# Alee08/multiagent-rl-rm

Measured on AMD Instinct MI355X. Metric: env×agent steps/sec at 65,536 envs (1/2/4/8 GPU) + CPU-ref parity rate, higher is better.
Workload: dtype int32; 1 GPU; FrozenLake map1, 65,536 envs/GPU x 2 agents, built-in A->B->C RM (3-state RM), random actions; n_envs_per_gpu=65536, n_envs_total=65536, n_agents=2, rm_states=4, parallelism=dp1 (env shards, no data-path collective), dispatch=queue, windows=5

## Files before the change

### include/rmx.h

```cpp
#ifndef RMX_H
#define RMX_H

#include <stdint.h>
#include <stddef.h>

#ifdef __cplusplus
extern "C" {
#endif

#define RMX_ABI_VERSION 12

#define RMX_MAX_AGENTS 8
#define RMX_MAX_CELLS 4096
#define RMX_MAX_RM_STATES 255
#define RMX_MAX_EVENTS 255

#define RMX_OK 0
#define RMX_E_INVALID (-1)
#define RMX_E_HIP (-2)
#define RMX_E_ACTION (-3)
#define RMX_E_STATE (-4)
#define RMX_E_TRACE (-5)

#define RMX_DEVICE_HOST (-1)

#define RMX_FROZEN_LAKE 0
#define RMX_OFFICE_WORLD 1

#define RMX_UP 0
#define RMX_DOWN 1
#define RMX_LEFT 2
#define RMX_RIGHT 3
#define RMX_WAIT 4

#define RMX_CELL_CAN_UP 0x01u
#define RMX_CELL_CAN_DOWN 0x02u
#define RMX_CELL_CAN_LEFT 0x04u
#define RMX_CELL_CAN_RIGHT 0x08u
#define RMX_CELL_HAZARD 0x10u

#define RMX_F_ACTIVE 0x01u
#define RMX_F_FAIL 0x02u
#define RMX_F_TERM 0x04u
#define RMX_F_TRUNC 0x08u
#define RMX_F_ENV_TERM 0x10u
#define RMX_F_RM_TERM 0x20u
#define RMX_F_ENV_DONE 0x40u
#define RMX_F_STEPS_SHIFT 16

#define RMX_STAT_SUM_RETURN 0
#define RMX_STAT_EPISODES 1
#define RMX_STAT_SUCCESSES 2
#define RMX_STAT_SUM_LENGTH 3
#define RMX_NSTATS 4

typedef struct rmx_config {
  int32_t kind;
  int32_t width;
  int32_t height;
  int32_t n_agents;
  int32_t n_rm_states;
  int32_t n_events;
  int32_t max_t;
  int32_t device;
  int64_t n_envs;
  int64_t env_offset;
  int64_t n_envs_global;
  float hazard_penalty;
  float wall_penalty;
  int32_t hazard_fail;
  int32_t wall_fail;
  float gamma;
  int32_t has_shaping;
  float reward_modifier;
  int32_t n_qrm_max;
  int32_t stochastic;
  int32_t slip_n[4];
  int32_t slip_out[4][4];
  double slip_cdf[4][4];
  uint64_t seed_scale, seed_env_stride, seed_episode_stride;
  int32_t random_starts;
  const uint16_t* cell;
  const uint8_t* cell_event;
  const uint8_t* next_q;
  const float* rm_reward;
  const float* shape;
  const int32_t* init_q;
  const int32_t* final_q;
  const int32_t* start_xy;
  const int32_t* n_qrm;
  const uint8_t* qrm_states;
  const int32_t* enc_nq;
} rmx_config;

typedef struct rmx_buffers {
  int32_t* pos_x;
  int32_t* pos_y;
  int32_t* rm_q;
  uint32_t* flags;
  float* ep_ret;
  int32_t* t;
  float* reward;
  float* shaping;
  uint8_t* env_done;
  float* renv;
  int32_t* qrm_s;
  int32_t* qrm_sn;
  float* qrm_rq;
  uint8_t* qrm_done;
  uint64_t* rng;
  int32_t* episode;
  int32_t* enc_state;
} rmx_buffers;

typedef struct rmx_handle rmx_handle;

int rmx_abi_version(void);
int rmx_device_count(int32_t* n);
const char* rmx_last_error(void);
const char* rmx_build_info(void);

int rmx_create(const rmx_config* cfg, rmx_handle** out);
void rmx_destroy(rmx_handle* h);

int rmx_bind(rmx_handle* h, const rmx_buffers* buf);

int rmx_reset(rmx_handle* h, const uint8_t* env_mask_dev, uint64_t seed, void* hip_stream);

int rmx_step(rmx_handle* h, const int32_t* actions_dev, int autoreset, void* hip_stream);

int rmx_step_hashed(rmx_handle* h, uint64_t seed, int64_t t_global, int autoreset, void* hip_stream);

int rmx_fill_actions(rmx_handle* h, uint64_t seed, int64_t t0, int32_t T, int32_t* actions_dev,
                     void* hip_stream);

int rmx_rollout(rmx_handle* h, uint64_t seed, int64_t t0, int32_t T, float* reward_trace_dev,
                void* hip_stream);

int rmx_mdp_states(rmx_handle* h, int32_t agent, int64_t* n_states);
int rmx_mdp(rmx_handle* h, int32_t agent, int32_t fix_frozen_lake, int32_t* next_dev, float* reward_dev,
            uint8_t* done_dev, void* hip_stream);

int rmx_stats_device(rmx_handle* h, double* out_dev, void* hip_stream);
int rmx_stats_host(rmx_handle* h, double* out_host);
int rmx_stats_clear(rmx_handle* h, void* hip_stream);

int rmx_step_report(rmx_handle* h, const int32_t* actions_dev, int autoreset, double* stats_out_dev,
                    void* hip_stream);
int rmx_step_report_fused(const rmx_handle* h);

int rmx_step_seq(rmx_handle* h, const int32_t* actions_dev, int64_t action_stride, int32_t n_steps, int autoreset,
                 double* stats_out_dev, void* hip_stream);
int rmx_seq_packed(const rmx_handle* h);
int rmx_queue_counters(const rmx_handle* h, int64_t* out3);
#define RMX_QUEUE_INFO_N 7
#define RMX_QUEUE_UNUSED 0
#define RMX_QUEUE_READY 1
#define RMX_QUEUE_UNAVAILABLE 2
#define RMX_QUEUE_RETIRED 3
#define RMX_SEQ_NONE 0
#define RMX_SEQ_QUEUE 1
#define RMX_SEQ_STREAM_KERNEL 2
#define RMX_SEQ_STREAM_DISABLED 3
#define RMX_SEQ_STREAM_QUEUE 4
#define RMX_SEQ_HOST 5
int rmx_queue_info(const rmx_handle* h, int64_t* out, int32_t n);
int rmx_queue_timing(rmx_handle* h, int every);
int rmx_queue_times(const rmx_handle* h, uint64_t* stamps, int64_t cap, int64_t* n);
int rmx_code_object_check(const void* co, size_t bytes, int64_t* n_step_kernels, int64_t* n_refused, char* report,
                          size_t report_cap);

#define RMX_VARIANT_GENERIC 0
#define RMX_VARIANT_LANE_PER_AGENT 1
#define RMX_VARIANT_FAST 2
#define RMX_VARIANT_FAST_LANE_PER_AGENT 3
#define RMX_VARIANT_HOST 4
int rmx_step_variant(const rmx_handle* h);

#define RMX_STEP_INFO_N 14
#define RMX_TABLES_NONE 0
#define RMX_TABLES_GLOBAL 1
#define RMX_TABLES_MERGED 2
#define RMX_TABLES_MERGED4 3
int rmx_step_info(const rmx_handle* h, int64_t* out, int32_t n);

typedef struct rmx_learn_config {
  double gamma, learning_rate ;
  int32_t use_qrm, use_rsh, trunc_is_terminal, dynamics ;
  const double* phi;
} rmx_learn_config;
#define RMX_LEARN_DYN_FIXED 0
#define RMX_LEARN_DYN_ENV 1
#define RMX_LEARN_UPDATE 1
#define RMX_LEARN_BEST 2
#define RMX_LEARN_NUMPY 4
int rmx_learn_states(const rmx_handle* h, int64_t* s_max);
int rmx_learn_bind(rmx_handle* h, const rmx_learn_config* cfg, double* q, double* visits);
int rmx_learn_step(rmx_handle* h, const int32_t* actions, int autoreset, void* hip_stream);
int rmx_learn_step_policy(rmx_handle* h, double epsilon, int flags, uint64_t seed, int64_t t_global, int autoreset,
                          int32_t* actions_out, void* hip_stream);
#define RMX_LEARN_RUN_MAX 4096
int rmx_learn_run(rmx_handle* h, int32_t T, double epsilon, int flags, uint64_t seed, int64_t t_global,
                  int32_t* actions_out , void* hip_stream);
int rmx_learn_rng_bind(rmx_handle* h, uint64_t* rng);
int rmx_learn_rng_seed(rmx_handle* h, const uint64_t* seeds_host , void* hip_stream);

int rmx_learn_lambda_slots(const rmx_handle* h, int32_t* l_full);
int rmx_learn_lambda_bind(rmx_handle* h, double lambd, int32_t cap, int32_t* trace_idx, double* trace_val,
                          int32_t* trace_cnt);
int rmx_learn_traces_clear(rmx_handle* h, const uint8_t* env_mask_dev, void* hip_stream);

int rmx_learn_eps_bind(rmx_handle* h, double* eps , double eps_end, double eps_decay);
int rmx_learn_eps_decay(rmx_handle* h, const uint8_t* env_mask , void* hip_stream);

int rmx_check_errors(rmx_handle* h);

int rmx_state_bytes(const rmx_handle* h, size_t* bytes);
int rmx_get_state(rmx_handle* h, void* host_blob, size_t bytes);
int rmx_set_state(rmx_handle* h, const void* host_blob, size_t bytes);

#define RMX_SYNC_MAX_ENVS 256
int rmx_reset_sync(rmx_handle* h, uint64_t seed, const rmx_buffers* out_host, void* hip_stream);
int rmx_step_sync(rmx_handle* h, const int32_t* actions_host, int autoreset, const rmx_buffers* out_host,
                  void* hip_stream);
int rmx_step_sync_begin(rmx_handle* h, const int32_t* actions_host, int autoreset, void* hip_stream);
int rmx_sync_wait(rmx_handle* h, const rmx_buffers* out_host);
int rmx_sync_end(rmx_handle* h);

#ifdef __cplusplus
}
#endif

#endif
```

### multiagent-rl-rm_amd/csrc/rmx_capi.cpp

```cpp
#include <algorithm>
#include <cstdlib>
#include <cstring>
#include <exception>
#include <string>
#include <vector>

#include "rmx_handle.h"

using namespace rmx::capi;

rmx::KParams rmx::capi::base_params(const rmx_handle* h) {
  rmx::KParams p;
  std::memset(&p, 0, sizeof(p));
  const rmx_config& c = h->cfg;
  p.tables = reinterpret_cast<const uint4*>(h->d_tables);
  p.tables_n16 = (int32_t)(h->tables_bytes / 16);
  p.skip_same = h->generic_skip;
  p.off_cell = h->off_cell;
  p.off_ev = h->off_ev;
  p.off_nq = h->off_nq;
  p.off_rr = h->off_rr;
  p.off_sh = h->off_sh;
  p.off_qrm = h->off_qrm;
  p.reward_modifier = c.reward_modifier;
  p.n_qrm_max = c.n_qrm_max;
  p.stochastic = c.stochastic ? 1 : 0;
  rmx::slip_fill(p, c);
  p.seed_scale = c.seed_scale;
  p.seed_env_stride = c.seed_env_stride;
  p.seed_episode_stride = c.seed_episode_stride;
  p.base_seed = h->base_seed;
  p.rng = h->buf.rng;
  p.episode = h->buf.episode;
  p.rng_on = (c.stochastic || c.random_starts) ? 1 : 0;
  p.random_starts = c.random_starts ? 1 : 0;
  p.n_free = h->n_free;
  p.free_cells = h->d_free;
  p.start_ws = h->d_start_ws;
  if (h->d_rsc) {
    p.rs_cells = reinterpret_cast<uint32_t*>(h->d_rsc);
    p.rs_rng = reinterpret_cast<uint64_t*>(h->d_rsc + rmx::start_cache_rng_off(c.n_agents, c.n_envs));
  }
  for (int a = 0; a < RMX_MAX_AGENTS; ++a) {
    p.n_qrm[a] = h->n_qrm[a];
    p.enc_nq[a] = h->enc_nq[a];
  }
  p.W = c.width;
  p.HW = c.width * c.height;
  p.A = c.n_agents;
  p.Q = c.n_rm_states;
  p.E = c.n_events;
  p.max_t = c.max_t;
  p.N = c.n_envs;
  p.hazard_penalty = c.hazard_penalty;
  p.wall_penalty = c.wall_penalty;
  p.hazard_fail = c.hazard_fail ? 1 : 0;
  p.wall_fail = c.wall_fail ? 1 : 0;
  p.has_shaping = c.has_shaping ? 1 : 0;
  p.gamma_is_one = (c.gamma == 1.0f) ? 1 : 0;
  for (int a = 0; a < RMX_MAX_AGENTS; ++a) {
    p.init_q[a] = h->init_q[a];
    p.final_q[a] = h->final_q[a];
    p.start_x[a] = h->start_x[a];
    p.start_y[a] = h->start_y[a];
  }
  p.disc = h->d_disc;
  p.pos_x = h->buf.pos_x;
  p.pos_y = h->buf.pos_y;
  p.rm_q = h->buf.rm_q;
  p.flags = h->buf.flags;
  p.ep_ret = h->buf.ep_ret;
  p.t = h->buf.t;
  p.reward = h->buf.reward;
  p.shaping = h->buf.shaping;
  p.env_done = h->buf.env_done;
  p.renv = h->buf.renv;
  p.enc_state = h->buf.enc_state;
  if (c.n_qrm_max > 0 && h->buf.qrm_s) {
    p.qrm_s = h->buf.qrm_s;
    p.qrm_sn = h->buf.qrm_sn;
    p.qrm_rq = h->buf.qrm_rq;
    p.qrm_done = h->buf.qrm_done;
  }
  p.env_offset = c.env_offset;
  p.n_global = c.n_envs_global;
  p.slab = h->d_slab;
  p.err = h->d_err;
  p.diag = h->diag;
  return p;
}

rmx::FastParams rmx::capi::fast_params(const rmx_handle* h) {
  rmx::FastParams p;
  std::memset(&p, 0, sizeof(p));
  const rmx_config& c = h->cfg;
  p.tables = reinterpret_cast<const uint4*>(h->d_fast);
  p.n16 = h->fast_n16;
  p.off_rm = h->fast_off_rm;
  p.off_info = h->fast_off_info;
  p.A = c.n_agents;
  p.W = c.width;
  p.E = c.n_events;
  p.max_t = c.max_t;
  p.N = (int32_t)c.n_envs;
  for (int a = 0; a < c.n_agents; ++a) {
    p.mv_base[a] = a * c.width * c.height * 5;
    p.rm_base[a] = a * c.n_rm_states * c.n_events;
    p.final_q[a] = h->final_q[a];
    p.init_q[a] = h->init_q[a];
    p.start_x[a] = h->start_x[a];
    p.start_y[a] = h->start_y[a];
  }
  p.hazard_penalty = c.hazard_penalty;
  p.wall_penalty = c.wall_penalty;
  p.has_shaping = c.has_shaping ? 1 : 0;
  p.gamma_is_one = (c.gamma == 1.0f) ? 1 : 0;
  p.tbl_mode = h->fast_tables;
  p.H = c.height;
  p.hazard_fail = c.hazard_fail ? 1 : 0;
  p.wall_fail = c.wall_fail ? 1 : 0;
  p.merged = reinterpret_cast<const uint4*>(h->d_merged);
  p.merged4 = h->merged4_bytes ? reinterpret_cast<const uint32_t*>(static_cast<unsigned char*>(h->d_merged) + h->merged4_off)
                               : nullptr;
  p.merged4_bytes = (int32_t)h->merged4_bytes;
  std::memcpy(p.mg_palb, h->mg_palb, sizeof(p.mg_palb));
  p.merged_bytes = (int32_t)h->merged_bytes;
  if (c.n_qrm_max > 0 && h->buf.qrm_s) {
    p.qrm_s = h->buf.qrm_s;
    p.qrm_sn = h->buf.qrm_sn;
    p.qrm_rq = h->buf.qrm_rq;
    p.qrm_done = h->buf.qrm_done;
    p.n_qrm_max = c.n_qrm_max;
    for (int a = 0; a < c.n_agents; ++a) {
      p.n_qrm[a] = h->n_qrm[a];
      p.enc_nq[a] = h->enc_nq[a];
      for (int j = 0; j < c.n_qrm_max && j < rmx::kFastMaxQrm; ++j) p.qrm_q[a][j] = h->fast_qrm_q[a][j];
    }
  }
  p.HW = c.width * c.height;
  for (int a = 0; a < c.n_agents; ++a) {
    p.mg_base[a] = h->mg_base[a];
    p.enc_nq[a] = h->enc_nq[a];
  }
  p.disc = h->d_disc;
  p.pos_x = h->buf.pos_x;
  p.pos_y = h->buf.pos_y;
  p.rm_q = h->buf.rm_q;
  p.flags = h->buf.flags;
  p.ep_ret = h->buf.ep_ret;
  p.t = h->buf.t;
  p.reward = h->buf.reward;
  p.shaping = h->buf.shaping;
  p.env_done = h->buf.env_done;
  p.renv = h->buf.renv;
  p.enc_state = h->buf.enc_state;
  p.env_offset = c.env_offset;
  p.n_global = c.n_envs_global;
  p.wave_stats = h->fast_wave_stats;
  p.skip_same = h->fast_skip;
  p.block = h->fast_block;
  p.slab = h->d_slab;
  p.es_ret = h->es_ret;
  p.es_cnt = h->es_cnt;
  p.es_succ = h->es_succ;
  p.err = h->d_err;
  p.diag = h->diag;
  p.stamps = h->d_stamps;
  p.pk = h->seq.d_pk;
  if (c.stochastic || c.random_starts) {
    p.slip = (c.stochastic ? rmx::kRngSlip : 0) | (c.random_starts ? rmx::kRngStarts : 0) |
             (h->seed_fixed ? rmx::kRngFixedSeed : 0);
    p.n_free = h->n_free;
    p.free_cells = h->d_free;
    p.start_ws = h->d_start_ws;
    if (h->d_rsc) {
      p.rs_cells = reinterpret_cast<const uint32_t*>(h->d_rsc);
      p.rs_rng = reinterpret_cast<const uint64_t*>(h->d_rsc + rmx::start_cache_rng_off(c.n_agents, c.n_envs));
      p.rs_dirty = h->rs_dirty ? 1 : 0;
    }
    if (h->d_nx) {
      const size_t N = (size_t)c.n_envs;
      p.nx_rng = reinterpret_cast<uint64_t*>(h->d_nx);
      p.nx_idx = reinterpret_cast<int32_t*>(h->d_nx + 32 * N);
      p.nx_ep = reinterpret_cast<int32_t*>(h->d_nx + 36 * N);
      p.rs_jump = reinterpret_cast<const uint4*>(h->d_nx + nx_jump_offset(c.n_envs));
    }
    rmx::slip_fill(p, c);
    p.seed_scale = c.seed_scale;
    p.seed_env_stride = c.seed_env_stride;
    p.seed_episode_stride = c.seed_episode_stride;
    p.base_seed = h->base_seed;
    p.rng = h->buf.rng;
    p.episode = h->buf.episode;
  }
  return p;
}

bool rmx::capi::fast_applies(const rmx_handle* h) {
  if (h->fast && (h->cfg.stochastic || h->cfg.random_starts)) {
    const int tm = h->fast_tables;
    return !h->buf.qrm_s && h->fast_skip == rmx::kSkipRare && (tm == rmx::kTblMerged4 || tm == rmx::kTblMerged) &&
           h->cfg.n_envs < ((int64_t)1 << 27) &&
           (!h->cfg.random_starts || h->seed_fixed || h->n_free + 8 <= rmx::kRsRowMax);
  }
  const int qmax = h->cfg.n_agents <= 2 ? rmx::kFastMaxQrm : 8;
  return h->fast && (!h->buf.qrm_s || (h->cfg.n_qrm_max <= qmax &&
                                       (int64_t)h->cfg.n_qrm_max * h->cfg.n_agents * h->cfg.n_envs < ((int64_t)1 << 30)));
}

hipError_t rmx::capi::reduce_stats(const rmx_handle* h, double* out, hipStream_t st) {
  double* partial = h->d_slab + (size_t)RMX_NSTATS * h->n_waves;
  unsigned int* ticket = reinterpret_cast<unsigned int*>(partial + (size_t)RMX_NSTATS * 2 * rmx::kStatsPartials);
  return rmx::launch_stats_reduce(h->d_slab, h->n_waves, h->es_ret, h->es_cnt, h->es_succ, h->cfg.n_envs, partial,
                                  ticket, out, st);
}

static hipError_t invalidate_next_shuffles(const rmx_handle* h, hipStream_t st) {
  if (!h->d_nx) return hipSuccess;
  const size_t N = (size_t)h->cfg.n_envs;
  return hipMemsetAsync(h->d_nx + 36 * N, 0xFF, 4 * N, st);
}

hipError_t rmx::capi::refresh_starts(rmx_handle* h, hipStream_t st) {
  hipError_t e = hipSuccess;
  if (h->d_rsc) e = rmx::launch_reset(base_params(h), nullptr, 0, st);
  if (e == hipSuccess) e = invalidate_next_shuffles(h, st);
  if (e == hipSuccess) h->rs_stale = false;
  return e;
}

int rmx::capi::starts_current(rmx_handle* h, void* stream) {
  if (h->rs_stale) HIP_TRY(refresh_starts(h, as_stream(stream)), "start cache refresh");
  return RMX_OK;
}

rmx::FastParams rmx::capi::step_fp(const rmx_handle* h, const int32_t* actions, uint64_t seed, int64_t t_global,
                                   int autoreset) {
  rmx::FastParams fp = fast_params(h);
  if (!h->cfg.random_starts) fp.slip &= ~rmx::kRngFixedSeed;
  fp.actions = actions;
  fp.seed = seed;
  fp.t_global = t_global;
  fp.autoreset = autoreset ? 1 : 0;
  if (fp.qrm_s) fp.tbl_mode = rmx::kTblGlobal;
  return fp;
}

int rmx::capi::do_step(rmx_handle* h, const int32_t* actions, int hashed, uint64_t seed, int64_t t_global, int autoreset,
                       void* stream) {
  int rc = check_bound(h);
  if (rc) return rc;
  if (!hashed && !actions) return fail(RMX_E_INVALID, "actions is NULL");
  if (h->host) {
    h->host->step(actions, autoreset, hashed != 0, seed, t_global);
    return RMX_OK;
  }
  SYNC_END_OR_RETURN(h);
  HIP_TRY(hipSetDevice(h->device), "hipSetDevice");
  if ((rc = starts_current(h, stream))) return rc;
  if (fast_applies(h)) {
    const rmx::FastParams fp = step_fp(h, actions, seed, t_global, autoreset);
    HIP_TRY(rmx::launch_step_fast(fp, hashed, h->cfg.kind, as_stream(stream)), "step launch");
    return RMX_OK;
  }
  rmx::KParams p = base_params(h);
  p.actions = actions;
  p.seed = seed;
  p.t_global = t_global;
  p.autoreset = autoreset ? 1 : 0;
  HIP_TRY(rmx::launch_step(p, hashed, h->cfg.kind, h->step_layout, grid_for(h, h->step_layout), dim3(h->block), h->tables_bytes, as_stream(stream)),
          "step launch");
  return RMX_OK;
}

bool rmx::capi::report_fuses(const rmx_handle* h) {
  const int64_t grid = (h->cfg.n_envs + 63) / 64;
  const int tm = h->fast_tables;
  return fast_applies(h) && !h->buf.qrm_s && !h->fast_wave_stats && h->fast_block == 64 &&
         h->fast_skip == rmx::kSkipRare && h->rpt_partial &&
         (tm == rmx::kTblMerged4 || tm == rmx::kTblMerged || tm == rmx::kTblGlobal) && h->n_waves <= 64 * grid;
}

rmx::FastParams rmx::capi::report_fp(const rmx_handle* h, const int32_t* actions, int autoreset, double* stats_out) {
  rmx::FastParams fp = fast_params(h);
  fp.actions = actions;
  fp.autoreset = autoreset ? 1 : 0;
  const int64_t grid = (h->cfg.n_envs + 63) / 64;
  fp.rpt_out = stats_out;
  fp.rpt_partial = h->rpt_partial;
  fp.rpt_ticket = h->rpt_ticket;
  fp.rpt_cs = (int32_t)((h->n_waves + grid - 1) / grid);
  fp.rpt_n_slab = (int32_t)h->n_waves;
  return fp;
}

extern "C" {

int rmx_abi_version(void) { return RMX_ABI_VERSION; }

int rmx_device_count(int32_t* n) {
  if (!n) return fail(RMX_E_INVALID, "n is NULL");
  int c = 0;
  const hipError_t e = hipGetDeviceCount(&c);
  *n = e == hipSuccess ? c : 0;
  return RMX_OK;
}

const char* rmx_last_error(void) { return g_err.c_str(); }

void rmx_destroy(rmx_handle* h) {
  if (!h) return;
  if (h->host) {
    delete h->host;
    delete h;
    return;
  }
  (void)hipSetDevice(h->device);
  (void)sync_end(h);
  if (h->sync.mb) (void)hipHostFree(h->sync.mb);
  if (h->sync.done) (void)hipEventDestroy(h->sync.done);
  if (h->sync.dep) (void)hipEventDestroy(h->sync.dep);
  if (h->sync.stream) (void)hipStreamDestroy(h->sync.stream);
  (void)hipFree(h->d_tables);
  (void)hipFree(h->d_disc);
  (void)hipFree(h->d_slab);
  (void)hipFree(h->d_stats);
  (void)hipFree(h->d_err);
  (void)hipFree(h->d_fast);
  (void)hipFree(h->d_merged);
  (void)hipFree(h->d_es);
  (void)hipFree(h->d_stamps);
  (void)hipFree(h->d_free);
  (void)hipFree(h->d_start_ws);
  (void)hipFree(h->d_nx);
  (void)hipFree(h->d_rsc);
  (void)hipFree(h->seq.d_pk);
  (void)hipFree(h->learn.d_phi);
  delete h;
}

int rmx_bind(rmx_handle* h, const rmx_buffers* b) {
  if (!h || !b) return fail(RMX_E_INVALID, "handle or buffers NULL");
  if (!b->pos_x || !b->pos_y || !b->rm_q || !b->flags || !b->ep_ret || !b->t || !b->reward)
    return fail(RMX_E_STATE, "a required state/output buffer is NULL");
  const bool any_qrm = b->qrm_s || b->qrm_sn || b->qrm_rq || b->qrm_done;
  const bool all_qrm = b->qrm_s && b->qrm_sn && b->qrm_rq && b->qrm_done;
  if (any_qrm && !all_qrm) return fail(RMX_E_STATE, "QRM outputs must be all bound or all NULL");
  if (all_qrm && h->cfg.n_qrm_max == 0) return fail(RMX_E_STATE, "QRM outputs bound but n_qrm_max == 0");
  if ((h->cfg.stochastic || h->cfg.random_starts) && (!b->rng || !b->episode))
    return fail(RMX_E_STATE, "stochastic mode / random starts need the rng and episode buffers");
  if (b->enc_state)
    for (int a = 0; a < h->cfg.n_agents; ++a)
      if (h->enc_nq[a] < 1) return fail(RMX_E_STATE, "enc_state bound but enc_nq not provided at rmx_create");
  if (h->host) {
    h->host->bind(*b);
    h->buf = *b;
    h->bound = true;
    return RMX_OK;
  }
  SYNC_END_OR_RETURN(h);
  if (h->sync.mb) {
    (void)hipHostFree(h->sync.mb);
    h->sync.mb = nullptr;
  }
  h->buf = *b;
  h->bound = true;
  h->rs_dirty = true;
  return RMX_OK;
}

int rmx_reset(rmx_handle* h, const uint8_t* env_mask_dev, uint64_t seed, void* stream) {
  int rc = check_bound(h);
  if (rc) return rc;
  if (h->host) {
    h->host->reset(env_mask_dev, seed);
    h->base_seed = seed;
    return RMX_OK;
  }
  SYNC_END_OR_RETURN(h);
  h->rs_dirty = env_mask_dev ? (h->rs_dirty || seed != h->base_seed) : false;
  h->base_seed = seed;
  HIP_TRY(hipSetDevice(h->device), "hipSetDevice");
  rmx::KParams p = base_params(h);
  HIP_TRY(rmx::launch_reset(p, env_mask_dev, 1, as_stream(stream)), "reset launch");
  HIP_TRY(invalidate_next_shuffles(h, as_stream(stream)), "reset precompute");
  h->rs_stale = false;
  return lambda_clear(h, env_mask_dev, stream);
}

int rmx_step(rmx_handle* h, const int32_t* actions_dev, int autoreset, void* stream) {
  return do_step(h, actions_dev, 0, 0, 0, autoreset, stream);
}

int rmx_step_report(rmx_handle* h, const int32_t* actions_dev, int autoreset, double* stats_out_dev, void* stream) {
  int rc = check_bound(h);
  if (rc) return rc;
  if (!actions_dev || !stats_out_dev) return fail(RMX_E_INVALID, "bad rmx_step_report arguments");
  if (h->host) {
    h->host->step(actions_dev, autoreset);
    std::memcpy(stats_out_dev, h->host->stats, sizeof(h->host->stats));
    return RMX_OK;
  }
  SYNC_END_OR_RETURN(h);
  if (!report_fuses(h)) {
    if ((rc = do_step(h, actions_dev, 0, 0, 0, autoreset, stream))) return rc;
    HIP_TRY(reduce_stats(h, stats_out_dev, as_stream(stream)), "stats launch");
    return RMX_OK;
  }
  HIP_TRY(hipSetDevice(h->device), "hipSetDevice");
  const rmx::FastParams fp = report_fp(h, actions_dev, autoreset, stats_out_dev);
  HIP_TRY(rmx::launch_step_fast(fp, 0, h->cfg.kind, as_stream(stream)), "step launch");
  return RMX_OK;
}

int rmx_step_report_fused(const rmx_handle* h) { return h && h->bound && report_fuses(h) ? 1 : 0; }

int rmx_step_hashed(rmx_handle* h, uint64_t seed, int64_t t_global, int autoreset, void* stream) {
  if (t_global < 0) return fail(RMX_E_INVALID, "t_global < 0");
  return do_step(h, nullptr, 1, seed, t_global, autoreset, stream);
}

int rmx_fill_actions(rmx_handle* h, uint64_t seed, int64_t t0, int32_t T, int32_t* actions_dev, void* stream) {
  if (!h || !actions_dev || T < 0 || t0 < 0) return fail(RMX_E_INVALID, "bad rmx_fill_actions arguments");
  if (T == 0) return RMX_OK;
  if (h->host) {
    h->host->fill_actions(seed, t0, T, actions_dev);
    return RMX_OK;
  }
  HIP_TRY(hipSetDevice(h->device), "hipSetDevice");
  HIP_TRY(rmx::launch_fill_actions(seed, t0, T, h->cfg.n_envs_global, h->cfg.env_offset, h->cfg.n_envs,
                                   h->cfg.n_agents, actions_dev, as_stream(stream)),
          "fill_actions launch");
  return RMX_OK;
}

int rmx_rollout(rmx_handle* h, uint64_t seed, int64_t t0, int32_t T, float* trace, void* stream) {
  int rc = check_bound(h);
  if (rc) return rc;
  if (T < 0 || t0 < 0) return fail(RMX_E_INVALID, "bad rollout length");
  if (T == 0) return RMX_OK;
  if (h->host) {
    const size_t AN = (size_t)h->cfg.n_agents * (size_t)h->cfg.n_envs;
    for (int32_t it = 0; it < T; ++it) h->host->step(nullptr, 1, true, seed, t0 + it, trace ? trace + (size_t)it * AN : nullptr);
    return RMX_OK;
  }
  SYNC_END_OR_RETURN(h);
  HIP_TRY(hipSetDevice(h->device), "hipSetDevice");
  if ((rc = starts_current(h, stream))) return rc;
  if (h->fast && ((!h->cfg.stochastic && !h->cfg.random_starts) || fast_applies(h))) {
    rmx::FastParams fp = fast_params(h);
    fp.seed = seed;
    fp.t_global = t0;
    fp.autoreset = 1;
    const bool merged = fp.tbl_mode == rmx::kTblMerged || fp.tbl_mode == rmx::kTblMerged4;
    const size_t rs_lds = h->cfg.random_starts ? 4 * (size_t)rmx::kRsWaveLds : 0;
    if (h->rollout_lds && (!merged || ((h->merged_bytes + 15) & ~(size_t)15) + rs_lds <= rmx::kRolloutLdsMax)) {
      fp.tbl_mode = merged ? rmx::kTblMergedLds : rmx::kTblLds;
      fp.block = 256;
    } else {
      fp.tbl_mode = merged ? rmx::kTblMerged : rmx::kTblGlobal;
    }
    HIP_TRY(rmx::launch_rollout_fast(fp, h->cfg.kind, T, trace, as_stream(stream)), "rollout launch");
    return RMX_OK;
  }
  rmx::KParams p = base_params(h);
  p.seed = seed;
  p.t_global = t0;
  p.autoreset = 1;
  HIP_TRY(rmx::launch_rollout(p, h->cfg.kind, h->rollout_layout, T, trace, grid_for(h, h->rollout_layout), dim3(h->block), h->tables_bytes,
                              as_stream(stream)),
          "rollout launch");
  return RMX_OK;
}

int rmx_mdp_states(rmx_handle* h, int32_t agent, int64_t* n_states) {
  if (!h || !n_states || agent < 0 || agent >= h->cfg.n_agents) return fail(RMX_E_INVALID, "bad rmx_mdp_states arguments");
  if (h->enc_nq[agent] < 1) return fail(RMX_E_INVALID, "enc_nq not provided at rmx_create");
  *n_states = (int64_t)h->cfg.width * h->cfg.height * h->enc_nq[agent];
  return RMX_OK;
}

int rmx_mdp(rmx_handle* h, int32_t agent, int32_t fix_frozen_lake, int32_t* next_dev, float* reward_dev,
            uint8_t* done_dev, void* stream) {
  int64_t S = 0;
  int rc = rmx_mdp_states(h, agent, &S);
  if (rc) return rc;
  if (!next_dev || !reward_dev || !done_dev) return fail(RMX_E_INVALID, "rmx_mdp output is NULL");
  if (h->host) {
    h->host->mdp(agent, fix_frozen_lake ? 1 : 0, next_dev, reward_dev, done_dev);
// ... 118 lines not shown
```

### multiagent-rl-rm_amd/csrc/rmx_capi_create.cpp

```cpp
#include <algorithm>
#include <cstdlib>
#include <cstring>
#include <exception>
#include <string>
#include <vector>

#include "rmx_handle.h"

using namespace rmx::capi;

namespace {

int validate(const rmx_config* c) {
  if (!c) return fail(RMX_E_INVALID, "config is NULL");
  const std::string msg = rmx::validate_config(*c);
  return msg.empty() ? RMX_OK : fail(RMX_E_INVALID, msg);
}

int create_host(const rmx_config* cfg, rmx_handle** out) {
  rmx_handle* h = new rmx_handle();
  h->host = new rmx::HostEngine();
  const std::string msg = h->host->init(*cfg);
  if (!msg.empty()) {
    delete h->host;
    delete h;
    return fail(RMX_E_INVALID, msg);
  }
  h->cfg = h->host->cfg;
  h->device = RMX_DEVICE_HOST;
  h->digest = rmx::config_digest(*cfg);
  for (int a = 0; a < cfg->n_agents; ++a) h->enc_nq[a] = h->host->p.enc_nq[a];
  *out = h;
  return RMX_OK;
}

struct RsJumpTable {
  uint32_t w[64][2][4];
  RsJumpTable() {
    typedef unsigned __int128 u128;
    const u128 M = ((u128)0x2360ED051FC65DA4ull << 64) | 0x4385DF649FCCF645ull;
    u128 mj = 1, sj = 0;
    for (int j = 0; j < 64; ++j) {
      sj += mj;
      mj *= M;
      const u128 v[2] = {mj, sj};
      for (int k = 0; k < 2; ++k)
        for (int q = 0; q < 4; ++q) w[j][k][q] = (uint32_t)(v[k] >> (32 * q));
    }
  }
};
const RsJumpTable rs_jump_table;

}

extern "C" {

struct CreateTables {
  std::vector<unsigned char> blob, fast_blob;
  std::vector<uint32_t> merged_tab;
  std::vector<float> disc;
  std::vector<uint16_t> free_cells;
};

static void create_env(rmx_handle* h, const rmx_config* cfg) {
  if (const char* qv = std::getenv("RMX_QUEUE")) h->seq.queue_off = std::strcmp(qv, "0") == 0;
  if (const char* pv = std::getenv("RMX_SEQ_PACKED")) h->seq.packed_off = std::strcmp(pv, "0") == 0;
  if (const char* b = std::getenv("RMX_BLOCK")) {
    int v = std::atoi(b);
    if (v == 64 || v == 128 || v == 256) h->block = v;
  }
#ifdef RMX_DIAG
  if (const char* d = std::getenv("RMX_DIAG_BITS")) h->diag = std::atoi(d);
#endif
  const bool rng_on = cfg->stochastic || cfg->random_starts;
  if (rng_on) h->rollout_layout = rmx::kLayoutThreadPerEnv;
  if (const char* l = std::getenv("RMX_LAYOUT")) {
    if (!std::strcmp(l, "tpe")) h->step_layout = h->rollout_layout = rmx::kLayoutThreadPerEnv;
    if (!std::strcmp(l, "lpe") && !rng_on) h->step_layout = h->rollout_layout = rmx::kLayoutLanePerAgent;
  }
}

static bool create_plan(rmx_handle* h, const rmx_config* cfg, CreateTables& tb) {
  const int A = cfg->n_agents;
  for (int a = 0; a < A; ++a) {
    h->init_q[a] = cfg->init_q[a];
    h->final_q[a] = cfg->final_q[a];
    h->start_x[a] = cfg->start_xy[2 * a];
    h->start_y[a] = cfg->start_xy[2 * a + 1];
  }
  rmx::BlobOffsets bo;
  if (!rmx::build_table_blob(*cfg, tb.blob, bo)) return false;
  h->tables_bytes = tb.blob.size();
  h->digest = rmx::config_digest(*cfg);
  h->off_cell = bo.cell;
  h->off_ev = bo.ev;
  h->off_nq = bo.nq;
  h->off_rr = bo.rr;
  h->off_sh = bo.sh;
  h->off_qrm = bo.qrm;
  if (cfg->n_qrm_max > 0) {
    for (int a = 0; a < A; ++a) {
      h->n_qrm[a] = cfg->n_qrm[a];
      for (int j = 0; j < cfg->n_qrm_max && j < rmx::kFastMaxQrm; ++j)
        h->fast_qrm_q[a][j] = cfg->qrm_states[a * cfg->n_qrm_max + j];
    }
  }
  for (int a = 0; a < A; ++a) h->enc_nq[a] = cfg->enc_nq ? cfg->enc_nq[a] : 0;
  tb.disc = rmx::discount_table(*cfg);
  if (cfg->random_starts) tb.free_cells = rmx::free_cells(*cfg);
  h->n_free = (int32_t)tb.free_cells.size();
  const int64_t gmax = std::max(grid_for(h, h->step_layout).x, grid_for(h, h->rollout_layout).x);
  std::vector<unsigned char>& fast_blob = tb.fast_blob;
  std::vector<uint32_t>& merged_tab = tb.merged_tab;
  {
    const char* fe = std::getenv("RMX_FAST");
    const bool want = fe ? std::strcmp(fe, "0") != 0 : true;
    rmx::FastLayout fl;
    h->fast = want && h->step_layout == rmx::kLayoutThreadPerEnv && rmx::build_fast_blob(*cfg, fast_blob, fl);
    h->fast_off_rm = fl.off_rm;
    h->fast_off_info = fl.off_info;
    h->fast_n16 = (int32_t)(fast_blob.size() / 16);
    if (h->fast) {
      std::vector<uint32_t> probe;
      const bool ok = rmx::build_merged(*cfg, fast_blob, h->fast_off_rm, h->mg_base, probe);
      h->fast_tables = ok && probe.size() * 4 <= kFastMergedDefaultBytes ? rmx::kTblMerged : rmx::kTblGlobal;
      if (h->fast_tables == rmx::kTblMerged && !cfg->stochastic) h->fast_tables = rmx::kTblMerged4;
    }
    if (const char* ft = std::getenv("RMX_FAST_TABLES")) {
      if (!std::strcmp(ft, "global")) h->fast_tables = rmx::kTblGlobal;
      if (!std::strcmp(ft, "merged")) h->fast_tables = rmx::kTblMerged;
      if (!std::strcmp(ft, "merged4")) h->fast_tables = rmx::kTblMerged4;
    }
    const bool want_m4 = h->fast_tables == rmx::kTblMerged4;
    if (h->fast && (h->fast_tables == rmx::kTblMerged || want_m4) &&
        !rmx::build_merged(*cfg, fast_blob, h->fast_off_rm, h->mg_base, merged_tab))
      h->fast_tables = rmx::kTblGlobal;
    if (want_m4 && h->fast_tables != rmx::kTblGlobal) {
      std::vector<uint32_t> compact;
      if (rmx::build_compact(*cfg, h->mg_base, merged_tab, h->mg_palb, compact)) {
        h->merged4_off = merged_tab.size() * 4;
        h->merged4_bytes = compact.size() * 4;
        merged_tab.insert(merged_tab.end(), compact.begin(), compact.end());
        while (merged_tab.size() % 4) merged_tab.push_back(0u);
      } else {
        h->fast_tables = rmx::kTblMerged;
      }
    }
    if (h->fast && h->fast_tables != rmx::kTblGlobal) {
      const size_t sec_words = (size_t)cfg->n_rm_states * cfg->width * cfg->height * 5 * 4;
      const size_t words16 = h->merged4_bytes ? h->merged4_off / 4 : merged_tab.size();
      h->merged_sections = (int)(words16 / sec_words);
    }
    if (!merged_tab.empty()) h->merged_bytes = h->merged4_bytes ? h->merged4_off : merged_tab.size() * 4;
  }
  h->seed_fixed = h->fast && (cfg->stochastic || cfg->random_starts) && cfg->seed_episode_stride == 0;
  h->n_waves = std::max<int64_t>(gmax * (h->block / 64), (cfg->n_envs + 255) / 256 * 4);
  h->fast_wave_stats = cfg->n_envs >= kFastWaveStatsMinEnvs ? 1 : 0;
  if (const char* fs = std::getenv("RMX_FAST_STATS")) h->fast_wave_stats = !std::strcmp(fs, "wave") ? 1 : 0;
  h->fast_skip = cfg->n_envs * (int64_t)cfg->n_agents >= kFastNtMinInstances ? rmx::kSkipRareNT : rmx::kSkipRare;
  h->generic_skip = cfg->n_envs >= kFastSkipMinEnvs ? 1 : 0;
  if (const char* fk = std::getenv("RMX_FAST_SKIP")) {
    const int v = std::atoi(fk);
    if (v == rmx::kSkipRare || v == rmx::kSkipRareNT) h->fast_skip = v;
  }
  if (const char* gk = std::getenv("RMX_GENERIC_SKIP")) h->generic_skip = std::atoi(gk) ? 1 : 0;
  h->fast_block = cfg->n_envs >= kFastSkipMinEnvs ? 256 : 64;
  if (const char* rl = std::getenv("RMX_ROLLOUT_LDS")) h->rollout_lds = std::atoi(rl) ? 1 : 0;
  return true;
}

static hipError_t create_upload(rmx_handle* h, const rmx_config* cfg, const CreateTables& tb) {
  hipError_t e = hipSuccess;
  auto put = [&e](auto** p, size_t bytes, int fill, const void* src = nullptr, size_t src_bytes = 0) {
    if (e == hipSuccess) e = hipMalloc(p, bytes);
    if (e == hipSuccess && fill >= 0) e = hipMemset(*p, fill, bytes);
    if (e == hipSuccess && src) e = hipMemcpy(*p, src, src_bytes, hipMemcpyHostToDevice);
  };
  const size_t N = (size_t)cfg->n_envs;
#ifdef RMX_DIAG
  if (std::getenv("RMX_DIAG_STAMPS")) put(&h->d_stamps, (N + 255) / 256 * 4 * 2 * rmx::kStamps * 8, 0);
#endif
  if (h->fast && !h->fast_wave_stats) {
    const size_t o_cnt = 8 * N, o_succ = o_cnt + 8 * N, o_part = (o_succ + 4 * N + 15) & ~size_t(15);
    const size_t o_ticket = (o_part + sizeof(double) * RMX_NSTATS * ((N + 63) / 64) + 127) & ~size_t(127);
    h->es_bytes = o_ticket + 128 * (1 + 32);
    put(&h->d_es, h->es_bytes, 0);
    if (e == hipSuccess) {
      h->es_ret = reinterpret_cast<double*>(h->d_es);
      h->es_cnt = reinterpret_cast<unsigned long long*>(h->d_es + o_cnt);
      h->es_succ = reinterpret_cast<uint32_t*>(h->d_es + o_succ);
      h->rpt_partial = reinterpret_cast<double*>(h->d_es + o_part);
      h->rpt_ticket = reinterpret_cast<unsigned int*>(h->d_es + o_ticket);
    }
  }
  put(&h->d_tables, h->tables_bytes, -1, tb.blob.data(), h->tables_bytes);
  put(&h->d_disc, sizeof(float) * tb.disc.size(), -1, tb.disc.data(), sizeof(float) * tb.disc.size());
  put(&h->d_slab, sizeof(double) * (RMX_NSTATS * (h->n_waves + 2 * rmx::kStatsPartials) + 2), 0);
  put(&h->d_stats, sizeof(double) * RMX_NSTATS, -1);
  put(&h->d_err, sizeof(uint32_t), 0);
  if (h->n_free > 0) {
    put(&h->d_free, sizeof(uint16_t) * (tb.free_cells.size() + 1), 0, tb.free_cells.data(),
        sizeof(uint16_t) * tb.free_cells.size());
    put(&h->d_start_ws, sizeof(uint16_t) * (size_t)rmx::shuffle_stride((int32_t)tb.free_cells.size()) * N, -1);
    if (!h->seed_fixed) {
      put(&h->d_nx, nx_jump_offset(cfg->n_envs) + sizeof(rs_jump_table.w), -1);
      if (e == hipSuccess) e = hipMemset(h->d_nx + 36 * N, 0xFF, 4 * N);
      if (e == hipSuccess)
        e = hipMemcpy(h->d_nx + nx_jump_offset(cfg->n_envs), rs_jump_table.w, sizeof(rs_jump_table.w), hipMemcpyHostToDevice);
    }
  }
  if (h->seed_fixed) put(&h->d_rsc, rmx::start_cache_bytes(cfg->n_agents, cfg->n_envs), 0);
  if (h->fast) put(&h->d_fast, tb.fast_blob.size(), -1, tb.fast_blob.data(), tb.fast_blob.size());
  if (!tb.merged_tab.empty())
    put(&h->d_merged, tb.merged_tab.size() * 4, -1, tb.merged_tab.data(), tb.merged_tab.size() * 4);
  return e;
}

int rmx_create(const rmx_config* cfg, rmx_handle** out) {
  if (!out) return fail(RMX_E_INVALID, "out is NULL");
  *out = nullptr;
  int rc = validate(cfg);
  if (rc) return rc;
  if (cfg->device == RMX_DEVICE_HOST) {
    try {
      return create_host(cfg, out);
    } catch (const std::exception& e) {
      return fail(RMX_E_INVALID, std::string("rmx_create (host): ") + e.what());
    }
  }
  if (cfg->device < 0) return fail(RMX_E_INVALID, "device must be a HIP device ordinal or RMX_DEVICE_HOST");
  HIP_TRY(hipSetDevice(cfg->device), "hipSetDevice");
  rmx_handle* h = new rmx_handle();
  h->cfg = *cfg;
  h->device = cfg->device;
  create_env(h, cfg);
  CreateTables tb;
  if (!create_plan(h, cfg, tb)) {
    delete h;
    return fail(RMX_E_INVALID, "tables exceed 64 KiB of LDS");
  }
  const hipError_t e = create_upload(h, cfg, tb);
  if (e != hipSuccess) {
    rmx_destroy(h);
    return hip_fail(e, "rmx_create allocation/upload");
  }
  h->cfg.cell = nullptr;
  h->cfg.cell_event = nullptr;
  h->cfg.next_q = nullptr;
  h->cfg.rm_reward = nullptr;
  h->cfg.shape = nullptr;
  h->cfg.init_q = h->cfg.final_q = h->cfg.start_xy = nullptr;
  h->cfg.n_qrm = h->cfg.enc_nq = nullptr;
  h->cfg.qrm_states = nullptr;
  *out = h;
  return RMX_OK;
}

}
```

### multiagent-rl-rm_amd/csrc/rmx_capi_seq.cpp

```cpp
#include <algorithm>
#include <atomic>
#include <cstring>
#include <exception>

#include "rmx_handle.h"

using namespace rmx::capi;

static bool seq_packs(const rmx_handle* h) {
  const int tm = h->fast_tables;
  return !h->seq.packed_off && !h->seq.pk_failed && !h->seq.pk_refused && h->cfg.n_envs < kFastWaveStatsMinEnvs &&
         rmx::pk_bytes(h->cfg.n_agents, (size_t)h->cfg.n_envs) < ((size_t)1 << 31) && fast_applies(h) && !h->cfg.stochastic && !h->cfg.random_starts &&
         !h->buf.qrm_s && !h->fast_wave_stats && h->fast_skip == rmx::kSkipRare &&
         (tm == rmx::kTblMerged4 || tm == rmx::kTblMerged) && h->cfg.n_agents <= rmx::kFastMaxAgents;
}

static bool seq_pack_buffer(rmx_handle* h) {
  if (h->seq.d_pk) return true;
  if (hipMalloc(&h->seq.d_pk, rmx::pk_bytes(h->cfg.n_agents, (size_t)h->cfg.n_envs)) != hipSuccess) {
    (void)hipGetLastError();
    h->seq.d_pk = nullptr;
    h->seq.pk_failed = true;
    return false;
  }
  return true;
}

static bool record_seq(rmx_handle* h, const int32_t* actions, int64_t stride, int32_t K, int autoreset,
                       double* stats_out, bool fused, bool packed) {
  h->seq.window.resize((size_t)K);
  for (int32_t k = 0; k < K; ++k) {
    const int32_t* a = actions + (size_t)k * (size_t)stride;
    const bool rpt = fused && k == K - 1;
    rmx::FastParams fp = rpt ? report_fp(h, a, autoreset, stats_out) : step_fp(h, a, 0, 0, autoreset);
    if (packed) fp.pk_io = k == 0 ? rmx::kIoColsToPk : (k == K - 1 ? rmx::kIoPkToCols : rmx::kIoPkToPk);
    rmx::StepCapture cap{&h->seq.window[(size_t)k], false};
    rmx::tl_capture = &cap;
    (void)rmx::launch_step_fast(fp, 0, h->cfg.kind, nullptr);
    rmx::tl_capture = nullptr;
    if (!cap.ok) return false;
    if (packed && !std::strstr(h->seq.window[(size_t)k].symbol, "step_fast_kernel_win")) return false;
  }
  return true;
}

static std::atomic<uint64_t> g_seq_keys{0};
constexpr int32_t kSeqMaxSteps = 1 << 20;

static int step_seq(rmx_handle* h, const int32_t* actions_dev, int64_t action_stride, int32_t n_steps, int autoreset,
                    double* stats_out_dev, void* stream) {
  int rc = check_bound(h);
  if (rc) return rc;
  if (!actions_dev || n_steps <= 0 || action_stride < 0) return fail(RMX_E_INVALID, "bad rmx_step_seq arguments");
  if (h->host) {
    h->seq.dispatch = RMX_SEQ_HOST;
    for (int32_t k = 0; k < n_steps; ++k) h->host->step(actions_dev + (size_t)k * (size_t)action_stride, autoreset);
    if (stats_out_dev) std::memcpy(stats_out_dev, h->host->stats, sizeof(h->host->stats));
    return RMX_OK;
  }
  SYNC_END_OR_RETURN(h);
  HIP_TRY(hipSetDevice(h->device), "hipSetDevice");
  if ((rc = starts_current(h, stream))) return rc;
  hipStream_t st = as_stream(stream);
  const bool fused = stats_out_dev && report_fuses(h);
  auto on_stream = [&](int why) {
    h->seq.dispatch = why;
    for (int32_t k = 0; k < n_steps; ++k) {
      const int32_t* a = actions_dev + (size_t)k * (size_t)action_stride;
      const int r = stats_out_dev && k == n_steps - 1 ? rmx_step_report(h, a, autoreset, stats_out_dev, stream)
                                                      : do_step(h, a, 0, 0, 0, autoreset, stream);
      if (r) return r;
    }
    HIP_TRY(hipStreamSynchronize(st), "step sequence");
    return (int)RMX_OK;
  };
  if (!fast_applies(h) || h->seq.queue_off) {
    rmx::queue_note_stream(h->device);
    return on_stream(h->seq.queue_off && fast_applies(h) ? RMX_SEQ_STREAM_DISABLED : RMX_SEQ_STREAM_KERNEL);
  }
  const bool packed = n_steps >= 2 && seq_packs(h) && seq_pack_buffer(h);
  rmx::FastParams base = fast_params(h);
  const bool same = h->seq.key && h->seq.actions == actions_dev && h->seq.stride == action_stride &&
                    h->seq.k == n_steps && h->seq.autoreset == (autoreset ? 1 : 0) && h->seq.out == stats_out_dev &&
                    std::memcmp(&base, &h->seq.base, sizeof(base)) == 0;
  if (!same) {
    h->seq.key = 0;
    h->seq.is_packed = packed && record_seq(h, actions_dev, action_stride, n_steps, autoreset, stats_out_dev, fused, true);
    if (packed && !h->seq.is_packed) {
      h->seq.pk_refused = true;
      (void)hipFree(h->seq.d_pk);
      h->seq.d_pk = nullptr;
      base = fast_params(h);
    }
    if (!h->seq.is_packed &&
        !record_seq(h, actions_dev, action_stride, n_steps, autoreset, stats_out_dev, fused, false)) {
      rmx::queue_note_stream(h->device);
      return on_stream(RMX_SEQ_STREAM_KERNEL);
    }
    ++h->seq.recordings;
    std::memcpy(&h->seq.base, &base, sizeof(base));
    h->seq.actions = actions_dev;
    h->seq.out = stats_out_dev;
    h->seq.stride = action_stride;
    h->seq.k = n_steps;
    h->seq.autoreset = autoreset ? 1 : 0;
    h->seq.key = ++g_seq_keys;
  }
  const hipError_t q = hipStreamQuery(st);
  if (q == hipErrorNotReady) HIP_TRY(hipStreamSynchronize(st), "step sequence");
  else if (q != hipSuccess) return hip_fail(q, "step sequence");
  std::string err;
  const int qr = rmx::queue_run(h->device, h->seq.window.data(), n_steps, h->seq.key, &err);
  if (qr == rmx::kQueueStream) return on_stream(RMX_SEQ_STREAM_QUEUE);
  if (qr) {
    h->seq.key = 0;
    h->seq.dispatch = RMX_SEQ_QUEUE;
    return fail(RMX_E_HIP, err);
  }
  h->seq.dispatch = RMX_SEQ_QUEUE;
  if (stats_out_dev && !fused) {
    HIP_TRY(reduce_stats(h, stats_out_dev, st), "stats launch");
    HIP_TRY(hipStreamSynchronize(st), "step sequence");
  }
  return RMX_OK;
}

extern "C" {

int rmx_step_seq(rmx_handle* h, const int32_t* actions_dev, int64_t action_stride, int32_t n_steps, int autoreset,
                 double* stats_out_dev, void* stream) {
  if (n_steps > kSeqMaxSteps) return fail(RMX_E_INVALID, "rmx_step_seq: more steps than one window takes");
  try {
    return step_seq(h, actions_dev, action_stride, n_steps, autoreset, stats_out_dev, stream);
  } catch (const std::exception& e) {
    if (h) h->seq.key = 0;
    return fail(RMX_E_HIP, std::string("rmx_step_seq: ") + e.what());
  }
}

int rmx_seq_packed(const rmx_handle* h) {
  return h && !h->host && h->seq.dispatch == RMX_SEQ_QUEUE && h->seq.key && h->seq.is_packed ? 1 : 0;
}

int rmx_queue_counters(const rmx_handle* h, int64_t* out3) {
  if (!h || !out3) return fail(RMX_E_INVALID, "bad rmx_queue_counters arguments");
  rmx::QueueInfo qi{0, 0, 0, 0, RMX_QUEUE_UNUSED};
  if (!h->host) rmx::queue_info(h->device, &qi);
  out3[0] = qi.windows;
  out3[1] = qi.uploads;
  out3[2] = qi.packets;
  return RMX_OK;
}

int rmx_queue_info(const rmx_handle* h, int64_t* out, int32_t n) {
  if (!h || !out || n < 0) return fail(RMX_E_INVALID, "bad rmx_queue_info arguments");
  rmx::QueueInfo qi{0, 0, 0, 0, RMX_QUEUE_UNUSED};
  if (!h->host) rmx::queue_info(h->device, &qi);
  const int64_t v[RMX_QUEUE_INFO_N] = {qi.windows,         qi.uploads,      qi.packets, qi.stream_windows, qi.state,
                                       h->seq.dispatch, h->seq.recordings};
  for (int32_t i = 0; i < n && i < RMX_QUEUE_INFO_N; ++i) out[i] = v[i];
  return RMX_OK;
}

int rmx_queue_timing(rmx_handle* h, int every) {
  if (!h || every < 0) return fail(RMX_E_INVALID, "bad rmx_queue_timing arguments");
  if (h->host) return RMX_OK;
  rmx::queue_set_timing(h->device, every);
  return RMX_OK;
}

int rmx_queue_times(const rmx_handle* h, uint64_t* stamps, int64_t cap, int64_t* n) {
  if (!h || !n || cap < 0 || (cap > 0 && !stamps)) return fail(RMX_E_INVALID, "bad rmx_queue_times arguments");
  *n = h->host || h->seq.dispatch != RMX_SEQ_QUEUE ? 0 : rmx::queue_times(h->device, stamps, cap);
  return RMX_OK;
}

int rmx_code_object_check(const void* co, size_t bytes, int64_t* n_step_kernels, int64_t* n_refused, char* report,
                          size_t report_cap) {
  if (!n_step_kernels || !n_refused || (co && bytes == 0)) return fail(RMX_E_INVALID, "bad rmx_code_object_check arguments");
  try {
    std::string first;
    const int rc = rmx::code_object_check(co, bytes, n_step_kernels, n_refused, &first);
    if (report && report_cap) {
      const size_t n = std::min(first.size(), report_cap - 1);
      std::memcpy(report, first.data(), n);
      report[n] = 0;
    }
    return rc ? fail(RMX_E_INVALID, "rmx_code_object_check: " + first) : RMX_OK;
  } catch (const std::exception& e) {
    return fail(RMX_E_INVALID, std::string("rmx_code_object_check: ") + e.what());
  }
}

}
```

### multiagent-rl-rm_amd/csrc/rmx_fast.hip

```cpp
#include <hip/hip_runtime.h>

#include <cstddef>
#include <cstdio>
#include <cstring>
#include <type_traits>
#include <stdint.h>

#include "rmx_device.h"
#include "rmx_internal.h"

namespace rmx {

namespace {

__device__ __forceinline__ __amdgpu_buffer_rsrc_t col_rsrc(const void* base, uint32_t bytes) {
  return __builtin_amdgcn_make_buffer_rsrc(const_cast<void*>(base), 0, (int)bytes, 0x00020000);
}
constexpr int kStoreAux = 16;
constexpr int kStoreAuxNT = 18;
__device__ __forceinline__ int32_t col_ld(__amdgpu_buffer_rsrc_t r, uint32_t lane_bytes, uint32_t sgpr_bytes) {
  return __builtin_amdgcn_raw_buffer_load_b32(r, lane_bytes, sgpr_bytes, 0);
}
#ifdef RMX_DIAG
__device__ __forceinline__ void col_st_d(__amdgpu_buffer_rsrc_t r, uint32_t lane_bytes, uint32_t sgpr_bytes, int32_t v,
// ... 443 lines not shown
  for (int a = 0; a < A; ++a) {
    int32_t pos = a;
#pragma unroll
    for (int k = 1; k < A; ++k) {
      const int32_t jk = lrow[n + k];
      pos = pos == k ? jk : (pos == jk ? k : pos);
    }
    for (int32_t h = 0; h < n; ++h) {
      const int32_t f = lrow[pos];
      if (f == 0) break;
      pos = f;
    }
    slot[a] = pos;
  }
}

constexpr int kRsCoopLanes = 8;
typedef unsigned __int128 u128;
__device__ __forceinline__ uint64_t rl64(uint64_t v, int l) {
  return ((uint64_t)(uint32_t)__builtin_amdgcn_readlane((int)(uint32_t)(v >> 32), l) << 32) |
         (uint32_t)__builtin_amdgcn_readlane((int)(uint32_t)v, l);
}

template <bool CHAIN>
__device__ __forceinline__ void rs_coop_finish(const FastParams& p, RsNext& nx, bool need, unsigned char* row,
                                               uint32_t lane, uint4* blk, int32_t n, int A) {
  uint2* outs = reinterpret_cast<uint2*>(blk + kRsCoopLanes * 64);
  if (!__any(need)) return;
  const uint4 m4 = p.rs_jump[2 * lane], s4 = p.rs_jump[2 * lane + 1];
  const u128 MJ = ((u128)(((uint64_t)m4.w << 32) | m4.z) << 64) | (((uint64_t)m4.y << 32) | m4.x);
  const u128 SJ = ((u128)(((uint64_t)s4.w << 32) | s4.z) << 64) | (((uint64_t)s4.y << 32) | s4.x);
  bool mine = need;
  while (true) {
    uint64_t todo = __ballot(mine && nx.i > 0);
    if (todo == 0) break;
    int slot_of_me = -1;
    for (int g = 0; g < kRsCoopLanes && todo != 0; ++g) {
      const int L = __builtin_ctzll(todo);
      todo &= todo - 1;
      const u128 s = ((u128)rl64(nx.g.hi, L) << 64) | rl64(nx.g.lo, L);
      const u128 c = ((u128)rl64(nx.g.ihi, L) << 64) | rl64(nx.g.ilo, L);
      const u128 sl = MJ * s + SJ * c;
      const uint64_t hi = (uint64_t)(sl >> 64), lo = (uint64_t)sl;
      blk[g * 64 + lane] = make_uint4((uint32_t)lo, (uint32_t)(lo >> 32), (uint32_t)hi, (uint32_t)(hi >> 32));
      const uint64_t x = hi ^ lo;
      const unsigned rot = (unsigned)(hi >> 58);
      const uint64_t o = (x >> rot) | (x << ((64u - rot) & 63u));
      outs[g * 64 + lane] = make_uint2((uint32_t)o, (uint32_t)(o >> 32));
      slot_of_me = (int)lane == L ? g : slot_of_me;
    }
    asm volatile("" ::: "memory");
    if (slot_of_me >= 0) {
      uint32_t mask = rs_mask(nx.i);
      const uint2* mo = outs + slot_of_me * 64;
      int q = 0;
      for (; q < 64 && nx.i > 0; ++q) {
        const uint2 o = mo[q];
        rs_take<CHAIN>(nx, mask, o.x, row, n, A);
        if (nx.i > 0) rs_take<CHAIN>(nx, mask, o.y, row, n, A);
      }
      const uint4 last = blk[slot_of_me * 64 + q - 1];
      nx.g.hi = ((uint64_t)last.w << 32) | last.z;
      nx.g.lo = ((uint64_t)last.y << 32) | last.x;
    }
    asm volatile("" ::: "memory");
  }
}

template <int A>
__device__ __forceinline__ void rs_step(const FastParams& p, Pcg& rng, int32_t& episode, RsNext& nx, bool rs, bool live,
                                        int64_t e_global, unsigned char* row, unsigned char* lds, uint32_t tid,
                                        int32_t (&sx)[A], int32_t (&sy)[A]) {
  const int32_t n = p.n_free;
  constexpr bool CHAIN = A >= 3;
  const bool any_rs = __any(rs && live);
  uint32_t fc0 = 0, fc1 = 0;
  const uint32_t lane = tid & 63u;
  if (any_rs) {
    const auto rf = col_rsrc(p.free_cells, ((uint32_t)n * 2u + 3u) & ~3u);
    fc0 = __builtin_amdgcn_raw_buffer_load_b32(rf, lane * 4u, 0, 0);
    fc1 = __builtin_amdgcn_raw_buffer_load_b32(rf, lane * 4u + 256u, 0, 0);
  }
  if (rs) episode += 1;
  const int32_t want = rs ? episode : episode + 1;
  if (live && nx.k != want) {
    nx.g = seed_pcg64(seed_of(p, e_global, want));
    nx.i = n - 1;
    nx.k = want;
    nx.fresh = true;
    if constexpr (CHAIN) rs_clear_row(row, n);
  }
  int32_t slot[A];
  if (any_rs)
    rs_coop_finish<CHAIN>(p, nx, rs && live && nx.i > 0, row, lane,
                   reinterpret_cast<uint4*>(lds + (tid >> 6) * (uint32_t)kRsWaveLds + 512u), n, A);
  if (rs) {
    if (live) {
      asm volatile("" ::: "memory");
      if constexpr (CHAIN)
        rs_undo_chain<A>(row, n, lds + (tid >> 6) * (uint32_t)kRsWaveLds + 512u + lane * (uint32_t)kRsRowMax, slot);
      else
        rs_undo_full<A>(row, n, slot);
      rng = nx.g;
      nx.g = seed_pcg64(seed_of(p, e_global, episode + 1));
      nx.i = n - 1;
      nx.k = episode + 1;
      nx.fresh = true;
      if constexpr (CHAIN) rs_clear_row(row, n);
    } else {
      rng = seed_pcg64(seed_of(p, e_global, episode));
    }
  }
  if (__any(live && nx.i > 0)) {
    if (live) rs_draws<CHAIN>(nx, row, kRsDrawsPerStep / 2, n, A);
  }
  if (any_rs) {
    uint32_t* cw = reinterpret_cast<uint32_t*>(lds + (tid >> 6) * (uint32_t)kRsWaveLds);
    cw[lane] = fc0;
    cw[lane + 64] = fc1;
    asm volatile("" ::: "memory");
    if (rs && live) {
      const uint16_t* cells = reinterpret_cast<const uint16_t*>(cw);
#pragma unroll
      for (int a = 0; a < A; ++a) {
        const int32_t c = (int32_t)cells[slot[a]];
        sx[a] = c % p.W;
        sy[a] = c / p.W;
      }
    }
  }
}


template <int KIND, int A, bool HASHED, int TBL, int QXB = 0, int SKIP = kSkipNone, bool RPT = false,
          int SLIP = 0>
__global__ void __launch_bounds__(256) step_fast_kernel(int32_t N_arg, int32_t blk_arg, const int32_t* x_arg,
                                                        const int32_t* y_arg, const int32_t* q_arg,
                                                        const uint32_t* f_arg, const int32_t* t_arg,
                                                        const int32_t* act_arg, FastParams p) {
  constexpr int IO = kIoCols;
#include "rmx_fast_step.inc"
}

template <int KIND, int A, int TBL, bool RPT, int IO>
__global__ void __launch_bounds__(256) step_fast_kernel_win(int32_t N_arg, int32_t blk_arg, const int32_t* x_arg,
                                                            const int32_t* y_arg, const int32_t* q_arg,
                                                            const uint32_t* f_arg, const int32_t* t_arg,
                                                            const int32_t* act_arg, FastParams p) {
  constexpr bool HASHED = false;
  constexpr int QXB = 0, SKIP = kSkipRare, SLIP = 0;
#include "rmx_fast_step.inc"
}

template <int KIND, int A, int TBL, int SLIP = 0>
__global__ void __launch_bounds__(256) rollout_fast_kernel(FastParams p, int32_t T, float* __restrict__ trace) {
  static_assert(TBL == kTblGlobal || TBL == kTblMerged || TBL == kTblLds || TBL == kTblMergedLds,
                "rollout: global / merged tables, in L2 or LDS");
  static_assert(!SLIP || TBL == kTblMerged || TBL == kTblMergedLds, "rollout slip: merged tables");
  constexpr bool RNG = SLIP != 0, DRAW = (SLIP & kRngSlip) != 0;
  constexpr bool RSTART = (SLIP & kRngStarts) != 0 && KIND == RMX_FROZEN_LAKE;
  constexpr bool OW_SLIP = DRAW && KIND == RMX_OFFICE_WORLD;
  constexpr bool MERGED = TBL == kTblMerged || TBL == kTblMergedLds;
  constexpr bool IN_LDS = TBL == kTblLds || TBL == kTblMergedLds;
  extern __shared__ __attribute__((aligned(16))) unsigned char lds[];
  const int tid = threadIdx.x;
  if constexpr (IN_LDS) {
    const uint4* src = MERGED ? p.merged : p.tables;
    const int n16 = MERGED ? p.merged_bytes / 16 : p.n16;
    for (int i = tid; i < n16; i += (int)blockDim.x) reinterpret_cast<uint4*>(lds)[i] = src[i];
    __syncthreads();
  }
  const uint32_t mg_n16 = (uint32_t)p.merged_bytes / 16u;
  const uint32_t rs_lds_off = IN_LDS ? ((uint32_t)(MERGED ? p.merged_bytes : p.n16 * 16) + 15u) & ~15u : 0u;
  const int32_t N = p.N;
  const int32_t e_raw = (int32_t)(blockIdx.x * blockDim.x) + tid;
  const bool live = e_raw < N;
  const int32_t e = live ? e_raw : N - 1;
  const uint32_t off = (uint32_t)e * 4u;
  const uint32_t col = (uint32_t)N * 4u;
  const uint32_t cols = col * (uint32_t)A;
  const auto r_x = col_rsrc(p.pos_x, cols), r_y = col_rsrc(p.pos_y, cols), r_q = col_rsrc(p.rm_q, cols);
  const auto r_f = col_rsrc(p.flags, cols), r_ret = col_rsrc(p.ep_ret, cols), r_t = col_rsrc(p.t, col);
  const auto r_rew = col_rsrc(p.reward, cols);
  AgentIO s[A];
  int32_t t = col_ld(r_t, off, 0);
#pragma unroll
  for (int a = 0; a < A; ++a) {
    s[a].x = col_ld(r_x, off, a * col);
    s[a].y = col_ld(r_y, off, a * col);
    s[a].q = col_ld(r_q, off, a * col);
    s[a].f = (uint32_t)col_ld(r_f, off, a * col);
    s[a].ret = __int_as_float(col_ld(r_ret, off, a * col));
  }
  Pcg rng = {0ull, 0ull, 0ull, 0ull};
  int32_t episode = 0;
  if constexpr (RNG) {
    rng = {p.rng[e], p.rng[(int64_t)N + e], p.rng[2 * (int64_t)N + e], p.rng[3 * (int64_t)N + e]};
    episode = p.episode[e];
  }
  constexpr bool FIXED = RNG && (SLIP & kRngFixedSeed) != 0;
  constexpr bool FCELLS = FIXED && RSTART;
  uint32_t fcw[FCELLS ? (A + 1) / 2 : 1] = {};
  Pcg frng = {0ull, 0ull, 0ull, 0ull};
  if constexpr (FIXED) {
    if constexpr (FCELLS)
#pragma unroll
      for (int w = 0; w < (A + 1) / 2; ++w) fcw[w] = p.rs_cells[(int64_t)w * N + e];
    frng = {p.rs_rng[e], p.rs_rng[(int64_t)N + e], p.rs_rng[2 * (int64_t)N + e], p.rs_rng[3 * (int64_t)N + e]};
  }
  RsNext nx = {{0ull, 0ull, 0ull, 0ull}, 0, -1, 0, false};
  unsigned char* rs_row = nullptr;
  if constexpr (RSTART && !FIXED) {
    nx.g = {p.nx_rng[e], p.nx_rng[(int64_t)N + e], p.nx_rng[2 * (int64_t)N + e], p.nx_rng[3 * (int64_t)N + e]};
    nx.i = p.nx_idx[e];
    nx.k = p.nx_ep[e];
    nx.i0 = nx.i;
    rs_row = reinterpret_cast<unsigned char*>(p.start_ws) + (size_t)e * (size_t)(2 * shuffle_stride(p.n_free));
  }
  const auto mg = col_rsrc(p.merged, MERGED ? (uint32_t)p.merged_bytes : 0u);
  const auto tb = make_tables<!IN_LDS>(lds, p);
  const int64_t eg = p.env_offset + e;
  uint64_t ctr[A];
#pragma unroll
  for (int a = 0; a < A; ++a)
    ctr[a] = (((uint64_t)p.t_global * (uint64_t)p.n_global + (uint64_t)eg) * (uint64_t)A + (uint64_t)a) * kGolden;
  const uint64_t dctr = (uint64_t)p.n_global * (uint64_t)A * kGolden;
  LaneStats ls = {0.0, 0, 0, 0};
  uint32_t bad = 0, done = 0;
  AgentRes o[A];
  for (int32_t it = 0; it < T; ++it) {
    const bool rs = (s[0].f & RMX_F_ENV_DONE) != 0;
    t = rs ? 0 : t;
    const int32_t t1 = t + 1;
    const float disc = p.gamma_is_one ? 1.0f : p.disc[min((uint32_t)t, (uint32_t)p.max_t + 1u)];
    int32_t sx[A], sy[A];
#pragma unroll
    for (int a = 0; a < A; ++a) sx[a] = p.start_x[a], sy[a] = p.start_y[a];
    if constexpr (RNG) {
      if constexpr (FIXED) {
        if (rs) {
          if constexpr (FCELLS) fixed_start_cells<A>(fcw, sx, sy);
          rng = frng;
          episode += 1;
        }
      } else if constexpr (RSTART)
        rs_step<A>(p, rng, episode, nx, rs, live, eg, rs_row, lds + rs_lds_off, (uint32_t)tid, sx, sy);
      else
        random_start_reset<A, false>(p, rng, episode, rs, live, eg, lds, (uint32_t)tid, rs_lds_off, sx, sy);
    }
    AgentTmp k[A];
    uint32_t m[A];
    uint4 r[A];
    auto record = [&](int a, uint32_t mi) {
      const uint32_t idx = (uint32_t)p.mg_base[a] + __umul24(__umul24((uint32_t)s[a].q, (uint32_t)p.HW), 5u) + mi;
      if constexpr (IN_LDS) {
        return reinterpret_cast<const uint4*>(lds)[min(idx, mg_n16 - 1u)];
      } else {
        const auto v = __builtin_amdgcn_raw_buffer_load_b128(mg, idx * 16u, 0, 0);
        return make_uint4(v[0], v[1], v[2], v[3]);
      }
    };
    uint32_t blocked[OW_SLIP ? A : 1] = {};
#pragma unroll
    for (int a = 0; a < A; ++a) {
      s[a].act = (int32_t)(splitmix64(p.seed ^ ctr[a]) >> 62);
      ctr[a] += dctr;
      s[a].x = rs ? sx[a] : s[a].x;
      s[a].y = rs ? sy[a] : s[a].y;
      s[a].q = rs ? p.init_q[a] : s[a].q;
      s[a].f = rs ? RMX_F_ACTIVE : s[a].f;
      s[a].ret = rs ? 0.0f : s[a].ret;
    }
    if constexpr (OW_SLIP) {
      uint32_t wi[A];
#pragma unroll
      for (int a = 0; a < A; ++a) wi[a] = record(a, move_index<KIND>(s[a], (uint32_t)p.final_q[a], 0u, p, bad, k[a])).x;
#pragma unroll
      for (int a = 0; a < A; ++a) {
        const uint32_t ac = agent_action<KIND>(s[a], (uint32_t)p.final_q[a], bad, k[a]);
        blocked[a] = (ac < (uint32_t)RMX_WAIT && (wi[a] & kMvWall)) ? 1u : 0u;
        s[a].act = (int32_t)(blocked[a] ? (uint32_t)RMX_WAIT
                                        : (ac < (uint32_t)RMX_WAIT ? (uint32_t)slip_choice(p, (int32_t)ac, rng) : ac));
      }
    }
#pragma unroll
    for (int a = 0; a < A; ++a) {
      if constexpr (DRAW && KIND == RMX_FROZEN_LAKE) {
        if ((s[a].f & RMX_F_ACTIVE) && (uint32_t)s[a].q != (uint32_t)p.final_q[a])
          s[a].act = slip_choice(p, s[a].act, rng);
      }
      if constexpr (MERGED) {
        r[a] = record(a, move_index<KIND>(s[a], (uint32_t)p.final_q[a], 0u, p, bad, k[a]));
      } else {
        m[a] = tb.mv(move_index<KIND>(s[a], (uint32_t)p.final_q[a], (uint32_t)p.mv_base[a], p, bad, k[a]));
      }
    }
#pragma unroll
    for (int a = 0; a < A; ++a) {
      if constexpr (OW_SLIP) {
        const uint32_t hz = __builtin_amdgcn_ubfe(r[a].x, 25, 1);
        const uint32_t fl = (blocked[a] & (uint32_t)p.wall_fail) | (hz & (uint32_t)p.hazard_fail);
        r[a].x = (r[a].x & ~(kMvWall | kMvFail)) | (blocked[a] << 24) | (fl << 26);
      }
      if constexpr (MERGED) {
        const uint32_t w0 = r[a].x;
        k[a].mm = k[a].moving ? w0 : 0u;
// ... 16 lines not shown
    double rsum = 0.0;
    int succ = 0;
#pragma unroll
    for (int a = 0; a < A; ++a) {
      s[a].f |= done ? RMX_F_ENV_DONE : 0u;
      rsum += (double)s[a].ret;
      succ += (int)o[a].succ;
      if (trace && live) trace[((int64_t)it * A + a) * N + e] = o[a].reward;
    }
    if (done && live) {
      ls.ret += rsum;
      ls.episodes += 1;
      ls.successes += succ;
      ls.length += t1;
    }
  }
  if (live) {
    col_st(r_t, off, 0, t);
    if (p.env_done) byte_st(p, (uint32_t)e, done);
    if constexpr (RNG) {
      p.rng[e] = rng.hi;
      p.rng[(int64_t)N + e] = rng.lo;
      p.rng[2 * (int64_t)N + e] = rng.ihi;
      p.rng[3 * (int64_t)N + e] = rng.ilo;
      p.episode[e] = episode;
    }
    if constexpr (RSTART && !FIXED) {
      p.nx_rng[e] = nx.g.hi;
      p.nx_rng[(int64_t)N + e] = nx.g.lo;
      p.nx_rng[2 * (int64_t)N + e] = nx.g.ihi;
      p.nx_rng[3 * (int64_t)N + e] = nx.g.ilo;
      p.nx_idx[e] = nx.i;
      p.nx_ep[e] = nx.k;
    }
#pragma unroll
    for (int a = 0; a < A; ++a) {
      col_st(r_x, off, a * col, s[a].x);
      col_st(r_y, off, a * col, s[a].y);
      col_st(r_q, off, a * col, s[a].q);
      col_st(r_f, off, a * col, (int32_t)s[a].f);
      col_st(r_ret, off, a * col, __float_as_int(s[a].ret));
      col_st(r_rew, off, a * col, __float_as_int(o[a].reward));
      if (p.shaping) col_st(col_rsrc(p.shaping, cols), off, a * col, __float_as_int(o[a].shaping));
      if (p.renv) col_st(col_rsrc(p.renv, cols), off, a * col, __float_as_int(o[a].renv));
      if (p.enc_state)
        col_st(col_rsrc(p.enc_state, cols), off, a * col, (s[a].y * p.W + s[a].x) * p.enc_nq[a] + s[a].q);
    }
  } else {
    bad = 0;
  }
  if (__any(bad)) {
    if ((tid & 63) == 0) atomicOr(p.err, 1u);
  }
  wave_flush(p.slab, ls, __any(ls.episodes != 0));
}

template <int KIND, int A>
static void launch_rollout_a(const FastParams& p, int32_t T, float* trace, dim3 g, dim3 b, hipStream_t st) {
  if (p.slip) {
    auto go = [&](auto rng_flags) {
      constexpr int R = decltype(rng_flags)::value;
      const size_t rs = (R & kRngStarts) && !(R & kRngFixedSeed) ? (size_t)(b.x / 64) * (size_t)kRsWaveLds : 0;
      if (p.tbl_mode == kTblMergedLds)
        hipLaunchKernelGGL((rollout_fast_kernel<KIND, A, kTblMergedLds, R>), g, b,
                           (((size_t)p.merged_bytes + 15) & ~(size_t)15) + rs, st, p, T, trace);
      else
        hipLaunchKernelGGL((rollout_fast_kernel<KIND, A, kTblMerged, R>), g, b, rs, st, p, T, trace);
    };
    if constexpr (KIND == RMX_FROZEN_LAKE) {
      constexpr int S = kRngStarts, F = kRngStarts | kRngFixedSeed;
      if (p.slip == S) return go(std::integral_constant<int, S>{});
      if (p.slip == (kRngSlip | S)) return go(std::integral_constant<int, kRngSlip | S>{});
      if (p.slip == F) return go(std::integral_constant<int, F>{});
      if (p.slip == (kRngSlip | F)) return go(std::integral_constant<int, kRngSlip | F>{});
    }
    if (p.slip == (kRngSlip | kRngFixedSeed)) return go(std::integral_constant<int, kRngSlip | kRngFixedSeed>{});
    return go(std::integral_constant<int, kRngSlip>{});
  }
  switch (p.tbl_mode) {
    case kTblMergedLds:
      hipLaunchKernelGGL((rollout_fast_kernel<KIND, A, kTblMergedLds>), g, b, (size_t)p.merged_bytes, st, p, T, trace);
      break;
    case kTblLds:
      hipLaunchKernelGGL((rollout_fast_kernel<KIND, A, kTblLds>), g, b, (size_t)p.n16 * 16, st, p, T, trace);
      break;
    case kTblMerged: hipLaunchKernelGGL((rollout_fast_kernel<KIND, A, kTblMerged>), g, b, 0, st, p, T, trace); break;
    default: hipLaunchKernelGGL((rollout_fast_kernel<KIND, A, kTblGlobal>), g, b, 0, st, p, T, trace); break;
  }
}

template <int KIND>
static void launch_rollout_k(const FastParams& p, int32_t T, float* trace, hipStream_t st) {
  const dim3 b((unsigned)p.block), g((unsigned)(((int64_t)p.N + p.block - 1) / p.block));
  switch (p.A) {
    case 1: launch_rollout_a<KIND, 1>(p, T, trace, g, b, st); break;
    case 2: launch_rollout_a<KIND, 2>(p, T, trace, g, b, st); break;
    case 3: launch_rollout_a<KIND, 3>(p, T, trace, g, b, st); break;
    default: launch_rollout_a<KIND, 4>(p, T, trace, g, b, st); break;
  }
}

hipError_t launch_rollout_fast(const FastParams& p, int kind, int32_t T, float* trace, hipStream_t st) {
  if (kind == RMX_FROZEN_LAKE)
    launch_rollout_k<RMX_FROZEN_LAKE>(p, T, trace, st);
  else
    launch_rollout_k<RMX_OFFICE_WORLD>(p, T, trace, st);
  return hipGetLastError();
}

thread_local StepCapture* tl_capture = nullptr;

static StepArgs step_args(const FastParams& p, uint32_t blk) {
  return StepArgs{p.N, (int32_t)blk, p.pos_x, p.pos_y, p.rm_q, p.flags, p.t, p.actions, p};
}

static void capture_launch(StepCapture* c, dim3 g, dim3 b, size_t lds, const StepArgs& a, const FastParams& p) {
  StepLaunch& L = *c->out;
  L.grid = g.x;
  L.block = b.x;
  L.lds = (uint32_t)lds;
  std::memset(&L.args, 0, sizeof(L.args));
  std::memcpy(&L.args, &a, offsetof(StepArgs, p));
  std::memcpy(&L.args.p, &p, sizeof(FastParams));
  c->ok = true;
}

template <int KIND, int A, bool HASHED, int TBL, int QXB = 0, int SKIP = kSkipNone, bool RPT = false, int SLIP = 0>
static void go_step(dim3 g, dim3 b, size_t lds, hipStream_t st, const FastParams& p) {
  const StepArgs a = step_args(p, b.x);
  if (StepCapture* c = tl_capture) {
    snprintf(c->out->symbol, sizeof(c->out->symbol),
             "_ZN3rmx16step_fast_kernelILi%dELi%dELb%dELi%dELi%dELi%dELb%dELi%dEEEviiPKiS2_S2_PKjS2_S2_NS_"
             "10FastParamsE.kd",
             KIND, A, (int)HASHED, TBL, QXB, SKIP, (int)RPT, SLIP);
    return capture_launch(c, g, b, lds, a, p);
  }
  hipLaunchKernelGGL((step_fast_kernel<KIND, A, HASHED, TBL, QXB, SKIP, RPT, SLIP>), g, b, lds, st, a.N, a.blk, a.pos_x,
                     a.pos_y, a.rm_q, a.flags, a.t, a.actions, a.p);
}

template <int KIND, int A, int TBL, bool RPT, int IO>
static void go_step_win(dim3 g, dim3 b, hipStream_t st, const FastParams& p) {
  const StepArgs a = step_args(p, b.x);
  if (StepCapture* c = tl_capture) {
    snprintf(c->out->symbol, sizeof(c->out->symbol),
             "_ZN3rmx20step_fast_kernel_winILi%dELi%dELi%dELb%dELi%dEEEviiPKiS2_S2_PKjS2_S2_NS_10FastParamsE.kd", KIND, A,
             TBL, (int)RPT, IO);
    return capture_launch(c, g, b, 0, a, p);
  }
  hipLaunchKernelGGL((step_fast_kernel_win<KIND, A, TBL, RPT, IO>), g, b, 0, st, a.N, a.blk, a.pos_x, a.pos_y, a.rm_q,
                     a.flags, a.t, a.actions, a.p);
}

template <int KIND, int A, int TBL>
static void launch_win(const FastParams& p, dim3 g, dim3 b, hipStream_t st) {
  switch (p.pk_io) {
    case kIoColsToPk: go_step_win<KIND, A, TBL, false, kIoColsToPk>(g, b, st, p); break;
    case kIoPkToPk: go_step_win<KIND, A, TBL, false, kIoPkToPk>(g, b, st, p); break;
    default:
      if (p.rpt_out)
        go_step_win<KIND, A, TBL, true, kIoPkToCols>(g, b, st, p);
      else
        go_step_win<KIND, A, TBL, false, kIoPkToCols>(g, b, st, p);
      break;
  }
}

template <int KIND, int A, int QXB>
static void launch_qrm(const FastParams& p, int hashed, dim3 g, hipStream_t st) {
  if (hashed)
    go_step<KIND, A, true, kTblGlobal, QXB>(g, dim3(256), 0, st, p);
  else
    go_step<KIND, A, false, kTblGlobal, QXB>(g, dim3(256), 0, st, p);
}

template <int KIND, int A, int TBL>
static void launch_tpe_t(const FastParams& p, int hashed, hipStream_t st) {
  if constexpr (TBL == kTblGlobal) {
    if (p.qrm_s) {
      const dim3 g((unsigned)(((int64_t)p.N + 255) / 256));
      if (p.n_qrm_max <= 4)
        launch_qrm<KIND, A, 4>(p, hashed, g, st);
      else if (p.n_qrm_max <= 8 || A > 2)
        launch_qrm<KIND, A, 8>(p, hashed, g, st);
      else if constexpr (A <= 2)
        launch_qrm<KIND, A, 16>(p, hashed, g, st);
      return;
    }
  }
  const dim3 b((unsigned)p.block), g((unsigned)(((int64_t)p.N + p.block - 1) / p.block));
  if (p.skip_same == kSkipRareNT) {
    if (hashed)
      go_step<KIND, A, true, TBL, 0, kSkipRareNT>(g, b, 0, st, p);
    else
      go_step<KIND, A, false, TBL, 0, kSkipRareNT>(g, b, 0, st, p);
    return;
  }
  if constexpr (TBL == kTblMerged4 || TBL == kTblMerged) {
    if (p.slip) {
      auto go = [&](auto rng_flags) {
        constexpr int R = decltype(rng_flags)::value;
        const size_t lr = (R & kRngStarts) && !(R & kRngFixedSeed) ? (size_t)(b.x / 64) * (size_t)kRsWaveLds
                                                                      : 0;
        if (hashed)
          go_step<KIND, A, true, TBL, 0, kSkipRare, false, R>(g, b, lr, st, p);
        else if (p.rpt_out)
          go_step<KIND, A, false, TBL, 0, kSkipRare, true, R>(g, b, lr, st, p);
        else
          go_step<KIND, A, false, TBL, 0, kSkipRare, false, R>(g, b, lr, st, p);
      };
      if constexpr (KIND == RMX_FROZEN_LAKE) {
        constexpr int S = kRngStarts, F = kRngStarts | kRngFixedSeed;
        if (p.slip == S) return go(std::integral_constant<int, S>{});
        if (p.slip == (kRngSlip | S)) return go(std::integral_constant<int, kRngSlip | S>{});
        if (p.slip == F) return go(std::integral_constant<int, F>{});
        if (p.slip == (kRngSlip | F)) return go(std::integral_constant<int, kRngSlip | F>{});
      }
      return go(std::integral_constant<int, kRngSlip>{});
    }
    if (p.pk_io != kIoCols && p.pk && !hashed && !p.qrm_s && !p.wave_stats) return launch_win<KIND, A, TBL>(p, g, b, st);
  }
  if (p.rpt_out && !hashed) {
    go_step<KIND, A, false, TBL, 0, kSkipRare, true>(g, b, 0, st, p);
    return;
  }
  if (hashed)
    go_step<KIND, A, true, TBL, 0, kSkipRare>(g, b, 0, st, p);
  else
    go_step<KIND, A, false, TBL, 0, kSkipRare>(g, b, 0, st, p);
}

template <int KIND, int A>
static void launch_tpe(const FastParams& p, int hashed, hipStream_t st) {
  switch (p.tbl_mode) {
    case kTblMerged: launch_tpe_t<KIND, A, kTblMerged>(p, hashed, st); break;
    case kTblMerged4: launch_tpe_t<KIND, A, kTblMerged4>(p, hashed, st); break;
    default: launch_tpe_t<KIND, A, kTblGlobal>(p, hashed, st); break;
  }
}

template <int KIND>
static void launch_k(const FastParams& p, int hashed, hipStream_t st) {
  switch (p.A) {
    case 1: launch_tpe<KIND, 1>(p, hashed, st); break;
    case 2: launch_tpe<KIND, 2>(p, hashed, st); break;
    case 3: launch_tpe<KIND, 3>(p, hashed, st); break;
    default: launch_tpe<KIND, 4>(p, hashed, st); break;
  }
}

hipError_t launch_step_fast(const FastParams& p, int hashed, int kind, hipStream_t st) {
  if (kind == RMX_FROZEN_LAKE)
    launch_k<RMX_FROZEN_LAKE>(p, hashed, st);
  else
    launch_k<RMX_OFFICE_WORLD>(p, hashed, st);
  return hipGetLastError();
}

}
```

### multiagent-rl-rm_amd/csrc/rmx_fast_step.inc

```
  constexpr bool QRM = QXB > 0;
  constexpr bool IN_PK = IO == kIoPkToPk || IO == kIoPkToCols, OUT_PK = IO == kIoColsToPk || IO == kIoPkToPk;
  static_assert(IO == kIoCols || ((TBL == kTblMerged || TBL == kTblMerged4) && !HASHED && QXB == 0 && SLIP == 0 &&
                                  SKIP == kSkipRare),
                "packed windows: the deterministic merged-table step (x, y, rm_q come out of table bytes)");
  static_assert(!(RPT && OUT_PK), "the report rides in a window's last packet");
  static_assert(TBL == kTblGlobal || TBL == kTblMerged || TBL == kTblMerged4, "step: global or merged tables");
  static_assert(!QRM || TBL == kTblGlobal, "QRM outputs need the move word's event (global tables)");
  constexpr bool M4 = TBL == kTblMerged4;
  constexpr bool MERGED = TBL == kTblMerged || M4;
  constexpr bool STATS_FIRST = KIND == RMX_FROZEN_LAKE && A <= 2;
  constexpr bool RNG = SLIP != 0, DRAW = (SLIP & kRngSlip) != 0;
  constexpr bool RSTART = (SLIP & kRngStarts) != 0 && KIND == RMX_FROZEN_LAKE;
  constexpr int SAUX = SKIP == kSkipRareNT ? kStoreAuxNT : kStoreAux;
  const auto st = [&](__amdgpu_buffer_rsrc_t r, uint32_t lane_bytes, uint32_t sgpr_bytes, int32_t v) {
#ifdef RMX_DIAG
    if (p.diag & 32) {
      __builtin_amdgcn_raw_buffer_store_b32(v, r, lane_bytes, sgpr_bytes, 0);
      return;
    }
#endif
    __builtin_amdgcn_raw_buffer_store_b32(v, r, lane_bytes, sgpr_bytes, SAUX);
  };
  extern __shared__ __attribute__((aligned(16))) unsigned char lds[];
  const int tid = threadIdx.x;
#ifdef RMX_DIAG
  uint64_t st_clk[kStamps] = {}, st_rt[kStamps] = {};
#endif
  STAMP(0);
  constexpr bool PRE = A >= 3;
  const int32_t N = PRE ? N_arg : p.N;
#ifdef RMX_DIAG
  uint32_t wg = blockIdx.x;
  if ((p.diag & 65536) && (gridDim.x & 7u) == 0) wg = (wg & 7u) * (gridDim.x >> 3) + (wg >> 3);
  const int32_t e_raw = (int32_t)(wg * blockDim.x) + tid;
#else
  const int32_t e_raw = (int32_t)blockIdx.x * (PRE ? blk_arg : (int32_t)blockDim.x) + tid;
#endif
  const bool live = e_raw < N;
  const int32_t e = live ? e_raw : N - 1;
  const uint32_t off = (uint32_t)e * 4u;
  const uint32_t col = (uint32_t)N * 4u;
  const uint32_t cols = col * (uint32_t)A;
  const auto r_x = col_rsrc(PRE ? x_arg : p.pos_x, cols), r_y = col_rsrc(PRE ? y_arg : p.pos_y, cols);
  const auto r_q = col_rsrc(PRE ? q_arg : p.rm_q, cols), r_f = col_rsrc(PRE ? f_arg : p.flags, cols);
  const auto r_t = col_rsrc(PRE ? t_arg : p.t, col);
  const auto r_act = col_rsrc(PRE ? act_arg : p.actions, cols), r_rew = col_rsrc(p.reward, cols);
  AgentIO s[A];
  AgentIO s0[A];
  int32_t t;
  if constexpr (!IN_PK) t = col_ld(r_t, off, 0);
  __amdgpu_buffer_rsrc_t r_ret;
  [[maybe_unused]] const auto r_pk = col_rsrc(p.pk, IO != kIoCols ? col * (uint32_t)(3 * A + 1) : 0u);
  if constexpr (IN_PK) {
    t = col_ld(r_pk, off, (uint32_t)pk_col_t(A) * col);
    r_ret = col_rsrc(p.ep_ret, cols);
#pragma unroll
    for (int a = 0; a < A; ++a) {
      const uint32_t cw = (uint32_t)col_ld(r_pk, off, (uint32_t)pk_col_cell(A, a) * col);
      s[a].x = (int32_t)pk_x(cw);
      s[a].y = (int32_t)pk_y(cw);
      s[a].q = (int32_t)pk_q(cw);
      s[a].f = (uint32_t)col_ld(r_pk, off, (uint32_t)pk_col_flags(A, a) * col);
      s[a].ret = __int_as_float(col_ld(r_pk, off, (uint32_t)pk_col_ret(A, a) * col));
      s[a].act = col_ld(r_act, off, a * col);
      s0[a] = s[a];
    }
  } else if constexpr (!PRE) {
    r_ret = col_rsrc(p.ep_ret, cols);
#pragma unroll
    for (int a = 0; a < A; ++a) {
      s[a].x = col_ld(r_x, off, a * col);
      s[a].y = col_ld(r_y, off, a * col);
      s[a].q = col_ld(r_q, off, a * col);
      s[a].f = (uint32_t)col_ld(r_f, off, a * col);
      s[a].ret = __int_as_float(col_ld(r_ret, off, a * col));
      s[a].act = HASHED ? hash_action(p.seed, p.t_global, p.n_global, p.env_offset + e, A, a) : col_ld(r_act, off, a * col);
      s0[a] = s[a];
    }
  } else {
#pragma unroll
    for (int a = 0; a < A; ++a) {
      s[a].x = col_ld(r_x, off, a * col);
      s[a].y = col_ld(r_y, off, a * col);
      s[a].q = col_ld(r_q, off, a * col);
      s[a].f = (uint32_t)col_ld(r_f, off, a * col);
      s[a].act = HASHED ? hash_action(p.seed, p.t_global, p.n_global, p.env_offset + e, A, a) : col_ld(r_act, off, a * col);
      if constexpr (KIND == RMX_FROZEN_LAKE) __builtin_amdgcn_sched_barrier(0);
    }
    __builtin_amdgcn_sched_barrier(0);
    r_ret = col_rsrc(p.ep_ret, cols);
#pragma unroll
    for (int a = 0; a < A; ++a) {
      s[a].ret = __int_as_float(col_ld(r_ret, off, a * col));
      s0[a] = s[a];
    }
  }
  Pcg rng = {0ull, 0ull, 0ull, 0ull};
  int32_t episode = 0;
  constexpr bool FIXED = RNG && (SLIP & kRngFixedSeed) != 0;
  constexpr bool FCELLS = FIXED && RSTART;
  constexpr bool RNG_LATE = FIXED && !DRAW;
  if constexpr (RNG && !RNG_LATE) {
    rng = ld_pcg(p.rng, N, e);
    episode = col_ld(col_rsrc(p.episode, (uint32_t)N * 4u), off, 0);
  }
  uint32_t fcw[FCELLS ? (A + 1) / 2 : 1] = {};
  Pcg frng = {0ull, 0ull, 0ull, 0ull};
  if constexpr (FIXED) {
    if constexpr (FCELLS) {
      const auto r_fc = col_rsrc(p.rs_cells, col * (uint32_t)((A + 1) / 2));
#pragma unroll
      for (int w = 0; w < (A + 1) / 2; ++w) fcw[w] = (uint32_t)col_ld(r_fc, off, (uint32_t)w * col);
    }
    if constexpr (RNG_LATE) episode = col_ld(col_rsrc(p.episode, (uint32_t)N * 4u), off, 0);
    if constexpr (DRAW) {
      if (p.rs_dirty) {
        frng = ld_pcg(p.rs_rng, N, e);
      } else {
        const auto r = col_rsrc(p.rs_rng, (uint32_t)N * 16u);
        const auto w0 = __builtin_amdgcn_raw_buffer_load_b64(r, (uint32_t)e * 8u, 0, 0);
        const auto w1 = __builtin_amdgcn_raw_buffer_load_b64(r, (uint32_t)e * 8u, (uint32_t)N * 8u, 0);
        frng.hi = ((uint64_t)w0[1] << 32) | w0[0];
        frng.lo = ((uint64_t)w1[1] << 32) | w1[0];
      }
    }
  }
  RsNext nx = {{0ull, 0ull, 0ull, 0ull}, 0, -1, 0, false};
  if constexpr (RSTART && !FIXED) {
    const auto r_nx = col_rsrc(p.nx_rng, (uint32_t)N * 32u);
    const uint32_t o8 = (uint32_t)e * 8u, c8 = (uint32_t)N * 8u;
    const auto w0 = __builtin_amdgcn_raw_buffer_load_b64(r_nx, o8, 0, 0);
    const auto w1 = __builtin_amdgcn_raw_buffer_load_b64(r_nx, o8, c8, 0);
    const auto w2 = __builtin_amdgcn_raw_buffer_load_b64(r_nx, o8, 2u * c8, 0);
    const auto w3 = __builtin_amdgcn_raw_buffer_load_b64(r_nx, o8, 3u * c8, 0);
    nx.g = {((uint64_t)w0[1] << 32) | w0[0], ((uint64_t)w1[1] << 32) | w1[0], ((uint64_t)w2[1] << 32) | w2[0],
            ((uint64_t)w3[1] << 32) | w3[0]};
    nx.i = col_ld(col_rsrc(p.nx_idx, (uint32_t)N * 4u), off, 0);
    nx.k = col_ld(col_rsrc(p.nx_ep, (uint32_t)N * 4u), off, 0);
    nx.i0 = nx.i;
  }
  SlabSlot slot = {{0.0, 0.0, 0.0, 0.0}};
  if (p.wave_stats) slot = slab_prefetch(p.slab);
  ReportIn rin;
  if constexpr (RPT) rin = report_prefetch(p, e, live);
  const auto mg = col_rsrc(p.merged, MERGED ? (uint32_t)p.merged_bytes : 0u);
  const auto mg4 = col_rsrc(p.merged4, M4 ? (uint32_t)p.merged4_bytes : 0u);
#ifdef RMX_DIAG
  const int diag = p.diag;
  STAMP(1);
  STAMP(2);
#endif
  const auto tb = make_tables<true>(lds, p);

#ifdef RMX_DIAG
  if (diag & 8192) {
    if (live) {
      st(r_t, off, 0, t + 1);
      if (p.env_done) byte_st<SAUX>(p, (uint32_t)e, (uint32_t)t & 1u);
#pragma unroll
      for (int a = 0; a < A; ++a) {
        st(r_x, off, a * col, s[a].x + s[a].act);
        st(r_y, off, a * col, s[a].y);
        st(r_q, off, a * col, s[a].q);
        st(r_f, off, a * col, (int32_t)s[a].f);
        st(r_ret, off, a * col, __float_as_int(s[a].ret));
        st(r_rew, off, a * col, s[a].act);
      }
    }
    return;
  }
#endif
  const bool rs = p.autoreset && (s[0].f & RMX_F_ENV_DONE);
  t = rs ? 0 : t;
  const int32_t t1 = t + 1;
  constexpr bool LATE_DISC = KIND == RMX_OFFICE_WORLD && A == 1;
  float disc = LATE_DISC ? 1.0f : (p.gamma_is_one ? 1.0f : p.disc[min((uint32_t)t, (uint32_t)p.max_t + 1u)]);
  uint32_t bad = 0, all_term = 1u, all_trunc = 1u;
  int32_t sx[A], sy[A];
#pragma unroll
  for (int a = 0; a < A; ++a) sx[a] = p.start_x[a], sy[a] = p.start_y[a];
  if constexpr (RNG) {
    if constexpr (FIXED) {
      if (rs) {
        if constexpr (FCELLS) fixed_start_cells<A>(fcw, sx, sy);
        episode += 1;
        if constexpr (DRAW) {
          rng.hi = frng.hi;
          rng.lo = frng.lo;
          if (p.rs_dirty) {
            rng.ihi = frng.ihi;
            rng.ilo = frng.ilo;
          }
        }
      }
    } else if constexpr (RSTART)
      rs_step<A>(p, rng, episode, nx, rs, live, p.env_offset + e,
                 reinterpret_cast<unsigned char*>(p.start_ws) + (size_t)e * (size_t)(2 * shuffle_stride(p.n_free)), lds,
                 (uint32_t)tid, sx, sy);
    else
      random_start_reset<A, false>(p, rng, episode, rs, live, p.env_offset + e, lds, (uint32_t)tid, 0u, sx, sy);
  }
  AgentTmp k[A];
  uint32_t m[A];
  uint32_t prev_cell[A];
  uint2 qe[A][QXB > 0 ? QXB : 1];
  constexpr bool OW_SLIP = DRAW && KIND == RMX_OFFICE_WORLD;
  uint32_t blocked[OW_SLIP ? A : 1] = {};
  if constexpr (OW_SLIP) {
    static_assert(MERGED, "OfficeWorld slip: 16-B or 4-B merged records");
    uint32_t wi[A];
#pragma unroll
    for (int a = 0; a < A; ++a) {
      s[a].x = rs ? sx[a] : s[a].x;
      s[a].y = rs ? sy[a] : s[a].y;
      s[a].q = rs ? p.init_q[a] : s[a].q;
      s[a].f = rs ? RMX_F_ACTIVE : s[a].f;
      s[a].ret = rs ? 0.0f : s[a].ret;
      const uint32_t mi = move_index<KIND>(s[a], (uint32_t)p.final_q[a], 0u, p, bad, k[a]);
      const uint32_t idx = (uint32_t)p.mg_base[a] + __umul24(__umul24((uint32_t)s[a].q, (uint32_t)p.HW), 5u) + mi;
      wi[a] = M4 ? __builtin_amdgcn_raw_buffer_load_b32(mg4, idx * 4u, 0, 0)
                 : __builtin_amdgcn_raw_buffer_load_b32(mg, idx * 16u, 0, 0);
    }
#pragma unroll
    for (int a = 0; a < A; ++a) {
      const uint32_t ac = agent_action<KIND>(s[a], (uint32_t)p.final_q[a], bad, k[a]);
      blocked[a] = (ac < (uint32_t)RMX_WAIT && (wi[a] & kMvWall)) ? 1u : 0u;
      s[a].act = (int32_t)(blocked[a] ? (uint32_t)RMX_WAIT
                                      : (ac < (uint32_t)RMX_WAIT ? (uint32_t)slip_choice(p, (int32_t)ac, rng) : ac));
    }
  }
  uint4 r[A];
  AgentRes o[A];
#pragma unroll
  for (int a = 0; a < A; ++a) {
    s[a].x = rs ? sx[a] : s[a].x;
    s[a].y = rs ? sy[a] : s[a].y;
    s[a].q = rs ? p.init_q[a] : s[a].q;
    s[a].f = rs ? RMX_F_ACTIVE : s[a].f;
    s[a].ret = rs ? 0.0f : s[a].ret;
    if constexpr (DRAW && KIND == RMX_FROZEN_LAKE) {
      if ((s[a].f & RMX_F_ACTIVE) && (uint32_t)s[a].q != (uint32_t)p.final_q[a]) {
        if (s[a].act == RMX_WAIT)
          bad |= 1u;
        else if ((uint32_t)s[a].act < (uint32_t)RMX_WAIT)
          s[a].act = slip_choice(p, s[a].act, rng);
      }
    }
#ifdef RMX_DIAG
    if (a == 0) STAMP(3);
    if (diag & 4096) {
      const uint32_t mi = move_index<KIND>(s[a], (uint32_t)p.final_q[a], (uint32_t)p.mv_base[a], p, bad, k[a]);
      m[a] = (mi & 0x00030303u);
      continue;
    }
#endif
    if constexpr (MERGED) {
      const uint32_t ac = agent_action<KIND>(s[a], (uint32_t)p.final_q[a], bad, k[a]);
      constexpr uint32_t RB = M4 ? 4u : 16u;
      const uint32_t hw5 = ((uint32_t)p.HW * (5u * RB)) & 0xFFFFFFu, w5 = ((uint32_t)p.W * (5u * RB)) & 0xFFFFFFu;
      const uint32_t ro = ((uint32_t)s[a].q & 0xFFu) * hw5 + ((uint32_t)s[a].y & 0xFFu) * w5 +
                          ((uint32_t)s[a].x & 0xFFu) * (5u * RB) + (ac + (uint32_t)p.mg_base[a]) * RB;
      if constexpr (M4) {
        r[a] = make_uint4(__builtin_amdgcn_raw_buffer_load_b32(mg4, ro, 0, 0), 0u, 0u, 0u);
      } else {
        const auto v = __builtin_amdgcn_raw_buffer_load_b128(mg, ro, 0, 0);
        r[a] = make_uint4(v[0], v[1], v[2], v[3]);
      }
    } else {
      if constexpr (QRM) prev_cell[a] = (uint32_t)(s[a].y * p.W + s[a].x);
      m[a] = tb.mv(move_index<KIND>(s[a], (uint32_t)p.final_q[a], (uint32_t)p.mv_base[a], p, bad, k[a]));
    }
  }
  if constexpr (RNG_LATE) {
    if (rs && live && p.rs_dirty) rng = ld_pcg(p.rs_rng, N, e);
  }
  if (LATE_DISC && !p.gamma_is_one) {
    __builtin_amdgcn_sched_barrier(0);
    disc = p.disc[min((uint32_t)t, (uint32_t)p.max_t + 1u)];
  }
#pragma unroll
  for (int a = 0; a < A; ++a) {
#ifdef RMX_DIAG
    if (a == 0) STAMP(4);
    if (diag & 4096) {
      const uint32_t ti = rm_index(s[a], m[a], (uint32_t)p.rm_base[a], p, k[a]);
      r[a] = make_uint4(ti & 3u, 0u, 0u, 0u);
      continue;
    }
#endif
    if constexpr (M4) {
      const int32_t pb = __builtin_amdgcn_readfirstlane((int)p.mg_palb[a]);
      r[a].y = __float_as_uint((float)(int32_t)__builtin_amdgcn_sbfe(pb, (r[a].x >> 25) & 0x18u, 8u));
    }
    if constexpr (OW_SLIP) {
      const uint32_t hz = __builtin_amdgcn_ubfe(r[a].x, 25, 1);
      const uint32_t fl = (blocked[a] & (uint32_t)p.wall_fail) | (hz & (uint32_t)p.hazard_fail);
      r[a].x = (r[a].x & ~(kMvWall | kMvFail)) | (blocked[a] << 24) | (fl << 26);
    }
    if constexpr (MERGED) {
      const uint32_t w0 = r[a].x;
      k[a].mm = k[a].moving ? w0 : 0u;
      s[a].x = (int32_t)(w0 & 0xFFu);
      s[a].y = (int32_t)__builtin_amdgcn_ubfe(w0, 8, 8);
      r[a].x = __builtin_amdgcn_ubfe(w0, 16, 8) | (__builtin_amdgcn_ubfe(w0, 27, 1) << 8);
      continue;
    }
    const uint32_t ti = rm_index(s[a], m[a], (uint32_t)p.rm_base[a], p, k[a]);
    if constexpr (QRM) {
      const uint32_t ev = __builtin_amdgcn_ubfe(m[a], 16, 8);
#pragma unroll
      for (int j = 0; j < QXB; ++j) {
        qe[a][j] = make_uint2(0u, 0u);
        if (j < p.n_qrm[a]) {
          const uint4 v = tb.rm((uint32_t)p.rm_base[a] + (uint32_t)p.qrm_q[a][j] * (uint32_t)p.E + ev);
          qe[a][j] = make_uint2(v.x, v.w);
        }
      }
    }
    r[a] = tb.rm(ti);
  }
  STAMP(5);
#pragma unroll
  for (int a = 0; a < A; ++a) {
    o[a] = finish<KIND>(s[a], k[a], r[a], t1, disc, p);
    all_term &= o[a].term;
    all_trunc &= o[a].trunc;
  }
  const uint32_t done = (all_term | all_trunc) & (live ? 1u : 0u);
#ifdef RMX_DIAG
  if (p.stamps) {
    asm volatile("" ::"v"(done), "v"(s[0].f), "v"(s[A - 1].f), "v"(o[0].reward), "v"(o[A - 1].reward));
  }
#endif
  auto flush_stats = [&]() {
    if (p.wave_stats) {
      LaneStats ls = {0.0, (int)done, 0, done ? t1 : 0};
      double rsum = 0.0;
#pragma unroll
      for (int a = 0; a < A; ++a) {
        rsum += (double)s[a].ret;
        ls.successes += done ? (int)o[a].succ : 0;
      }
      ls.ret = done ? rsum : 0.0;
      wave_flush_slot(p.slab, slot, ls, __any(done));
    } else if (done) {
      double rs = 0.0;
      uint32_t sc = 0;
#pragma unroll
      for (int a = 0; a < A; ++a) {
        rs += (double)s[a].ret;
        sc += o[a].succ;
      }
      env_stats_env(p, e, t1);
      env_stats_ret(p, e, rs, sc);
    }
  };
  if constexpr (STATS_FIRST) flush_stats();
  STAMP(6);
  if constexpr (OUT_PK) {
    if (live) {
      st(r_pk, off, (uint32_t)pk_col_t(A) * col, t1);
#pragma unroll
      for (int a = 0; a < A; ++a) {
        const uint32_t f1 = s[a].f | (done ? RMX_F_ENV_DONE : 0u);
        st(r_pk, off, (uint32_t)pk_col_cell(A, a) * col, (int32_t)pk_cell((uint32_t)s[a].x, (uint32_t)s[a].y, (uint32_t)s[a].q));
        st(r_pk, off, (uint32_t)pk_col_flags(A, a) * col, (int32_t)f1);
        if (IO == kIoColsToPk || __float_as_int(s[a].ret) != __float_as_int(s0[a].ret))
          st(r_pk, off, (uint32_t)pk_col_ret(A, a) * col, __float_as_int(s[a].ret));
      }
    } else {
      bad = 0;
    }
  } else if (live) {
    constexpr bool ALL = SKIP == kSkipNone || IO == kIoPkToCols;
    st(r_t, off, 0, t1);
    if (p.env_done) byte_st<SAUX>(p, (uint32_t)e, done);
#pragma unroll
    for (int a = 0; a < A; ++a) {
      const uint32_t f1 = s[a].f | (done ? RMX_F_ENV_DONE : 0u);
      st(r_x, off, a * col, s[a].x);
      st(r_y, off, a * col, s[a].y);
      if (ALL || s[a].q != s0[a].q) st(r_q, off, a * col, s[a].q);
      st(r_f, off, a * col, (int32_t)f1);
      if (ALL || __float_as_int(s[a].ret) != __float_as_int(s0[a].ret))
        st(r_ret, off, a * col, __float_as_int(s[a].ret));
      st(r_rew, off, a * col, __float_as_int(o[a].reward));
    }
    if (p.shaping) {
      const auto r = col_rsrc(p.shaping, cols);
#pragma unroll
      for (int a = 0; a < A; ++a) st(r, off, a * col, __float_as_int(o[a].shaping));
    }
    if (p.renv) {
      const auto r = col_rsrc(p.renv, cols);
#pragma unroll
      for (int a = 0; a < A; ++a) st(r, off, a * col, __float_as_int(o[a].renv));
    }
    if (p.enc_state) {
      const auto r = col_rsrc(p.enc_state, cols);
#pragma unroll
      for (int a = 0; a < A; ++a) st(r, off, a * col, (s[a].y * p.W + s[a].x) * p.enc_nq[a] + s[a].q);
    }
    if constexpr (RNG) {
      const auto r_rng = col_rsrc(p.rng, (uint32_t)N * 32u);
      const uint32_t o8 = (uint32_t)e * 8u, c8 = (uint32_t)N * 8u;
      typedef uint32_t u32x2 __attribute__((ext_vector_type(2)));
      if (DRAW || (rs && (!FIXED || p.rs_dirty))) {
        __builtin_amdgcn_raw_buffer_store_b64(u32x2{(uint32_t)rng.hi, (uint32_t)(rng.hi >> 32)}, r_rng, o8, 0, SAUX);
        __builtin_amdgcn_raw_buffer_store_b64(u32x2{(uint32_t)rng.lo, (uint32_t)(rng.lo >> 32)}, r_rng, o8, c8, SAUX);
      }
      if (rs && FIXED && !p.rs_dirty) {
        st(col_rsrc(p.episode, (uint32_t)N * 4u), off, 0, episode);
      } else if (rs) {
        __builtin_amdgcn_raw_buffer_store_b64(u32x2{(uint32_t)rng.ihi, (uint32_t)(rng.ihi >> 32)}, r_rng, o8, 2u * c8,
                                              SAUX);
        __builtin_amdgcn_raw_buffer_store_b64(u32x2{(uint32_t)rng.ilo, (uint32_t)(rng.ilo >> 32)}, r_rng, o8, 3u * c8,
                                              SAUX);
        st(col_rsrc(p.episode, (uint32_t)N * 4u), off, 0, episode);
      }
      if constexpr (RSTART && !FIXED) {
        const auto r_nx = col_rsrc(p.nx_rng, (uint32_t)N * 32u);
        if (nx.fresh || nx.i != nx.i0) {
          __builtin_amdgcn_raw_buffer_store_b64(u32x2{(uint32_t)nx.g.hi, (uint32_t)(nx.g.hi >> 32)}, r_nx, o8, 0, SAUX);
          __builtin_amdgcn_raw_buffer_store_b64(u32x2{(uint32_t)nx.g.lo, (uint32_t)(nx.g.lo >> 32)}, r_nx, o8, c8, SAUX);
          st(col_rsrc(p.nx_idx, (uint32_t)N * 4u), off, 0, nx.i);
        }
        if (nx.fresh) {
          __builtin_amdgcn_raw_buffer_store_b64(u32x2{(uint32_t)nx.g.ihi, (uint32_t)(nx.g.ihi >> 32)}, r_nx, o8, 2u * c8,
                                                SAUX);
          __builtin_amdgcn_raw_buffer_store_b64(u32x2{(uint32_t)nx.g.ilo, (uint32_t)(nx.g.ilo >> 32)}, r_nx, o8, 3u * c8,
                                                SAUX);
          st(col_rsrc(p.nx_ep, (uint32_t)N * 4u), off, 0, nx.k);
        }
      }
    }
  } else {
    bad = 0;
  }
#ifdef RMX_DIAG
  if (QRM && (p.diag & 131072)) {
    uint32_t keep = 0;
#pragma unroll
    for (int a = 0; a < A; ++a)
#pragma unroll
      for (int j = 0; j < (QXB > 0 ? QXB : 1); ++j) keep ^= qe[a][j].x ^ qe[a][j].y;
    if (keep == 0x7fffffffu) atomicOr(p.err, 2u);
  } else
#endif
  if constexpr (QRM) {
    const int32_t Qx = p.n_qrm_max;
    const uint32_t nq_col = (uint32_t)Qx * (uint32_t)A * (uint32_t)N;
    const auto r_s = col_rsrc(p.qrm_s, nq_col * 4u), r_sn = col_rsrc(p.qrm_sn, nq_col * 4u);
    const auto r_rq = col_rsrc(p.qrm_rq, nq_col * 4u), r_dn = col_rsrc(p.qrm_done, nq_col);
#pragma unroll
    for (int a = 0; a < A; ++a) {
      const uint32_t nQ = (uint32_t)p.enc_nq[a];
      const uint32_t new_cell = (uint32_t)(s[a].y * p.W + s[a].x);
      const uint32_t env_term = (s[a].f >> 4) & 1u;
#pragma unroll
      for (int j = 0; j < QXB; ++j) {
        if (j >= Qx) continue;
        const bool valid = j < p.n_qrm[a];
        const uint32_t so = (uint32_t)(a * Qx + j) * (uint32_t)N;
        const int32_t s_enc = valid ? (int32_t)(prev_cell[a] * nQ + p.qrm_q[a][j]) : -1;
        const int32_t sn_enc = valid ? (int32_t)(new_cell * nQ + (qe[a][j].x & 0xFFu)) : -1;
        const uint32_t dn = valid ? (env_term | ((qe[a][j].x >> 8) & 1u)) : 0u;
        if (live) {
          st(r_s, off, so * 4u, s_enc);
          st(r_sn, off, so * 4u, sn_enc);
          st(r_rq, off, so * 4u, valid ? (int32_t)qe[a][j].y : 0);
          __builtin_amdgcn_raw_buffer_store_b8((uint8_t)dn, r_dn, (uint32_t)e, so, kStoreAux);
        }
      }
    }
  }
  if (__any(bad)) {
    if ((tid & 63) == 0) atomicOr(p.err, 1u);
  }
#ifdef RMX_DIAG
  STAMP(7);
  if (!(diag & 1)) {
#endif
  if constexpr (!STATS_FIRST) flush_stats();
#ifdef RMX_DIAG
  }
  STAMP(8);
  if (p.stamps && (tid & 63) == 0) {
    unsigned long long* w = p.stamps + (((size_t)blockIdx.x * blockDim.x + tid) >> 6) * (2 * kStamps);
#pragma unroll
    for (int i = 0; i < kStamps; ++i) {
      w[i] = st_clk[i];
      w[kStamps + i] = st_rt[i];
    }
  }
#endif
  if constexpr (RPT) {
    double rs = 0.0;
    uint32_t sc = 0;
#pragma unroll
    for (int a = 0; a < A; ++a) {
      rs += (double)s[a].ret;
      sc += o[a].succ;
    }
    report_tail(p, rin, done, rs, sc, t1);
  }
```

### multiagent-rl-rm_amd/csrc/rmx_handle.h

```cpp
#pragma once
#include <hip/hip_runtime.h>

#include <chrono>
#include <string>
#include <vector>

#include "rmx_host.h"
#include "rmx_hoststep.h"
#include "rmx_internal.h"

struct rmx_handle {
  rmx_config cfg;
  rmx::HostEngine* host = nullptr;
  struct Seq {
    std::vector<rmx::StepLaunch> window;
    rmx::FastParams base;
    const int32_t* actions = nullptr;
    const double* out = nullptr;
    int64_t stride = 0;
    int32_t k = 0;
    int autoreset = -1;
    uint64_t key = 0;
    bool queue_off = false;
    bool packed_off = false;
    bool pk_failed = false;
    bool pk_refused = false;
    uint32_t* d_pk = nullptr;
    bool is_packed = false;
    int dispatch = RMX_SEQ_NONE;
    int64_t recordings = 0;
  } seq;
  int device = 0;
  int block = 256;
  int step_layout = rmx::kLayoutThreadPerEnv;
  int rollout_layout = rmx::kLayoutLanePerAgent;
  void* d_tables = nullptr;
  size_t tables_bytes = 0;
  int32_t off_cell = 0, off_ev = 0, off_nq = 0, off_rr = 0, off_sh = 0, off_qrm = 0;
  int32_t n_qrm[RMX_MAX_AGENTS]{}, enc_nq[RMX_MAX_AGENTS]{};
  float* d_disc = nullptr;
  double* d_slab = nullptr;
  int64_t n_waves = 0;
  double* d_stats = nullptr;
  uint32_t* d_err = nullptr;
  rmx_buffers buf{};
  bool bound = false;
  uint64_t base_seed = 123;
  uint64_t digest = 0;
  int32_t diag = 0;
  unsigned long long* d_stamps = nullptr;
  int32_t init_q[RMX_MAX_AGENTS]{}, final_q[RMX_MAX_AGENTS]{}, start_x[RMX_MAX_AGENTS]{}, start_y[RMX_MAX_AGENTS]{};
  bool fast = false;
  int fast_wave_stats = 0;
  int fast_skip = 0;
  int generic_skip = 0;
  int fast_block = 256;
  int rollout_lds = 1;
  int fast_tables = rmx::kTblGlobal;
  void* d_fast = nullptr;
  void* d_merged = nullptr;
  size_t merged_bytes = 0;
  int merged_sections = 0;
  unsigned char* d_es = nullptr;
  size_t es_bytes = 0;
  double* es_ret = nullptr;
  unsigned long long* es_cnt = nullptr;
  uint32_t* es_succ = nullptr;
  double* rpt_partial = nullptr;
  unsigned int* rpt_ticket = nullptr;
  int32_t fast_n16 = 0, fast_off_rm = 0, fast_off_info = 0;
  uint8_t fast_qrm_q[RMX_MAX_AGENTS][rmx::kFastMaxQrm]{};
  int32_t mg_base[RMX_MAX_AGENTS]{};
  size_t merged4_off = 0, merged4_bytes = 0;
  uint32_t mg_palb[RMX_MAX_AGENTS]{};
  int32_t n_free = 0;
  uint16_t* d_free = nullptr;
  uint16_t* d_start_ws = nullptr;
  unsigned char* d_nx = nullptr;
  bool seed_fixed = false;
  unsigned char* d_rsc = nullptr;
  bool rs_stale = false;
  bool rs_dirty = true;
  struct Sync {
    unsigned char* mb = nullptr;
    size_t bytes = 0;
    rmx::SyncIO io{};
    hipStream_t stream = nullptr;
    hipEvent_t done = nullptr, dep = nullptr;
    bool running = false;
    bool pending = false;
    void* caller = nullptr;
    uint32_t seq = 0;
    uint32_t served = 0;
    int oneshot = 0;
    uint64_t idle_ticks = 0, life_ticks = 0;
    bool enc = false;
#ifdef RMX_DIAG
    std::chrono::steady_clock::time_point t_post;
    double wait_ns = 0;
#endif
  } sync;
  struct Learn {
    rmx::LearnParams params{};
    bool on = false;
    double* d_phi = nullptr;
    uint64_t* rng = nullptr;
    rmx::LambdaParams lam{};
    bool lam_on = false;
    rmx::EpsParams eps{};
  } learn;
};

namespace rmx {
namespace capi {

constexpr size_t kFastMergedDefaultBytes = 128 * 1024;
constexpr int64_t kFastWaveStatsMinEnvs = 1 << 20;
constexpr int64_t kFastSkipMinEnvs = 1 << 20;
constexpr int64_t kFastNtMinInstances = int64_t(1) << 23;

inline thread_local std::string g_err;

inline int fail(int code, const std::string& msg) {
  g_err = msg;
  return code;
}

inline int hip_fail(hipError_t e, const char* what) {
  return fail(RMX_E_HIP, std::string(what) + ": " + hipGetErrorString(e));
}

#define HIP_TRY(expr, what)            \
  do {                                 \
    hipError_t _e = (expr);            \
    if (_e != hipSuccess) return rmx::capi::hip_fail(_e, what); \
  } while (0)

inline hipStream_t as_stream(void* s) { return reinterpret_cast<hipStream_t>(s); }

inline int check_bound(const rmx_handle* h) {
  if (!h) return fail(RMX_E_INVALID, "handle is NULL");
  if (!h->bound) return fail(RMX_E_STATE, "buffers not bound (rmx_bind)");
  return RMX_OK;
}

inline int64_t threads_for(const rmx_handle* h, int layout) {
  return layout == rmx::kLayoutLanePerAgent ? h->cfg.n_envs * rmx::lanes_per_env(h->cfg.n_agents) : h->cfg.n_envs;
}

inline dim3 grid_for(const rmx_handle* h, int layout) {
  return dim3((unsigned)((threads_for(h, layout) + h->block - 1) / h->block));
}

inline size_t nx_jump_offset(int64_t n_envs) { return (40 * (size_t)n_envs + 255) & ~(size_t)255; }

rmx::KParams base_params(const rmx_handle* h);
rmx::FastParams fast_params(const rmx_handle* h);
bool fast_applies(const rmx_handle* h);
hipError_t reduce_stats(const rmx_handle* h, double* out, hipStream_t st);
hipError_t refresh_starts(rmx_handle* h, hipStream_t st);
int starts_current(rmx_handle* h, void* stream);
rmx::FastParams step_fp(const rmx_handle* h, const int32_t* actions, uint64_t seed, int64_t t_global, int autoreset);
int do_step(rmx_handle* h, const int32_t* actions, int hashed, uint64_t seed, int64_t t_global, int autoreset,
            void* stream);
bool report_fuses(const rmx_handle* h);
rmx::FastParams report_fp(const rmx_handle* h, const int32_t* actions, int autoreset, double* stats_out);

int lambda_clear(rmx_handle* h, const uint8_t* env_mask_dev, void* stream);

int sync_end(rmx_handle* h);

#define SYNC_END_OR_RETURN(h)   \
  do {                          \
    const int _rc = rmx::capi::sync_end(h); \
    if (_rc) return _rc;        \
  } while (0)

}
}
```

### multiagent-rl-rm_amd/csrc/rmx_internal.h

```cpp
#pragma once
#include <hip/hip_runtime.h>
#include <stdint.h>

#include <cmath>
#include <string>

#include "../../include/rmx.h"
#include "rmx_layout.h"
#include "rmx_learn.h"
#include "rmx_rules.h"

namespace rmx {

__host__ __device__ constexpr int32_t shuffle_stride(int32_t n) { return (n + 7) & ~7; }
__host__ __device__ constexpr int32_t rs_wave_lds(int32_t n) { return 256 * ((n + 3) >> 2) + 512; }
constexpr int kRsWaveLds = 512 + 8 * 64 * (16 + 8);
constexpr int kRsRowMax = 192;
constexpr int kRngSlip = 1, kRngStarts = 2, kRngFixedSeed = 4;
inline size_t start_cache_rng_off(int A, int64_t N) { return (4 * (size_t)((A + 1) / 2) * (size_t)N + 255) & ~(size_t)255; }
inline size_t start_cache_bytes(int A, int64_t N) { return start_cache_rng_off(A, N) + 32 * (size_t)N; }

template <typename P>
inline void slip_fill(P& p, const rmx_config& c) {
  bool uniform = true;
  p.slip_pack = 0;
  for (int i = 0; i < 4; ++i) {
    p.slip_n[i] = c.slip_n[i];
    uniform = uniform && c.slip_n[i] == c.slip_n[0];
    for (int j = 0; j < 4; ++j) {
      p.slip_out[i][j] = c.slip_out[i][j];
      p.slip_thr[i][j] = slip_threshold(c.slip_cdf[i][j]);
      uniform = uniform && (j >= 3 || p.slip_thr[i][j] == slip_threshold(c.slip_cdf[0][j])) &&
                (uint32_t)c.slip_out[i][j] <= 7u;
      p.slip_pack |= (uint64_t)((uint32_t)c.slip_out[i][j] & 7u) << (3 * (4 * i + j));
    }
  }
  p.slip_uniform = uniform ? 1 : 0;
}

struct KParams {
  const uint4* tables;
  int32_t tables_n16;
  int32_t off_cell, off_ev, off_nq, off_rr, off_sh, off_qrm;
  int32_t W, HW, A, Q, E, max_t;
  int64_t N;
  float hazard_penalty, wall_penalty;
  int32_t hazard_fail, wall_fail, has_shaping, gamma_is_one;
  float reward_modifier;
  int32_t n_qrm_max;
  int32_t stochastic;
  int32_t slip_n[4], slip_out[4][4];
  uint64_t slip_thr[4][4];
  int32_t slip_uniform;
  uint64_t slip_pack;
  uint64_t seed_scale, seed_env_stride, seed_episode_stride, base_seed;
  uint64_t* rng;
  int32_t* episode;
  int32_t rng_on, random_starts, n_free;
  const uint16_t* free_cells;
  uint16_t* start_ws;
  int32_t* enc_state;
  int32_t n_qrm[RMX_MAX_AGENTS], enc_nq[RMX_MAX_AGENTS];
  int32_t init_q[RMX_MAX_AGENTS], final_q[RMX_MAX_AGENTS], start_x[RMX_MAX_AGENTS], start_y[RMX_MAX_AGENTS];
  const float* disc;
  int32_t* pos_x;
  int32_t* pos_y;
  int32_t* rm_q;
  uint32_t* flags;
  float* ep_ret;
  int32_t* t;
  float* reward;
  float* shaping;
  uint8_t* env_done;
  float* renv;
  int32_t* qrm_s;
  int32_t* qrm_sn;
  float* qrm_rq;
  uint8_t* qrm_done;
  const int32_t* actions;
  uint64_t seed;
  int64_t t_global, env_offset, n_global;
  int32_t autoreset;
  double* slab;
  int32_t diag;
  uint32_t* err;
  int32_t skip_same;
  uint32_t* rs_cells;
  uint64_t* rs_rng;
};


struct FastParams {
  const uint4* tables;
  int32_t n16, off_rm, off_info;
  int32_t pad6;
  const uint4* merged;
  int32_t merged_bytes;
  int32_t mg_base[kFastMaxAgents];
  int32_t pad0;
  const uint32_t* merged4;
  int32_t merged4_bytes;
  uint32_t mg_palb[kFastMaxAgents];
  int32_t HW;
  int32_t* qrm_s;
  int32_t* qrm_sn;
  float* qrm_rq;
  uint8_t* qrm_done;
  int32_t n_qrm_max;
  int32_t n_qrm[kFastMaxAgents], enc_nq[kFastMaxAgents];
  uint8_t qrm_q[kFastMaxAgents][kFastMaxQrm];
  int32_t W, H, E, max_t, N, A;
  int32_t hazard_fail, wall_fail;
  int32_t mv_base[kFastMaxAgents];
  int32_t rm_base[kFastMaxAgents];
  int32_t final_q[kFastMaxAgents], init_q[kFastMaxAgents], start_x[kFastMaxAgents], start_y[kFastMaxAgents];
  float hazard_penalty, wall_penalty;
  int32_t has_shaping, gamma_is_one, autoreset;
  int32_t tbl_mode;
  int32_t skip_same;
  int32_t block;
  int32_t pad1;
  const float* disc;
  int32_t* pos_x;
  int32_t* pos_y;
  int32_t* rm_q;
  uint32_t* flags;
  float* ep_ret;
  int32_t* t;
  float* reward;
  float* shaping;
  uint8_t* env_done;
  float* renv;
  int32_t* enc_state;
  const int32_t* actions;
  uint64_t seed;
  int64_t t_global, env_offset, n_global;
  int32_t wave_stats;
  int32_t pad2;
  double* slab;
  double* es_ret;
  unsigned long long* es_cnt;
  uint32_t* es_succ;
  uint32_t* err;
  int32_t diag;
  int32_t pad3;
  unsigned long long* stamps;
  double* rpt_out;
  double* rpt_partial;
  unsigned int* rpt_ticket;
  int32_t rpt_cs, rpt_n_slab;
  int32_t slip_n[4], slip_out[4][4];
  uint64_t slip_thr[4][4];
  int32_t slip_uniform;
  int32_t pad4;
  uint64_t slip_pack;
  uint64_t seed_scale, seed_env_stride, seed_episode_stride, base_seed;
  uint64_t* rng;
  int32_t* episode;
  int32_t slip;
  int32_t n_free;
  const uint16_t* free_cells;
  uint16_t* start_ws;
  uint64_t* nx_rng;
  int32_t* nx_idx;
  int32_t* nx_ep;
  const uint4* rs_jump;
  const uint32_t* rs_cells;
  const uint64_t* rs_rng;
  int32_t rs_dirty;
  int32_t pad5;
  uint32_t* pk;
  int32_t pk_io;
  int32_t pad7;
};
#define RMX_FAST_PARAMS_FIELDS(X) X(tables) X(n16) X(off_rm) X(off_info) X(pad6) X(merged) \
   X(merged_bytes) X(mg_base) X(pad0) X(merged4) X(merged4_bytes) X(mg_palb) X(HW) X(qrm_s) X(qrm_sn) X(qrm_rq) \
   X(qrm_done) X(n_qrm_max) X(n_qrm) X(enc_nq) X(qrm_q) X(W) X(H) X(E) X(max_t) X(N) X(A) X(hazard_fail) \
   X(wall_fail) X(mv_base) X(rm_base) X(final_q) X(init_q) X(start_x) X(start_y) X(hazard_penalty) X(wall_penalty) \
   X(has_shaping) X(gamma_is_one) X(autoreset) X(tbl_mode) X(skip_same) X(block) X(pad1) X(disc) X(pos_x) X(pos_y) \
   X(rm_q) X(flags) X(ep_ret) X(t) X(reward) X(shaping) X(env_done) X(renv) X(enc_state) X(actions) X(seed) \
   X(t_global) X(env_offset) X(n_global) X(wave_stats) X(pad2) X(slab) X(es_ret) X(es_cnt) X(es_succ) X(err) X(diag) \
   X(pad3) X(stamps) X(rpt_out) X(rpt_partial) X(rpt_ticket) X(rpt_cs) X(rpt_n_slab) X(slip_n) X(slip_out) \
   X(slip_thr) X(slip_uniform) X(pad4) X(slip_pack) X(seed_scale) X(seed_env_stride) X(seed_episode_stride) \
   X(base_seed) X(rng) X(episode) X(slip) X(n_free) X(free_cells) X(start_ws) X(nx_rng) X(nx_idx) X(nx_ep) \
   X(rs_jump) X(rs_cells) X(rs_rng) X(rs_dirty) X(pad5) X(pk) X(pk_io) X(pad7)
#define RMX_FP_FIELD_BYTES(f) +sizeof(FastParams::f)
constexpr size_t kFastParamsFieldBytes = 0 RMX_FAST_PARAMS_FIELDS(RMX_FP_FIELD_BYTES);
#undef RMX_FP_FIELD_BYTES
static_assert(kFastParamsFieldBytes == sizeof(FastParams), "FastParams has implicit padding or an unlisted field");
constexpr int kStamps = 9;

hipError_t launch_step_fast(const FastParams& p, int hashed, int kind, hipStream_t st);

struct StepArgs {
  int32_t N, blk;
  const int32_t *pos_x, *pos_y, *rm_q;
  const uint32_t* flags;
  const int32_t* t;
  const int32_t* actions;
  FastParams p;
};
static_assert(sizeof(StepArgs) == 56 + sizeof(FastParams), "step_fast_kernel's parameter list: no padding");
struct StepLaunch {
  char symbol[160];
  uint32_t grid, block, lds;
  StepArgs args;
};
struct StepCapture {
  StepLaunch* out;
  bool ok;
};
extern thread_local StepCapture* tl_capture;
constexpr int kQueueStream = 1;
constexpr int kQueueUnused = RMX_QUEUE_UNUSED, kQueueReady = RMX_QUEUE_READY, kQueueUnavailable = RMX_QUEUE_UNAVAILABLE,
              kQueueRetired = RMX_QUEUE_RETIRED;
int queue_run(int device, const StepLaunch* L, int K, uint64_t key, std::string* err);
void queue_note_stream(int device);
struct QueueInfo {
  int64_t windows, uploads, packets, stream_windows;
  int state;
};
void queue_info(int device, QueueInfo* out);
void queue_set_timing(int device, int every);
int64_t queue_times(int device, uint64_t* out, int64_t cap);
int code_object_check(const void* co, size_t bytes, int64_t* n_step, int64_t* n_refused, std::string* first);
hipError_t launch_rollout_fast(const FastParams& p, int kind, int32_t T, float* trace, hipStream_t st);

constexpr uint32_t kSyncStep = 1, kSyncReset = 2, kSyncExit = 3;
constexpr int kSyncInlineActs = 15;
constexpr uint32_t kSyncInline = 1u << 3, kSyncAutoreset = 1u << 2, kSyncBadAct = 15u;
struct alignas(128) SyncReq {
  uint32_t seq;
  uint32_t ctl;
  uint32_t acts;
  uint32_t seq_echo;
  uint64_t seed;
};
struct alignas(128) SyncAck {
  uint32_t seq;
  uint32_t bad;
  uint64_t t_seen, t_done;
};
struct SyncCols {
  uint4* rec;
  uint4* envrec;
  int32_t* qrm_s;
  int32_t* qrm_sn;
  float* qrm_rq;
  uint8_t* qrm_done;
};
struct SyncIO {
  SyncReq* req;
  SyncAck* ack;
  const int32_t* act;
  SyncCols out;
  uint32_t seq0;
  uint32_t pad;
  uint64_t idle_ticks;
  uint64_t life_ticks;
};
hipError_t launch_resident(const KParams& p, const SyncIO& io, int kind, int threads, size_t lds, hipStream_t st);

inline int amax_bucket(int A) { return A <= 4 ? A : 8; }
inline int lanes_per_env(int A) { return A <= 1 ? 1 : A <= 2 ? 2 : A <= 4 ? 4 : 8; }
constexpr int kLayoutThreadPerEnv = 0;
constexpr int kLayoutLanePerAgent = 1;

hipError_t launch_step(const KParams& p, int hashed, int kind, int layout, dim3 g, dim3 b, size_t lds,
                       hipStream_t st);
hipError_t launch_rollout(const KParams& p, int kind, int layout, int32_t T, float* trace, dim3 g, dim3 b,
                          size_t lds, hipStream_t st);
hipError_t launch_reset(const KParams& p, const uint8_t* mask, int write_state, hipStream_t st);
hipError_t launch_fill_actions(uint64_t seed, int64_t t0, int32_t T, int64_t n_global, int64_t env_offset, int64_t N,
                               int A, int32_t* out, hipStream_t st);
hipError_t launch_mdp(const KParams& p, int kind, int ag, int fix_fl, int64_t S, int32_t* next, float* reward,
                      uint8_t* done, size_t lds, hipStream_t st);
hipError_t launch_learn_step(const KParams& p, const LearnParams& lp, const LearnCall& lc, const LambdaParams* lam,
                             const EpsParams* eps, int kind, size_t lds, hipStream_t st);
hipError_t launch_learn_run(const KParams& p, const LearnParams& lp, const LearnCall& lc, const LambdaParams* lam,
                            const EpsParams* eps, int32_t T, int kind, size_t lds, hipStream_t st);
hipError_t launch_learn_step_eps(const KParams& p, const LearnParams& lp, const LearnCall& lc, const LambdaParams* lam,
                                 const EpsParams* eps, int kind, size_t lds, hipStream_t st);
hipError_t launch_learn_run_eps(const KParams& p, const LearnParams& lp, const LearnCall& lc, const LambdaParams* lam,
                                const EpsParams* eps, int32_t T, int kind, size_t lds, hipStream_t st);
hipError_t launch_traces_clear(int32_t* cnt, const uint8_t* mask, int A, int64_t N, hipStream_t st);
hipError_t launch_eps_decay(const EpsParams& ep, const uint8_t* mask, int A, int64_t N, hipStream_t st);
constexpr int kStatsPartials = 512;
constexpr int kStatsEnvsPerThread = 4;
hipError_t launch_stats_reduce(const double* slab, int64_t n_waves, const double* es_ret, const unsigned long long* es_cnt,
                               const uint32_t* es_succ, int64_t N, double* partial, unsigned int* ticket,
                               double* out, hipStream_t st);

}
```

### multiagent-rl-rm_amd/csrc/rmx_tables.cpp

```cpp
#include "rmx_host.h"

#include <string.h>

#include <algorithm>

namespace rmx {

namespace {

size_t align16(size_t x) { return (x + 15) & ~size_t(15); }

}

std::string validate_config(const rmx_config& cr) {
  const rmx_config* c = &cr;
  if (c->kind != RMX_FROZEN_LAKE && c->kind != RMX_OFFICE_WORLD) return "unknown env kind";
  if (c->width <= 0 || c->height <= 0 || (int64_t)c->width * c->height > RMX_MAX_CELLS) return "grid size out of range";
  if (c->n_agents < 1 || c->n_agents > RMX_MAX_AGENTS) return "n_agents must be 1..8";
  if (c->n_rm_states < 1 || c->n_rm_states > RMX_MAX_RM_STATES) return "n_rm_states out of range";
  if (c->n_events < 1 || c->n_events > RMX_MAX_EVENTS) return "n_events out of range";
  if (c->n_envs < 1 || c->n_envs > (int64_t)1 << 31) return "n_envs out of range";
  if (c->env_offset < 0 || c->n_envs_global < c->env_offset + c->n_envs) return "env_offset / n_envs_global inconsistent";
  if (c->max_t < 0 || c->max_t > 60000) return "max_t out of range";
  if (!c->cell || !c->cell_event || !c->next_q || !c->rm_reward || !c->init_q || !c->final_q || !c->start_xy)
    return "a required table pointer is NULL";
  if (c->has_shaping && !c->shape) return "has_shaping set but shape is NULL";
  if (c->n_qrm_max < 0 || c->n_qrm_max > c->n_rm_states) return "n_qrm_max out of range";
  if (c->stochastic) {
    for (int i = 0; i < 4; ++i) {
      if (c->slip_n[i] < 1 || c->slip_n[i] > 4) return "slip_n must be 1..4";
      for (int j = 0; j < c->slip_n[i]; ++j) {
        if (c->slip_out[i][j] < 0 || c->slip_out[i][j] > RMX_WAIT) return "slip_out id out of range";
        if (j > 0 && !(c->slip_cdf[i][j] >= c->slip_cdf[i][j - 1])) return "slip_cdf not monotone";
      }
    }
  }
  if (c->n_qrm_max > 0 && (!c->n_qrm || !c->qrm_states || !c->enc_nq)) return "n_qrm_max > 0 but a QRM table is NULL";
  const int A = c->n_agents, Q = c->n_rm_states, E = c->n_events, HW = c->width * c->height;
  for (int a = 0; a < A; ++a) {
    const int sx = c->start_xy[2 * a], sy = c->start_xy[2 * a + 1];
    if (sx < 0 || sx >= c->width || sy < 0 || sy >= c->height) return "start cell outside grid";
    if (c->init_q[a] < 0 || c->init_q[a] >= Q) return "init_q out of range";
    if (c->final_q[a] < -1 || c->final_q[a] >= Q) return "final_q out of range";
    for (int i = 0; i < HW; ++i)
      if (c->cell_event[(size_t)a * HW + i] >= E) return "cell_event id >= n_events";
    for (int i = 0; i < Q * E; ++i)
      if (c->next_q[(size_t)a * Q * E + i] >= Q) return "next_q entry >= n_rm_states";
    if (c->enc_nq && (c->enc_nq[a] < 1 || c->enc_nq[a] > Q)) return "enc_nq must be in 1..n_rm_states";
    if (c->n_qrm_max > 0) {
      if (c->n_qrm[a] < 0 || c->n_qrm[a] > c->n_qrm_max) return "n_qrm out of range";
      for (int j = 0; j < c->n_qrm[a]; ++j)
        if (c->qrm_states[(size_t)a * c->n_qrm_max + j] >= Q) return "qrm_states entry >= n_rm_states";
    }
  }
  const int up = c->kind == RMX_FROZEN_LAKE ? -1 : 1;
  const int dx[4] = {0, 0, -1, 1}, dy[4] = {up, -up, 0, 0};
  for (int y = 0; y < c->height; ++y)
    for (int x = 0; x < c->width; ++x)
      for (int k = 0; k < 4; ++k)
        if ((c->cell[y * c->width + x] >> k) & 1u) {
          const int nx = x + dx[k], ny = y + dy[k];
          if (nx < 0 || nx >= c->width || ny < 0 || ny >= c->height) return "cell tile allows a move off the grid";
        }
  if (c->random_starts) {
    if (c->kind != RMX_FROZEN_LAKE) return "random_starts is a FrozenLake option (ma_frozen_lake.py:37-39)";
    if ((int64_t)free_cells(cr).size() < A) return "Not enough free cells to place all agents.";
  }
  return std::string();
}

uint64_t config_digest(const rmx_config& c) {
  uint64_t h = 0xcbf29ce484222325ull;
  auto mix = [&](const void* p, size_t n) {
    const unsigned char* b = static_cast<const unsigned char*>(p);
    for (size_t i = 0; i < n; ++i) h = (h ^ b[i]) * 0x100000001b3ull;
  };
  auto mixv = [&](auto v) { mix(&v, sizeof(v)); };
  const size_t A = (size_t)c.n_agents, Q = (size_t)c.n_rm_states, E = (size_t)c.n_events;
  const size_t HW = (size_t)c.width * (size_t)c.height;
  mixv(c.kind), mixv(c.width), mixv(c.height), mixv(c.n_agents), mixv(c.n_rm_states), mixv(c.n_events);
  mixv(c.max_t), mixv(c.hazard_penalty), mixv(c.wall_penalty), mixv(c.hazard_fail), mixv(c.wall_fail);
  mixv(c.gamma), mixv(c.has_shaping), mixv(c.reward_modifier), mixv(c.stochastic), mixv(c.random_starts);
  if (c.stochastic) mix(c.slip_n, sizeof(c.slip_n)), mix(c.slip_out, sizeof(c.slip_out)), mix(c.slip_cdf, sizeof(c.slip_cdf));
  mixv(c.seed_scale), mixv(c.seed_env_stride), mixv(c.seed_episode_stride);
  mix(c.cell, 2 * HW), mix(c.cell_event, A * HW), mix(c.next_q, A * Q * E), mix(c.rm_reward, 4 * A * Q * E);
  if (c.has_shaping) mix(c.shape, 4 * A * Q * E);
  mix(c.init_q, 4 * A), mix(c.final_q, 4 * A);
  if (!c.random_starts) mix(c.start_xy, 8 * A);
  return h;
}

bool build_table_blob(const rmx_config& c, std::vector<unsigned char>& blob, BlobOffsets& o) {
  const int A = c.n_agents, Q = c.n_rm_states, E = c.n_events, HW = c.width * c.height;
  size_t off = 0;
  o.cell = (int32_t)off;
  off = align16(off + sizeof(uint16_t) * HW);
  o.ev = (int32_t)off;
  off = align16(off + (size_t)A * HW);
  o.nq = (int32_t)off;
  off = align16(off + (size_t)A * Q * E);
  o.rr = (int32_t)off;
  off = align16(off + sizeof(float) * A * Q * E);
  o.sh = (int32_t)off;
  if (c.has_shaping) off = align16(off + sizeof(float) * A * Q * E);
  o.qrm = (int32_t)off;
  if (c.n_qrm_max > 0) off = align16(off + (size_t)A * c.n_qrm_max);
  if (off > 64 * 1024) return false;
  blob.assign(off, 0);
  memcpy(blob.data() + o.cell, c.cell, sizeof(uint16_t) * HW);
  memcpy(blob.data() + o.ev, c.cell_event, (size_t)A * HW);
  memcpy(blob.data() + o.nq, c.next_q, (size_t)A * Q * E);
  memcpy(blob.data() + o.rr, c.rm_reward, sizeof(float) * A * Q * E);
  if (c.has_shaping) memcpy(blob.data() + o.sh, c.shape, sizeof(float) * A * Q * E);
  if (c.n_qrm_max > 0) memcpy(blob.data() + o.qrm, c.qrm_states, (size_t)A * c.n_qrm_max);
  return true;
}

std::vector<float> discount_table(const rmx_config& c) {
  std::vector<float> disc((size_t)c.max_t + 2);
  double g = 1.0;
  for (size_t i = 0; i < disc.size(); ++i) {
    disc[i] = (float)g;
    g *= (double)c.gamma;
  }
  return disc;
}

bool build_fast_blob(const rmx_config& c, std::vector<unsigned char>& blob, FastLayout& L) {
  const int A = c.n_agents, Q = c.n_rm_states, E = c.n_events, W = c.width, H = c.height, HW = W * H;
  if (A > kFastMaxAgents || W > 255 || H > 255 || E > 255 || Q > 255)
    return false;
  if ((int64_t)A * c.n_envs >= ((int64_t)1 << 30)) return false;
  const size_t mv_bytes = align16(sizeof(uint32_t) * (size_t)A * HW * 5);
  const size_t rm_bytes = 16 * (size_t)A * Q * E;
  const size_t info_bytes = 16 * (size_t)A;
  const size_t total = mv_bytes + rm_bytes + info_bytes;
  if (total + 4 * 128 + 4 * 3 * 64 > kFastBlobMaxBytes) return false;
  blob.assign(total, 0);
  L.off_rm = (int32_t)mv_bytes;
  L.off_info = (int32_t)(mv_bytes + rm_bytes);
  uint32_t* info = reinterpret_cast<uint32_t*>(blob.data() + L.off_info);
  for (int a = 0; a < A; ++a) {
    const uint32_t fqb = c.final_q[a] < 0 ? 255u : (uint32_t)c.final_q[a];
    info[4 * a + 0] = (uint32_t)(a * HW * 5);
    info[4 * a + 1] = (uint32_t)(a * Q * E);
    info[4 * a + 2] = (uint32_t)c.start_xy[2 * a] | ((uint32_t)c.start_xy[2 * a + 1] << 8) |
                      ((uint32_t)c.init_q[a] << 16) | (fqb << 24);
    info[4 * a + 3] = c.enc_nq ? (uint32_t)c.enc_nq[a] : 0u;
  }
  const int up = c.kind == RMX_FROZEN_LAKE ? -1 : 1;
  const int dx[4] = {0, 0, -1, 1}, dy[4] = {up, -up, 0, 0};
  uint32_t* mv = reinterpret_cast<uint32_t*>(blob.data());
  for (int a = 0; a < A; ++a)
    for (int y = 0; y < H; ++y)
      for (int x = 0; x < W; ++x)
        for (int ac = 0; ac <= RMX_WAIT; ++ac) {
          const int cix = y * W + x;
          const bool can = ac < RMX_WAIT && ((c.cell[cix] >> ac) & 1u);
          const bool wall = c.kind == RMX_OFFICE_WORLD && ac < RMX_WAIT && !can;
          const int nx = can ? x + dx[ac] : x, ny = can ? y + dy[ac] : y;
          const int nc = ny * W + nx;
          const bool haz = (c.cell[nc] & RMX_CELL_HAZARD) != 0;
          const bool failing = c.kind == RMX_FROZEN_LAKE ? haz : ((wall && c.wall_fail) || (haz && c.hazard_fail));
          const uint32_t ev = c.cell_event[(size_t)a * HW + nc];
          mv[((size_t)a * HW + cix) * 5 + ac] = (uint32_t)nx | ((uint32_t)ny << 8) | (ev << 16) | (wall ? kMvWall : 0u) |
                                                (haz ? kMvHazard : 0u) | (failing ? kMvFail : 0u);
        }
  uint32_t* rm = reinterpret_cast<uint32_t*>(blob.data() + L.off_rm);
  for (int a = 0; a < A; ++a)
    for (int i = 0; i < Q * E; ++i) {
      const size_t ti = (size_t)a * Q * E + i;
      const uint32_t nq = c.next_q[ti];
      const float mrq = c.reward_modifier * c.rm_reward[ti];
      const float shp = c.has_shaping ? c.shape[ti] : 0.0f;
      rm[4 * ti] = nq | ((int32_t)nq == c.final_q[a] ? (1u << 8) : 0u);
      memcpy(&rm[4 * ti + 1], &mrq, sizeof(float));
      memcpy(&rm[4 * ti + 2], &shp, sizeof(float));
      memcpy(&rm[4 * ti + 3], &c.rm_reward[ti], sizeof(float));
    }
  return true;
}

bool build_merged(const rmx_config& c, const std::vector<unsigned char>& blob, int32_t off_rm, int32_t* mg_base,
                  std::vector<uint32_t>& out) {
  const int A = c.n_agents, Q = c.n_rm_states, E = c.n_events, HW = c.width * c.height;
  const size_t sec = (size_t)Q * HW * 5;
  if (sec * 16 > kMergedMaxBytes) return false;
  const uint32_t* mv = reinterpret_cast<const uint32_t*>(blob.data());
  const uint32_t* rm = reinterpret_cast<const uint32_t*>(blob.data() + off_rm);
  out.clear();
  std::vector<uint32_t> s(sec * 4);
  for (int a = 0; a < A; ++a) {
    std::fill(s.begin(), s.end(), 0u);
    for (int q = 0; q < Q; ++q)
      for (int cix = 0; cix < HW; ++cix)
        for (int ac = 0; ac <= RMX_WAIT; ++ac) {
          const uint32_t m = mv[((size_t)a * HW + cix) * 5 + ac];
          const uint32_t ev = (m >> 16) & 0xFFu;
          const uint32_t* r = rm + 4 * (((size_t)a * Q + q) * E + ev);
          const size_t o = 4 * (((size_t)q * HW + cix) * 5 + ac);
          s[o] = (m & 0x0700FFFFu) | ((r[0] & 0xFFu) << 16) | (((r[0] >> 8) & 1u) << 27);
          s[o + 1] = r[1];
          s[o + 2] = r[2];
        }
    int same = -1;
    for (size_t b = 0; b < out.size() / (sec * 4) && same < 0; ++b)
      if (std::equal(s.begin(), s.end(), out.begin() + b * sec * 4)) same = (int)b;
    if (same < 0) {
      same = (int)(out.size() / (sec * 4));
      if ((out.size() + s.size()) * 4 > kMergedMaxBytes) return false;
      out.insert(out.end(), s.begin(), s.end());
    }
    mg_base[a] = (int32_t)(same * sec);
  }
  return true;
}

bool build_compact(const rmx_config& c, const int32_t* mg_base, const std::vector<uint32_t>& merged, uint32_t* mg_palb,
                   std::vector<uint32_t>& out) {
  if (c.has_shaping) return false;
  const size_t sec = (size_t)c.n_rm_states * c.width * c.height * 5;
  const size_t n = merged.size() / 4;
  out.assign(n, 0u);
  for (size_t b = 0; b * sec < n; ++b) {
    std::vector<uint32_t> pal;
    for (size_t i = b * sec; i < (b + 1) * sec; ++i) {
      const uint32_t w0 = merged[4 * i], rw = merged[4 * i + 1];
      if (w0 >> 28) return false;
      size_t k = std::find(pal.begin(), pal.end(), rw) - pal.begin();
      if (k == pal.size()) {
        if (pal.size() == 4) return false;
        pal.push_back(rw);
      }
      out[i] = w0 | ((uint32_t)k << 28);
    }
    uint32_t packed = 0;
    for (int k = 0; k < (int)pal.size(); ++k) {
      float v;
      memcpy(&v, &pal[k], 4);
      if (!(v >= -128.0f && v <= 127.0f && v == (float)(int)v) || (v == 0.0f && (pal[k] >> 31))) return false;
      packed |= (uint32_t)(uint8_t)(int8_t)(int)v << (8 * k);
    }
    for (int a = 0; a < c.n_agents; ++a)
      if ((size_t)mg_base[a] == b * sec) mg_palb[a] = packed;
  }
  return true;
}

std::vector<uint16_t> free_cells(const rmx_config& c) {
  std::vector<uint16_t> out;
  for (int x = 0; x < c.width; ++x)
    for (int y = 0; y < c.height; ++y)
      if (!(c.cell[y * c.width + x] & RMX_CELL_HAZARD)) out.push_back((uint16_t)(y * c.width + x));
  return out;
}

}
```

### multiagent-rl-rm_amd/rmx/_capi.py

```python
from __future__ import annotations

import ctypes as C
import importlib.util
import os

from .tables import CompiledTables

LIB_NAME = "librmx.so"
LIB_PATH = os.path.join(os.path.dirname(os.path.abspath(__file__)), LIB_NAME)

RMX_OK, RMX_E_INVALID, RMX_E_HIP, RMX_E_ACTION, RMX_E_STATE, RMX_E_TRACE = 0, -1, -2, -3, -4, -5
F_ACTIVE, F_FAIL, F_TERM, F_TRUNC, F_ENV_TERM, F_RM_TERM, F_ENV_DONE = 0x01, 0x02, 0x04, 0x08, 0x10, 0x20, 0x40
F_STEPS_SHIFT = 16
NSTATS = 4
STAT_SUM_RETURN, STAT_EPISODES, STAT_SUCCESSES, STAT_SUM_LENGTH = 0, 1, 2, 3

EXPORTS = (
    "rmx_abi_version", "rmx_last_error", "rmx_build_info", "rmx_create", "rmx_destroy", "rmx_bind", "rmx_reset",
    "rmx_step", "rmx_step_hashed", "rmx_fill_actions", "rmx_rollout", "rmx_stats_device", "rmx_stats_host",
    "rmx_stats_clear", "rmx_check_errors", "rmx_mdp_states", "rmx_mdp", "rmx_step_variant", "rmx_state_bytes",
    "rmx_get_state", "rmx_set_state", "rmx_step_report", "rmx_step_report_fused", "rmx_reset_sync", "rmx_step_sync",
    "rmx_step_sync_begin", "rmx_sync_wait", "rmx_sync_end", "rmx_step_seq", "rmx_queue_counters", "rmx_queue_info",
    "rmx_code_object_check", "rmx_device_count", "rmx_queue_timing", "rmx_queue_times", "rmx_step_info",
    "rmx_seq_packed", "rmx_learn_states", "rmx_learn_bind", "rmx_learn_step", "rmx_learn_step_policy",
    "rmx_learn_rng_bind", "rmx_learn_rng_seed", "rmx_learn_lambda_slots", "rmx_learn_lambda_bind",
    "rmx_learn_traces_clear", "rmx_learn_run", "rmx_learn_eps_bind", "rmx_learn_eps_decay",
)
LEARN_UPDATE, LEARN_BEST, LEARN_NUMPY = 1, 2, 4
LEARN_DYN_FIXED, LEARN_DYN_ENV = 0, 1
LEARN_RUN_MAX = 4096
SYNC_MAX_ENVS = 256
QUEUE_INFO_N = 7
QUEUE_STATES = ("unused", "ready", "unavailable", "retired")
SEQ_DISPATCH = ("none", "queue", "stream:kernel", "stream:disabled", "stream:queue", "host")
VARIANT_GENERIC, VARIANT_LANE_PER_AGENT, VARIANT_FAST, VARIANT_FAST_LANE_PER_AGENT, VARIANT_HOST = 0, 1, 2, 3, 4
STEP_INFO_N = 14
STEP_INFO_FIELDS = ("variant", "tables", "record_bytes", "merged_sections", "merged_bytes", "merged4_bytes",
                    "fast_blob_bytes", "generic_blob_bytes", "store_mode", "wave_stats", "block", "qrm_fast",
                    "seed_fixed", "rollout_layout")
VARIANT_NAMES = ("generic", "lane_per_agent", "fast", "fast_lpe", "host")
TABLE_MODES = ("none", "global", "merged", "merged4")
LAYOUTS = ("thread_per_env", "lane_per_agent")
DEVICE_HOST = -1


ABI_VERSION = 12

CSRC = os.path.join(os.path.dirname(os.path.dirname(os.path.abspath(__file__))), "csrc")
HASHED_SOURCES = ("rmx_kernels.hip", "rmx_fast.hip", "rmx_fast_step.inc", "rmx_sync.hip", "rmx_capi.cpp",
                  "rmx_queue.cpp", "rmx_tables.cpp",
                  "rmx_handle.h", "rmx_capi_create.cpp", "rmx_capi_sync.cpp", "rmx_capi_seq.cpp", "rmx_capi_learn.cpp", "rmx_capi_state.cpp",
                  "rmx_comd.cpp", "rmx_build_info.cpp", "rmx_internal.h", "rmx_layout.h", "rmx_host.h", "rmx_device.h",
                  "rmx_generic.h", "rmx_comd.h", "rmx_hoststep.cpp", "rmx_hoststep.h", "rmx_learn.hip", "rmx_learn_run.hip", "rmx_learn.h",
                  "rmx_rules.h", "../../include/rmx.h",
                  "Makefile", "rmx_learn_eps.hip", "rmx_learn_run_eps.hip")


def source_hash(csrc: str = CSRC) -> str:
    import hashlib

    h = hashlib.sha256()
    for f in HASHED_SOURCES:
        with open(os.path.join(csrc, f), "rb") as fh:
            h.update(fh.read())
    return h.hexdigest()[:16]


def build_info(lib=None) -> dict:
    lib = lib or load_library(check_source=False)
    return dict(kv.split("=", 1) for kv in lib.rmx_build_info().decode().split())


class RmxConfig(C.Structure):
    _fields_ = [
        ("kind", C.c_int32), ("width", C.c_int32), ("height", C.c_int32), ("n_agents", C.c_int32),
        ("n_rm_states", C.c_int32), ("n_events", C.c_int32), ("max_t", C.c_int32), ("device", C.c_int32),
        ("n_envs", C.c_int64), ("env_offset", C.c_int64), ("n_envs_global", C.c_int64),
        ("hazard_penalty", C.c_float), ("wall_penalty", C.c_float), ("hazard_fail", C.c_int32),
        ("wall_fail", C.c_int32), ("gamma", C.c_float), ("has_shaping", C.c_int32),
        ("reward_modifier", C.c_float), ("n_qrm_max", C.c_int32),
        ("stochastic", C.c_int32), ("slip_n", C.c_int32 * 4), ("slip_out", (C.c_int32 * 4) * 4),
        ("slip_cdf", (C.c_double * 4) * 4), ("seed_scale", C.c_uint64), ("seed_env_stride", C.c_uint64),
        ("seed_episode_stride", C.c_uint64), ("random_starts", C.c_int32),
        ("cell", C.c_void_p), ("cell_event", C.c_void_p), ("next_q", C.c_void_p), ("rm_reward", C.c_void_p),
        ("shape", C.c_void_p), ("init_q", C.c_void_p), ("final_q", C.c_void_p), ("start_xy", C.c_void_p),
        ("n_qrm", C.c_void_p), ("qrm_states", C.c_void_p), ("enc_nq", C.c_void_p),
    ]


class RmxLearnConfig(C.Structure):
    _fields_ = [("gamma", C.c_double), ("learning_rate", C.c_double), ("use_qrm", C.c_int32), ("use_rsh", C.c_int32),
                ("trunc_is_terminal", C.c_int32), ("dynamics", C.c_int32), ("phi", C.c_void_p)]


class RmxBuffers(C.Structure):
    _fields_ = [(n, C.c_void_p) for n in
                ("pos_x", "pos_y", "rm_q", "flags", "ep_ret", "t", "reward", "shaping", "env_done", "renv",
                 "qrm_s", "qrm_sn", "qrm_rq", "qrm_done", "rng", "episode", "enc_state")]


def make_config(tab: CompiledTables, n_envs: int, env_offset: int = 0, n_envs_global: int = None,
                device: int = 0):
    import numpy as np

    arrays = {
        "cell": np.ascontiguousarray(tab.cell, np.uint16),
        "cell_event": np.ascontiguousarray(tab.cell_event, np.uint8),
        "next_q": np.ascontiguousarray(tab.next_q, np.uint8),
        "rm_reward": np.ascontiguousarray(tab.rm_reward, np.float32),
        "init_q": np.ascontiguousarray(tab.init_q, np.int32),
        "final_q": np.ascontiguousarray(tab.final_q, np.int32),
        "start_xy": np.ascontiguousarray(tab.start_xy, np.int32),
    }
    if tab.shape is not None:
        arrays["shape"] = np.ascontiguousarray(tab.shape, np.float32)
    if tab.n_qrm is not None:
        arrays["n_qrm"] = np.ascontiguousarray(tab.n_qrm, np.int32)
        arrays["qrm_states"] = np.ascontiguousarray(tab.qrm_states, np.uint8)
    if tab.enc_nq is not None:
        arrays["enc_nq"] = np.ascontiguousarray(tab.enc_nq, np.int32)
    cfg = RmxConfig()
    cfg.kind, cfg.width, cfg.height = tab.kind, tab.width, tab.height
    cfg.n_agents, cfg.n_rm_states, cfg.n_events = tab.n_agents, tab.n_rm_states, tab.n_events
    cfg.max_t, cfg.device = tab.max_t, device
    cfg.n_envs, cfg.env_offset = int(n_envs), int(env_offset)
    cfg.n_envs_global = int(n_envs if n_envs_global is None else n_envs_global)
    cfg.hazard_penalty, cfg.wall_penalty = tab.hazard_penalty, tab.wall_penalty
    cfg.hazard_fail, cfg.wall_fail, cfg.gamma = tab.hazard_fail, tab.wall_fail, tab.gamma
    cfg.has_shaping = int(tab.shape is not None)
    cfg.reward_modifier = float(tab.reward_modifier)
    cfg.n_qrm_max = int(tab.qrm_states.shape[1]) if tab.n_qrm is not None and int(tab.n_qrm.max()) > 0 else 0
    cfg.stochastic = int(tab.stochastic)
    if tab.stochastic:
        for i in range(4):
            cfg.slip_n[i] = int(tab.slip_n[i])
            for j in range(4):
                cfg.slip_out[i][j] = int(tab.slip_out[i, j])
                cfg.slip_cdf[i][j] = float(tab.slip_cdf[i, j])
    cfg.seed_scale, cfg.seed_env_stride, cfg.seed_episode_stride = (int(v) & (2**64 - 1) for v in tab.seed_schedule)
    cfg.random_starts = int(tab.random_starts)
    for k, v in arrays.items():
        setattr(cfg, k, v.ctypes.data)
    return cfg, arrays


_LIB = None
_RUNTIME = []


def torch_hip_runtime():
    spec = importlib.util.find_spec("torch")
    if spec is None or not spec.origin:
        return []
    d = os.path.join(os.path.dirname(spec.origin), "lib")
    return [os.path.join(d, n) for n in ("libhsa-runtime64.so", "libamdhip64.so") if os.path.exists(os.path.join(d, n))]


def load_library(path: str = None, check_source: bool = True):
    global _LIB
    if _LIB is not None:
        return _LIB
    path = path or os.environ.get("RMX_LIB") or LIB_PATH
    if not os.path.exists(path):
        raise RuntimeError(f"rmx HIP library not built: {path} is missing (run __graft_entry__.build())")
    for rt in torch_hip_runtime():
        try:
            _RUNTIME.append(C.CDLL(rt, mode=os.RTLD_NOW | os.RTLD_GLOBAL))
        except OSError:
            break
    lib = C.CDLL(path)
    vp, i32, i64, u64 = C.c_void_p, C.c_int32, C.c_int64, C.c_uint64
    sig = {
        "rmx_abi_version": (C.c_int, []),
        "rmx_device_count": (C.c_int, [C.POINTER(C.c_int32)]),
        "rmx_last_error": (C.c_char_p, []),
        "rmx_build_info": (C.c_char_p, []),
        "rmx_state_bytes": (C.c_int, [vp, C.POINTER(C.c_size_t)]),
        "rmx_get_state": (C.c_int, [vp, vp, C.c_size_t]),
        "rmx_set_state": (C.c_int, [vp, vp, C.c_size_t]),
        "rmx_create": (C.c_int, [C.POINTER(RmxConfig), C.POINTER(vp)]),
        "rmx_destroy": (None, [vp]),
        "rmx_bind": (C.c_int, [vp, C.POINTER(RmxBuffers)]),
        "rmx_reset": (C.c_int, [vp, vp, u64, vp]),
        "rmx_step": (C.c_int, [vp, vp, C.c_int, vp]),
        "rmx_step_hashed": (C.c_int, [vp, u64, i64, C.c_int, vp]),
        "rmx_fill_actions": (C.c_int, [vp, u64, i64, i32, vp, vp]),
        "rmx_rollout": (C.c_int, [vp, u64, i64, i32, vp, vp]),
        "rmx_stats_device": (C.c_int, [vp, vp, vp]),
        "rmx_stats_host": (C.c_int, [vp, C.POINTER(C.c_double)]),
        "rmx_stats_clear": (C.c_int, [vp, vp]),
        "rmx_check_errors": (C.c_int, [vp]),
        "rmx_step_variant": (C.c_int, [vp]),
        "rmx_step_report": (C.c_int, [vp, vp, C.c_int, vp, vp]),
        "rmx_step_report_fused": (C.c_int, [vp]),
        "rmx_seq_packed": (C.c_int, [vp]),
        "rmx_step_seq": (C.c_int, [vp, vp, C.c_int64, C.c_int32, C.c_int, vp, vp]),
        "rmx_queue_timing": (C.c_int, [vp, C.c_int]),
        "rmx_queue_times": (C.c_int, [vp, vp, C.c_int64, C.POINTER(C.c_int64)]),
        "rmx_queue_counters": (C.c_int, [vp, vp]),
        "rmx_queue_info": (C.c_int, [vp, vp, i32]),
        "rmx_step_info": (C.c_int, [vp, vp, i32]),
        "rmx_code_object_check": (C.c_int, [vp, C.c_size_t, C.POINTER(C.c_int64), C.POINTER(C.c_int64), C.c_char_p,
                                            C.c_size_t]),
        "rmx_mdp_states": (C.c_int, [vp, i32, C.POINTER(C.c_int64)]),
        "rmx_mdp": (C.c_int, [vp, i32, i32, vp, vp, vp, vp]),
        "rmx_reset_sync": (C.c_int, [vp, u64, C.POINTER(RmxBuffers), vp]),
        "rmx_step_sync": (C.c_int, [vp, vp, C.c_int, C.POINTER(RmxBuffers), vp]),
        "rmx_step_sync_begin": (C.c_int, [vp, vp, C.c_int, vp]),
        "rmx_sync_wait": (C.c_int, [vp, C.POINTER(RmxBuffers)]),
        "rmx_sync_end": (C.c_int, [vp]),
        "rmx_learn_states": (C.c_int, [vp, C.POINTER(C.c_int64)]),
        "rmx_learn_bind": (C.c_int, [vp, C.POINTER(RmxLearnConfig), vp, vp]),
        "rmx_learn_step": (C.c_int, [vp, vp, C.c_int, vp]),
        "rmx_learn_step_policy": (C.c_int, [vp, C.c_double, C.c_int, u64, i64, C.c_int, vp, vp]),
        "rmx_learn_run": (C.c_int, [vp, C.c_int32, C.c_double, C.c_int, u64, i64, vp, vp]),
        "rmx_learn_rng_bind": (C.c_int, [vp, vp]),
        "rmx_learn_rng_seed": (C.c_int, [vp, vp, vp]),
        "rmx_learn_lambda_slots": (C.c_int, [vp, C.POINTER(C.c_int32)]),
        "rmx_learn_lambda_bind": (C.c_int, [vp, C.c_double, i32, vp, vp, vp]),
        "rmx_learn_traces_clear": (C.c_int, [vp, vp, vp]),
        "rmx_learn_eps_bind": (C.c_int, [vp, vp, C.c_double, C.c_double]),
        "rmx_learn_eps_decay": (C.c_int, [vp, vp, vp]),
    }
    for name, (res, args) in sig.items():
        fn = getattr(lib, name)
        fn.restype, fn.argtypes = res, args
    if lib.rmx_abi_version() != ABI_VERSION:
        raise RuntimeError(f"{path}: ABI {lib.rmx_abi_version()}, these bindings need {ABI_VERSION} (rebuild)")
    if check_source and os.path.exists(os.path.join(CSRC, "Makefile")) and \
            os.path.abspath(path) == os.path.abspath(LIB_PATH):
        got, want = build_info(lib).get("src"), source_hash()
        if got != want:
            raise RuntimeError(f"{path} was built from other sources (src={got}, tree={want}): rebuild it "
                               "(__graft_entry__.build())")
    _LIB = lib
    return lib


def device_count(lib=None) -> int:
    lib = lib or load_library()
    n = C.c_int32()
    check(lib.rmx_device_count(C.byref(n)), "rmx_device_count")
    return n.value


def check(rc: int, what: str = "rmx"):
    if rc == RMX_OK:
        return
    msg = (_LIB.rmx_last_error() or b"").decode() if _LIB is not None else ""
    if rc in (RMX_E_INVALID, RMX_E_ACTION):
        raise ValueError(f"{what}: {msg} (rc={rc})")
    raise RuntimeError(f"{what}: {msg} (rc={rc})")
```

Baseline: 39.78 billion (env x agent)-steps/s.

## Add lean packed window form with precomputed per-agent transition table

Adds a "lean" packed state representation for queued multi-step windows. Each agent's position, RM state and flags are folded into one word that indexes a host-built table of next-row, flag and integer-reward entries. Middle steps run a slim kernel that does one table lookup per agent instead of the full merged-table step logic, and the first and last steps convert between the column layout and the lean form. This is meant to cut per-step memory traffic and ALU work. It adds table build and validation code, a fallback when capture fails, and only applies to deterministic runs with integer rewards and at least two agents.

Measured after the change: 40.43 billion (env x agent)-steps/s, median of 6. +1.6%, better.

```diff
diff --git a/include/rmx.h b/include/rmx.h
--- a/include/rmx.h
+++ b/include/rmx.h
@@ -152,6 +152,7 @@
 int rmx_step_seq(rmx_handle* h, const int32_t* actions_dev, int64_t action_stride, int32_t n_steps, int autoreset,
                  double* stats_out_dev, void* hip_stream);
 int rmx_seq_packed(const rmx_handle* h);
+int rmx_lean_check(const rmx_handle* h, int64_t* n_checked, int64_t* n_bad, char* report, size_t report_cap);
 int rmx_queue_counters(const rmx_handle* h, int64_t* out3);
 #define RMX_QUEUE_INFO_N 7
 #define RMX_QUEUE_UNUSED 0
diff --git a/multiagent-rl-rm_amd/csrc/rmx_capi.cpp b/multiagent-rl-rm_amd/csrc/rmx_capi.cpp
--- a/multiagent-rl-rm_amd/csrc/rmx_capi.cpp
+++ b/multiagent-rl-rm_amd/csrc/rmx_capi.cpp
@@ -167,6 +167,13 @@
   p.diag = h->diag;
   p.stamps = h->d_stamps;
   p.pk = h->seq.d_pk;
+  if (h->seq.d_ln) {
+    p.ln_tbl = h->seq.d_ln;
+    p.ln_bytes = (int32_t)(h->seq.ln.words.size() * 4);
+    p.ln_rows_off = h->seq.ln.rows_off;
+    std::memcpy(p.ln_base, h->seq.ln.base, sizeof(p.ln_base));
+    std::memcpy(p.ln_init, h->seq.ln.init, sizeof(p.ln_init));
+  }
   if (c.stochastic || c.random_starts) {
     p.slip = (c.stochastic ? rmx::kRngSlip : 0) | (c.random_starts ? rmx::kRngStarts : 0) |
              (h->seed_fixed ? rmx::kRngFixedSeed : 0);
@@ -335,6 +342,7 @@
   (void)hipFree(h->d_nx);
   (void)hipFree(h->d_rsc);
   (void)hipFree(h->seq.d_pk);
+  (void)hipFree(h->seq.d_ln);
   (void)hipFree(h->learn.d_phi);
   delete h;
 }
diff --git a/multiagent-rl-rm_amd/csrc/rmx_capi_create.cpp b/multiagent-rl-rm_amd/csrc/rmx_capi_create.cpp
--- a/multiagent-rl-rm_amd/csrc/rmx_capi_create.cpp
+++ b/multiagent-rl-rm_amd/csrc/rmx_capi_create.cpp
@@ -65,6 +65,7 @@
 static void create_env(rmx_handle* h, const rmx_config* cfg) {
   if (const char* qv = std::getenv("RMX_QUEUE")) h->seq.queue_off = std::strcmp(qv, "0") == 0;
   if (const char* pv = std::getenv("RMX_SEQ_PACKED")) h->seq.packed_off = std::strcmp(pv, "0") == 0;
+  if (const char* lv = std::getenv("RMX_SEQ_LEAN")) h->seq.lean_off = std::strcmp(lv, "0") == 0;
   if (const char* b = std::getenv("RMX_BLOCK")) {
     int v = std::atoi(b);
     if (v == 64 || v == 128 || v == 256) h->block = v;
@@ -152,6 +153,11 @@
       h->merged_sections = (int)(words16 / sec_words);
     }
     if (!merged_tab.empty()) h->merged_bytes = h->merged4_bytes ? h->merged4_off : merged_tab.size() * 4;
+    if (h->fast && h->fast_tables != rmx::kTblGlobal && !h->seq.lean_off && !h->seq.packed_off && !cfg->stochastic &&
+        !cfg->random_starts && cfg->n_agents >= 2) {
+      const rmx::TableView tv = {cfg->cell, cfg->cell_event, cfg->next_q, cfg->rm_reward, cfg->shape, cfg->qrm_states};
+      if (!rmx::build_lean_table(cfg->kind, rmx::lean_rules(*cfg), tv, h->seq.ln).empty()) h->seq.ln = rmx::LeanTable();
+    }
   }
   h->seed_fixed = h->fast && (cfg->stochastic || cfg->random_starts) && cfg->seed_episode_stride == 0;
   h->n_waves = std::max<int64_t>(gmax * (h->block / 64), (cfg->n_envs + 255) / 256 * 4);
diff --git a/multiagent-rl-rm_amd/csrc/rmx_capi_seq.cpp b/multiagent-rl-rm_amd/csrc/rmx_capi_seq.cpp
--- a/multiagent-rl-rm_amd/csrc/rmx_capi_seq.cpp
+++ b/multiagent-rl-rm_amd/csrc/rmx_capi_seq.cpp
@@ -26,20 +26,42 @@
   return true;
 }
 
+static bool seq_leans(const rmx_handle* h, int32_t K) {
+  return K >= 3 && h->cfg.n_agents >= 2 && !h->seq.lean_off && !h->seq.ln_failed && !h->seq.ln.words.empty();
+}
+
+static bool seq_lean_table(rmx_handle* h) {
+  if (h->seq.d_ln) return true;
+  const size_t bytes = h->seq.ln.words.size() * 4;
+  if (hipMalloc(&h->seq.d_ln, bytes) != hipSuccess ||
+      hipMemcpy(h->seq.d_ln, h->seq.ln.words.data(), bytes, hipMemcpyHostToDevice) != hipSuccess) {
+    (void)hipGetLastError();
+    (void)hipFree(h->seq.d_ln);
+    h->seq.d_ln = nullptr;
+    h->seq.ln_failed = true;
+    return false;
+  }
+  return true;
+}
+
 static bool record_seq(rmx_handle* h, const int32_t* actions, int64_t stride, int32_t K, int autoreset,
-                       double* stats_out, bool fused, bool packed) {
+                       double* stats_out, bool fused, bool packed, bool lean) {
   h->seq.window.resize((size_t)K);
   for (int32_t k = 0; k < K; ++k) {
     const int32_t* a = actions + (size_t)k * (size_t)stride;
     const bool rpt = fused && k == K - 1;
     rmx::FastParams fp = rpt ? report_fp(h, a, autoreset, stats_out) : step_fp(h, a, 0, 0, autoreset);
     if (packed) fp.pk_io = k == 0 ? rmx::kIoColsToPk : (k == K - 1 ? rmx::kIoPkToCols : rmx::kIoPkToPk);
+    if (lean) fp.pk_io = k == 0 ? rmx::kIoColsToLn : (k == K - 1 ? rmx::kIoLnToCols : rmx::kIoLnToLn);
     rmx::StepCapture cap{&h->seq.window[(size_t)k], false};
     rmx::tl_capture = &cap;
     (void)rmx::launch_step_fast(fp, 0, h->cfg.kind, nullptr);
     rmx::tl_capture = nullptr;
     if (!cap.ok) return false;
     if (packed && !std::strstr(h->seq.window[(size_t)k].symbol, "step_fast_kernel_win")) return false;
+    if (lean && !std::strstr(h->seq.window[(size_t)k].symbol, k == 0 || k == K - 1 ? "step_fast_kernel_win_ln"
+                                                                                   : "step_fast_kernel_win_lean"))
+      return false;
   }
   return true;
 }
@@ -79,13 +101,22 @@
     return on_stream(h->seq.queue_off && fast_applies(h) ? RMX_SEQ_STREAM_DISABLED : RMX_SEQ_STREAM_KERNEL);
   }
   const bool packed = n_steps >= 2 && seq_packs(h) && seq_pack_buffer(h);
+  const bool lean = packed && seq_leans(h, n_steps) && seq_lean_table(h);
   rmx::FastParams base = fast_params(h);
   const bool same = h->seq.key && h->seq.actions == actions_dev && h->seq.stride == action_stride &&
                     h->seq.k == n_steps && h->seq.autoreset == (autoreset ? 1 : 0) && h->seq.out == stats_out_dev &&
                     std::memcmp(&base, &h->seq.base, sizeof(base)) == 0;
   if (!same) {
     h->seq.key = 0;
-    h->seq.is_packed = packed && record_seq(h, actions_dev, action_stride, n_steps, autoreset, stats_out_dev, fused, true);
+    h->seq.is_lean = lean && record_seq(h, actions_dev, action_stride, n_steps, autoreset, stats_out_dev, fused, true, true);
+    if (lean && !h->seq.is_lean) {
+      h->seq.ln_failed = true;
+      (void)hipFree(h->seq.d_ln);
+      h->seq.d_ln = nullptr;
+      base = fast_params(h);
+    }
+    h->seq.is_packed = h->seq.is_lean || (packed && record_seq(h, actions_dev, action_stride, n_steps, autoreset,
+                                                               stats_out_dev, fused, true, false));
     if (packed && !h->seq.is_packed) {
       h->seq.pk_refused = true;
       (void)hipFree(h->seq.d_pk);
@@ -93,7 +124,7 @@
       base = fast_params(h);
     }
     if (!h->seq.is_packed &&
-        !record_seq(h, actions_dev, action_stride, n_steps, autoreset, stats_out_dev, fused, false)) {
+        !record_seq(h, actions_dev, action_stride, n_steps, autoreset, stats_out_dev, fused, false, false)) {
       rmx::queue_note_stream(h->device);
       return on_stream(RMX_SEQ_STREAM_KERNEL);
     }
@@ -139,7 +170,8 @@
 }
 
 int rmx_seq_packed(const rmx_handle* h) {
-  return h && !h->host && h->seq.dispatch == RMX_SEQ_QUEUE && h->seq.key && h->seq.is_packed ? 1 : 0;
+  if (!(h && !h->host && h->seq.dispatch == RMX_SEQ_QUEUE && h->seq.key && h->seq.is_packed)) return 0;
+  return h->seq.is_lean ? 2 : 1;
 }
 
 int rmx_queue_counters(const rmx_handle* h, int64_t* out3) {
@@ -173,6 +205,32 @@
   if (!h || !n || cap < 0 || (cap > 0 && !stamps)) return fail(RMX_E_INVALID, "bad rmx_queue_times arguments");
   *n = h->host || h->seq.dispatch != RMX_SEQ_QUEUE ? 0 : rmx::queue_times(h->device, stamps, cap);
   return RMX_OK;
+}
+
+int rmx_lean_check(const rmx_handle* h, int64_t* n_checked, int64_t* n_bad, char* report, size_t report_cap) {
+  if (!h || !n_checked || !n_bad) return fail(RMX_E_INVALID, "bad rmx_lean_check arguments");
+  if (!h->host) return fail(RMX_E_STATE, "rmx_lean_check: a host handle's tables are needed");
+  try {
+    const rmx::HostEngine& he = *h->host;
+    rmx_config c = he.cfg;
+    int32_t start_xy[2 * RMX_MAX_AGENTS];
+    for (int a = 0; a < RMX_MAX_AGENTS; ++a) start_xy[2 * a] = he.p.start_x[a], start_xy[2 * a + 1] = he.p.start_y[a];
+    c.init_q = he.p.init_q, c.final_q = he.p.final_q, c.start_xy = start_xy;
+    const rmx::LeanRules r = rmx::lean_rules(c);
+    rmx::LeanTable tb;
+    const std::string why = rmx::build_lean_table(he.cfg.kind, r, he.tv, tb);
+    if (!why.empty()) return fail(RMX_E_INVALID, why);
+    std::string first;
+    rmx::lean_check(he.cfg.kind, r, he.tv, tb, n_checked, n_bad, &first);
+    if (report && report_cap) {
+      const size_t n = std::min(first.size(), report_cap - 1);
+      std::memcpy(report, first.data(), n);
+      report[n] = 0;
+    }
+    return RMX_OK;
+  } catch (const std::exception& e) {
+    return fail(RMX_E_INVALID, std::string("rmx_lean_check: ") + e.what());
+  }
 }
 
 int rmx_code_object_check(const void* co, size_t bytes, int64_t* n_step_kernels, int64_t* n_refused, char* report,
diff --git a/multiagent-rl-rm_amd/csrc/rmx_fast.hip b/multiagent-rl-rm_amd/csrc/rmx_fast.hip
--- a/multiagent-rl-rm_amd/csrc/rmx_fast.hip
+++ b/multiagent-rl-rm_amd/csrc/rmx_fast.hip
@@ -619,6 +619,95 @@
 #include "rmx_fast_step.inc"
 }
 
+template <int KIND, int A, int TBL, bool RPT, int IO>
+__global__ void __launch_bounds__(256) step_fast_kernel_win_ln(int32_t N_arg, int32_t blk_arg, const int32_t* x_arg,
+                                                               const int32_t* y_arg, const int32_t* q_arg,
+                                                               const uint32_t* f_arg, const int32_t* t_arg,
+                                                               const int32_t* act_arg, FastParams p) {
+  static_assert(IO == kIoColsToLn || IO == kIoLnToCols, "the lean form's first and last packets");
+  constexpr bool HASHED = false;
+  constexpr int QXB = 0, SKIP = kSkipRare, SLIP = 0;
+#include "rmx_fast_step.inc"
+}
+
+template <int KIND, int A>
+__global__ void __launch_bounds__(256) step_fast_kernel_win_lean(int32_t, int32_t, const int32_t*, const int32_t*,
+                                                                 const int32_t*, const uint32_t*, const int32_t*,
+                                                                 const int32_t*, FastParams p) {
+  constexpr bool STATS_FIRST = KIND == RMX_FROZEN_LAKE && A <= 2;
+  const int32_t N = p.N;
+  const int32_t e_raw = (int32_t)blockIdx.x * (int32_t)blockDim.x + (int32_t)threadIdx.x;
+  const bool live = e_raw < N;
+  const int32_t e = live ? e_raw : N - 1;
+  const uint32_t off = (uint32_t)e * 4u, col = (uint32_t)N * 4u;
+  const auto r_pk = col_rsrc(p.pk, col * (uint32_t)(2 * A + 1));
+  const auto r_act = col_rsrc(p.actions, col * (uint32_t)A);
+  const uint32_t tw = (uint32_t)col_ld(r_pk, off, (uint32_t)ln_col_t(A) * col);
+  uint32_t w[A], en[A];
+  float ret[A], ret0[A];
+  int32_t act[A];
+#pragma unroll
+  for (int a = 0; a < A; ++a) {
+    w[a] = (uint32_t)col_ld(r_pk, off, (uint32_t)ln_col_word(A, a) * col);
+    ret[a] = __int_as_float(col_ld(r_pk, off, (uint32_t)ln_col_ret(A, a) * col));
+    act[a] = col_ld(r_act, off, a * col);
+  }
+  const auto r_ln = col_rsrc(p.ln_tbl, (uint32_t)p.ln_bytes);
+  const bool rs = p.autoreset && ln_done(tw);
+  const int32_t t = rs ? 0 : ln_t(tw);
+  const int32_t t1 = t + 1;
+  const float disc = p.gamma_is_one ? 1.0f : p.disc[min((uint32_t)t, (uint32_t)p.max_t + 1u)];
+  uint32_t bad = 0, all_term = 1u, all_trunc = 1u;
+#pragma unroll
+  for (int a = 0; a < A; ++a) {
+    w[a] = rs ? p.ln_init[a] : w[a];
+    ret0[a] = ret[a];
+    ret[a] = rs ? 0.0f : ret[a];
+    const uint32_t slot = ln_slot<KIND>(w[a], act[a], bad);
+    en[a] = __builtin_amdgcn_raw_buffer_load_b32(r_ln, ln_index(w[a], slot) * 4u, p.ln_base[a], 0);
+  }
+  uint32_t succ[A];
+#pragma unroll
+  for (int a = 0; a < A; ++a) {
+    const LeanOut o = ln_step<KIND>(w[a], en[a], t1, p.max_t, disc, ret[a]);
+    w[a] = o.word;
+    ret[a] = o.ret;
+    succ[a] = o.succ;
+    all_term &= o.term;
+    all_trunc &= o.trunc;
+  }
+  const uint32_t done = (all_term | all_trunc) & (live ? 1u : 0u);
+  auto flush_stats = [&]() {
+    if (done) {
+      double rsum = 0.0;
+      uint32_t sc = 0;
+#pragma unroll
+      for (int a = 0; a < A; ++a) {
+        rsum += (double)ret[a];
+        sc += succ[a];
+      }
+      env_stats_env(p, e, t1);
+      env_stats_ret(p, e, rsum, sc);
+    }
+  };
+  if constexpr (STATS_FIRST) flush_stats();
+  if (live) {
+    col_st(r_pk, off, (uint32_t)ln_col_t(A) * col, (int32_t)ln_t_word(t1, done != 0u));
+#pragma unroll
+    for (int a = 0; a < A; ++a) {
+      col_st(r_pk, off, (uint32_t)ln_col_word(A, a) * col, (int32_t)w[a]);
+      if (__float_as_int(ret[a]) != __float_as_int(ret0[a]))
+        col_st(r_pk, off, (uint32_t)ln_col_ret(A, a) * col, __float_as_int(ret[a]));
+    }
+  } else {
+    bad = 0;
+  }
+  if (__any(bad)) {
+    if ((threadIdx.x & 63) == 0) atomicOr(p.err, 1u);
+  }
+  if constexpr (!STATS_FIRST) flush_stats();
+}
+
 template <int KIND, int A, int TBL, int SLIP = 0>
 __global__ void __launch_bounds__(256) rollout_fast_kernel(FastParams p, int32_t T, float* __restrict__ trace) {
   static_assert(TBL == kTblGlobal || TBL == kTblMerged || TBL == kTblLds || TBL == kTblMergedLds,
@@ -941,8 +1030,42 @@
                      a.flags, a.t, a.actions, a.p);
 }
 
+template <int KIND, int A, int TBL, bool RPT, int IO>
+static void go_step_win_ln(dim3 g, dim3 b, hipStream_t st, const FastParams& p) {
+  const StepArgs a = step_args(p, b.x);
+  if (StepCapture* c = tl_capture) {
+    snprintf(c->out->symbol, sizeof(c->out->symbol),
+             "_ZN3rmx23step_fast_kernel_win_lnILi%dELi%dELi%dELb%dELi%dEEEviiPKiS2_S2_PKjS2_S2_NS_10FastParamsE.kd", KIND,
+             A, TBL, (int)RPT, IO);
+    return capture_launch(c, g, b, 0, a, p);
+  }
+  hipLaunchKernelGGL((step_fast_kernel_win_ln<KIND, A, TBL, RPT, IO>), g, b, 0, st, a.N, a.blk, a.pos_x, a.pos_y, a.rm_q,
+                     a.flags, a.t, a.actions, a.p);
+}
+template <int KIND, int A>
+static void go_step_win_lean(dim3 g, dim3 b, hipStream_t st, const FastParams& p) {
+  const StepArgs a = step_args(p, b.x);
+  if (StepCapture* c = tl_capture) {
+    snprintf(c->out->symbol, sizeof(c->out->symbol),
+             "_ZN3rmx25step_fast_kernel_win_leanILi%dELi%dEEEviiPKiS2_S2_PKjS2_S2_NS_10FastParamsE.kd", KIND, A);
+    return capture_launch(c, g, b, 0, a, p);
+  }
+  hipLaunchKernelGGL((step_fast_kernel_win_lean<KIND, A>), g, b, 0, st, a.N, a.blk, a.pos_x, a.pos_y, a.rm_q, a.flags,
+                     a.t, a.actions, a.p);
+}
+
 template <int KIND, int A, int TBL>
 static void launch_win(const FastParams& p, dim3 g, dim3 b, hipStream_t st) {
+  if constexpr (A >= 2) {
+    switch (p.pk_io) {
+      case kIoColsToLn: return go_step_win_ln<KIND, A, TBL, false, kIoColsToLn>(g, b, st, p);
+      case kIoLnToLn: return go_step_win_lean<KIND, A>(g, b, st, p);
+      case kIoLnToCols:
+        if (p.rpt_out) return go_step_win_ln<KIND, A, TBL, true, kIoLnToCols>(g, b, st, p);
+        return go_step_win_ln<KIND, A, TBL, false, kIoLnToCols>(g, b, st, p);
+      default: break;
+    }
+  }
   switch (p.pk_io) {
     case kIoColsToPk: go_step_win<KIND, A, TBL, false, kIoColsToPk>(g, b, st, p); break;
     case kIoPkToPk: go_step_win<KIND, A, TBL, false, kIoPkToPk>(g, b, st, p); break;
@@ -1007,7 +1130,9 @@
       }
       return go(std::integral_constant<int, kRngSlip>{});
     }
-    if (p.pk_io != kIoCols && p.pk && !hashed && !p.qrm_s && !p.wave_stats) return launch_win<KIND, A, TBL>(p, g, b, st);
+    if (p.pk_io != kIoCols && p.pk && !hashed && !p.qrm_s && !p.wave_stats &&
+        (p.pk_io < kIoColsToLn || (p.ln_tbl && A >= 2)))
+      return launch_win<KIND, A, TBL>(p, g, b, st);
   }
   if (p.rpt_out && !hashed) {
     go_step<KIND, A, false, TBL, 0, kSkipRare, true>(g, b, 0, st, p);
diff --git a/multiagent-rl-rm_amd/csrc/rmx_fast_step.inc b/multiagent-rl-rm_amd/csrc/rmx_fast_step.inc
--- a/multiagent-rl-rm_amd/csrc/rmx_fast_step.inc
+++ b/multiagent-rl-rm_amd/csrc/rmx_fast_step.inc
@@ -1,9 +1,10 @@
   constexpr bool QRM = QXB > 0;
   constexpr bool IN_PK = IO == kIoPkToPk || IO == kIoPkToCols, OUT_PK = IO == kIoColsToPk || IO == kIoPkToPk;
+  constexpr bool IN_LN = IO == kIoLnToCols, OUT_LN = IO == kIoColsToLn;
   static_assert(IO == kIoCols || ((TBL == kTblMerged || TBL == kTblMerged4) && !HASHED && QXB == 0 && SLIP == 0 &&
                                   SKIP == kSkipRare),
                 "packed windows: the deterministic merged-table step (x, y, rm_q come out of table bytes)");
-  static_assert(!(RPT && OUT_PK), "the report rides in a window's last packet");
+  static_assert(!(RPT && (OUT_PK || OUT_LN)), "the report rides in a window's last packet");
   static_assert(TBL == kTblGlobal || TBL == kTblMerged || TBL == kTblMerged4, "step: global or merged tables");
   static_assert(!QRM || TBL == kTblGlobal, "QRM outputs need the move word's event (global tables)");
   constexpr bool M4 = TBL == kTblMerged4;
@@ -48,7 +49,7 @@
   AgentIO s[A];
   AgentIO s0[A];
   int32_t t;
-  if constexpr (!IN_PK) t = col_ld(r_t, off, 0);
+  if constexpr (!IN_PK && !IN_LN) t = col_ld(r_t, off, 0);
   __amdgpu_buffer_rsrc_t r_ret;
   [[maybe_unused]] const auto r_pk = col_rsrc(p.pk, IO != kIoCols ? col * (uint32_t)(3 * A + 1) : 0u);
   if constexpr (IN_PK) {
@@ -63,6 +64,28 @@
       s[a].f = (uint32_t)col_ld(r_pk, off, (uint32_t)pk_col_flags(A, a) * col);
       s[a].ret = __int_as_float(col_ld(r_pk, off, (uint32_t)pk_col_ret(A, a) * col));
       s[a].act = col_ld(r_act, off, a * col);
+      s0[a] = s[a];
+    }
+  } else if constexpr (IN_LN) {
+    const uint32_t tw = (uint32_t)col_ld(r_pk, off, (uint32_t)ln_col_t(A) * col);
+    t = ln_t(tw);
+    r_ret = col_rsrc(p.ep_ret, cols);
+    const auto r_ln = col_rsrc(p.ln_tbl, (uint32_t)p.ln_bytes);
+    uint32_t lw[A], cw[A];
+#pragma unroll
+    for (int a = 0; a < A; ++a) {
+      lw[a] = (uint32_t)col_ld(r_pk, off, (uint32_t)ln_col_word(A, a) * col);
+      s[a].ret = __int_as_float(col_ld(r_pk, off, (uint32_t)ln_col_ret(A, a) * col));
+      s[a].act = col_ld(r_act, off, a * col);
+    }
+#pragma unroll
+    for (int a = 0; a < A; ++a) cw[a] = __builtin_amdgcn_raw_buffer_load_b32(r_ln, ln_row(lw[a]) * 4u, p.ln_rows_off, 0);
+#pragma unroll
+    for (int a = 0; a < A; ++a) {
+      s[a].x = (int32_t)pk_x(cw[a]);
+      s[a].y = (int32_t)pk_y(cw[a]);
+      s[a].q = (int32_t)pk_q(cw[a]);
+      s[a].f = ln_flags(lw[a], ln_done(tw));
       s0[a] = s[a];
     }
   } else if constexpr (!PRE) {
@@ -357,7 +380,19 @@
   };
   if constexpr (STATS_FIRST) flush_stats();
   STAMP(6);
-  if constexpr (OUT_PK) {
+  if constexpr (OUT_LN) {
+    if (live) {
+      st(r_pk, off, (uint32_t)ln_col_t(A) * col, (int32_t)ln_t_word(t1, done != 0u));
+#pragma unroll
+      for (int a = 0; a < A; ++a) {
+        const uint32_t row = __umul24((uint32_t)s[a].q, (uint32_t)p.HW) + __umul24((uint32_t)s[a].y, (uint32_t)p.W) + (uint32_t)s[a].x;
+        st(r_pk, off, (uint32_t)ln_col_word(A, a) * col, (int32_t)ln_word(row, s[a].f, s[a].q == p.final_q[a]));
+        st(r_pk, off, (uint32_t)ln_col_ret(A, a) * col, __float_as_int(s[a].ret));
+      }
+    } else {
+      bad = 0;
+    }
+  } else if constexpr (OUT_PK) {
     if (live) {
       st(r_pk, off, (uint32_t)pk_col_t(A) * col, t1);
 #pragma unroll
@@ -372,7 +407,7 @@
       bad = 0;
     }
   } else if (live) {
-    constexpr bool ALL = SKIP == kSkipNone || IO == kIoPkToCols;
+    constexpr bool ALL = SKIP == kSkipNone || IO == kIoPkToCols || IO == kIoLnToCols;
     st(r_t, off, 0, t1);
     if (p.env_done) byte_st<SAUX>(p, (uint32_t)e, done);
 #pragma unroll
diff --git a/multiagent-rl-rm_amd/csrc/rmx_handle.h b/multiagent-rl-rm_amd/csrc/rmx_handle.h
--- a/multiagent-rl-rm_amd/csrc/rmx_handle.h
+++ b/multiagent-rl-rm_amd/csrc/rmx_handle.h
@@ -27,6 +27,11 @@
     bool pk_refused = false;
     uint32_t* d_pk = nullptr;
     bool is_packed = false;
+    bool lean_off = false;
+    bool ln_failed = false;
+    rmx::LeanTable ln;
+    uint32_t* d_ln = nullptr;
+    bool is_lean = false;
     int dispatch = RMX_SEQ_NONE;
     int64_t recordings = 0;
   } seq;
diff --git a/multiagent-rl-rm_amd/csrc/rmx_internal.h b/multiagent-rl-rm_amd/csrc/rmx_internal.h
--- a/multiagent-rl-rm_amd/csrc/rmx_internal.h
+++ b/multiagent-rl-rm_amd/csrc/rmx_internal.h
@@ -7,6 +7,7 @@
 
 #include "../../include/rmx.h"
 #include "rmx_layout.h"
+#include "rmx_lean.h"
 #include "rmx_learn.h"
 #include "rmx_rules.h"
 
@@ -172,6 +173,11 @@
   uint32_t* pk;
   int32_t pk_io;
   int32_t pad7;
+  const uint32_t* ln_tbl;
+  int32_t ln_bytes;
+  uint32_t ln_rows_off;
+  uint32_t ln_base[kFastMaxAgents];
+  uint32_t ln_init[kFastMaxAgents];
 };
 #define RMX_FAST_PARAMS_FIELDS(X) X(tables) X(n16) X(off_rm) X(off_info) X(pad6) X(merged) \
    X(merged_bytes) X(mg_base) X(pad0) X(merged4) X(merged4_bytes) X(mg_palb) X(HW) X(qrm_s) X(qrm_sn) X(qrm_rq) \
@@ -183,7 +189,8 @@
    X(pad3) X(stamps) X(rpt_out) X(rpt_partial) X(rpt_ticket) X(rpt_cs) X(rpt_n_slab) X(slip_n) X(slip_out) \
    X(slip_thr) X(slip_uniform) X(pad4) X(slip_pack) X(seed_scale) X(seed_env_stride) X(seed_episode_stride) \
    X(base_seed) X(rng) X(episode) X(slip) X(n_free) X(free_cells) X(start_ws) X(nx_rng) X(nx_idx) X(nx_ep) \
-   X(rs_jump) X(rs_cells) X(rs_rng) X(rs_dirty) X(pad5) X(pk) X(pk_io) X(pad7)
+   X(rs_jump) X(rs_cells) X(rs_rng) X(rs_dirty) X(pad5) X(pk) X(pk_io) X(pad7) X(ln_tbl) X(ln_bytes) X(ln_rows_off) \
+   X(ln_base) X(ln_init)
 #define RMX_FP_FIELD_BYTES(f) +sizeof(FastParams::f)
 constexpr size_t kFastParamsFieldBytes = 0 RMX_FAST_PARAMS_FIELDS(RMX_FP_FIELD_BYTES);
 #undef RMX_FP_FIELD_BYTES
diff --git a/multiagent-rl-rm_amd/csrc/rmx_lean.h b/multiagent-rl-rm_amd/csrc/rmx_lean.h
--- /dev/null
+++ b/multiagent-rl-rm_amd/csrc/rmx_lean.h
@@ -0,0 +1,106 @@
+#pragma once
+#include <stddef.h>
+#include <stdint.h>
+
+#include <string>
+#include <vector>
+
+#include "rmx_layout.h"
+#include "rmx_rules.h"
+
+namespace rmx {
+
+constexpr uint32_t kLnRowMask = 0x1FFFu, kLnMaxRows = 8192u;
+constexpr uint32_t kLnActive = 1u << 13, kLnFail = 1u << 14, kLnAtFinal = 1u << 15;
+constexpr uint32_t kLnDone = 1u << 31;
+constexpr uint32_t kLnERmTerm = 1u << 13, kLnEFail = 1u << 14;
+constexpr uint32_t kLnKeep = kLnRowMask | kLnAtFinal;
+constexpr int kLnSlots = 6, kLnSlotStill = 5;
+constexpr int kIoColsToLn = 4, kIoLnToLn = 5, kIoLnToCols = 6;
+
+constexpr int ln_col_word(int , int a) { return a; }
+constexpr int ln_col_ret(int A, int a) { return A + a; }
+constexpr int ln_col_t(int A) { return 2 * A; }
+constexpr size_t ln_bytes(int A, size_t n_envs) { return (size_t)(2 * A + 1) * n_envs * 4; }
+
+constexpr uint32_t ln_word(uint32_t row, uint32_t flags, bool at_final) {
+  return (row & kLnRowMask) | ((flags & RMX_F_ACTIVE) ? kLnActive : 0u) | ((flags & RMX_F_FAIL) ? kLnFail : 0u) |
+         (at_final ? kLnAtFinal : 0u) | (flags & 0xFFFF0000u);
+}
+constexpr uint32_t ln_row(uint32_t w) { return w & kLnRowMask; }
+constexpr uint32_t ln_flags(uint32_t w, bool env_done) {
+  return ((w >> 13) & 3u) | (env_done ? (uint32_t)RMX_F_ENV_DONE : 0u) | (w & 0xFFFF0000u);
+}
+constexpr uint32_t ln_t_word(int32_t t1, bool env_done) {
+  return ((uint32_t)t1 & ~kLnDone) | (env_done ? kLnDone : 0u);
+}
+constexpr int32_t ln_t(uint32_t tw) { return (int32_t)(tw << 1) >> 1; }
+constexpr bool ln_done(uint32_t tw) { return (tw & kLnDone) != 0; }
+constexpr uint32_t ln_entry(uint32_t next_row, bool rm_term, bool fails, bool next_at_final, int reward) {
+  return (next_row & kLnRowMask) | (rm_term ? kLnERmTerm : 0u) | (fails ? kLnEFail : 0u) |
+         (next_at_final ? kLnAtFinal : 0u) | ((uint32_t)(uint8_t)(int8_t)reward << 16);
+}
+
+template <int KIND>
+RMX_HD uint32_t ln_slot(uint32_t w, int32_t act, uint32_t& bad) {
+  const uint32_t active = (w >> 13) & 1u, at_final = (w >> 15) & 1u;
+  const uint32_t moving = KIND == RMX_FROZEN_LAKE ? (active & (at_final ^ 1u)) : active;
+  bad |= (uint32_t)act > (uint32_t)RMX_WAIT ? 1u : 0u;
+  const uint32_t ac = (uint32_t)act < (uint32_t)RMX_WAIT ? (uint32_t)act : (uint32_t)RMX_WAIT;
+  return moving ? ac : (uint32_t)kLnSlotStill;
+}
+RMX_HD uint32_t ln_index(uint32_t w, uint32_t slot) { return (w & kLnRowMask) * (uint32_t)kLnSlots + slot; }
+
+struct LeanOut {
+  uint32_t word;
+  float ret, reward;
+  uint32_t term, trunc, succ;
+};
+template <int KIND>
+RMX_HD LeanOut ln_step(uint32_t w, uint32_t en, int32_t t1, int32_t max_t, float disc, float ret) {
+  const uint32_t active = (w >> 13) & 1u, at_final = (w >> 15) & 1u;
+  const uint32_t moving = KIND == RMX_FROZEN_LAKE ? (active & (at_final ^ 1u)) : active;
+  const uint32_t wf = w + (moving << RMX_F_STEPS_SHIFT);
+  const uint32_t fail = ((w | en) >> 14) & 1u;
+  uint32_t trunc, env_term;
+  if (KIND == RMX_FROZEN_LAKE) {
+    trunc = ((wf >> RMX_F_STEPS_SHIFT) > (uint32_t)max_t || t1 > max_t) ? 1u : 0u;
+    env_term = trunc | at_final | fail;
+  } else {
+    trunc = t1 > max_t ? 1u : 0u;
+    env_term = fail;
+  }
+  const uint32_t still = active & ((env_term | trunc) ^ 1u);
+  const uint32_t rm_term = (en >> 13) & 1u;
+  LeanOut o;
+  o.reward = (float)(int32_t)(int8_t)(uint8_t)(en >> 16);
+  o.ret = fmaf(disc, o.reward, ret);
+  o.term = env_term | rm_term;
+  o.trunc = trunc;
+  o.succ = (rm_term && o.ret > 0.0f) ? 1u : 0u;
+  o.word = (wf & 0xFFFF0000u) | (en & kLnKeep) | (still << 13) | (fail << 14);
+  return o;
+}
+
+struct LeanRules {
+  int32_t W, HW, A, Q, E, max_t;
+  float hazard_penalty, wall_penalty;
+  int32_t hazard_fail, wall_fail, has_shaping, stochastic;
+  float reward_modifier;
+  int32_t final_q[RMX_MAX_AGENTS], init_q[RMX_MAX_AGENTS], start_x[RMX_MAX_AGENTS], start_y[RMX_MAX_AGENTS];
+};
+inline int32_t slip_choice(const LeanRules&, int32_t intended, Pcg&) { return intended; }
+LeanRules lean_rules(const rmx_config& c);
+
+struct LeanTable {
+  std::vector<uint32_t> words;
+  uint32_t base[kFastMaxAgents] = {};
+  uint32_t rows_off = 0;
+  uint32_t init[kFastMaxAgents] = {};
+  int32_t rows = 0;
+};
+std::string build_lean_table(int kind, const LeanRules& r, const TableView& T, LeanTable& out);
+void lean_check(int kind, const LeanRules& r, const TableView& T, const LeanTable& tb, int64_t* n_checked,
+                int64_t* n_bad, std::string* first);
+
+}
diff --git a/multiagent-rl-rm_amd/csrc/rmx_tables.cpp b/multiagent-rl-rm_amd/csrc/rmx_tables.cpp
--- a/multiagent-rl-rm_amd/csrc/rmx_tables.cpp
+++ b/multiagent-rl-rm_amd/csrc/rmx_tables.cpp
@@ -1,8 +1,11 @@
 #include "rmx_host.h"
 
+#include <stdio.h>
 #include <string.h>
 
 #include <algorithm>
+
+#include "rmx_lean.h"
 
 namespace rmx {
 
@@ -255,4 +258,141 @@
   return out;
 }
 
-}
+LeanRules lean_rules(const rmx_config& c) {
+  LeanRules r{};
+  r.W = c.width, r.HW = c.width * c.height, r.A = c.n_agents, r.Q = c.n_rm_states, r.E = c.n_events, r.max_t = c.max_t;
+  r.hazard_penalty = c.hazard_penalty, r.wall_penalty = c.wall_penalty;
+  r.hazard_fail = c.hazard_fail ? 1 : 0, r.wall_fail = c.wall_fail ? 1 : 0;
+  r.has_shaping = c.has_shaping ? 1 : 0, r.stochastic = c.stochastic ? 1 : 0;
+  r.reward_modifier = c.reward_modifier;
+  for (int a = 0; a < c.n_agents && a < RMX_MAX_AGENTS; ++a) {
+    r.final_q[a] = c.final_q[a], r.init_q[a] = c.init_q[a];
+    r.start_x[a] = c.start_xy[2 * a], r.start_y[a] = c.start_xy[2 * a + 1];
+  }
+  return r;
+}
+
+namespace {
+
+template <int KIND>
+std::string lean_build(const LeanRules& r, const TableView& T, LeanTable& out) {
+  const int A = r.A, HW = r.HW, W = r.W;
+  if (A < 1 || A > kFastMaxAgents) return "lean window: more agents than the fast path takes";
+  if (r.stochastic) return "lean window: slip draws are not table entries";
+  if ((int64_t)r.Q * HW > (int64_t)kLnMaxRows) return "lean window: more than 8192 rows per agent";
+  const int rows = r.Q * HW;
+  LeanRules rr = r;
+  rr.max_t = 0x7ffffff0;
+  out = LeanTable();
+  out.rows = rows;
+  const size_t sec = (size_t)rows * kLnSlots;
+  std::vector<uint32_t> s(sec);
+  for (int a = 0; a < A; ++a) {
+    const int32_t fq = r.final_q[a];
+    for (int row = 0; row < rows; ++row) {
+      const int q = row / HW, cell = row % HW;
+      for (int slot = 0; slot < kLnSlots; ++slot) {
+        const bool moves = slot < kLnSlotStill && !(KIND == RMX_FROZEN_LAKE && q == fq);
+        AgentReg st = {cell % W, cell / W, q, moves ? RMX_F_ACTIVE : 0u, 0.0f};
+        uint32_t bad = 0;
+        const AgentOut o = agent_step<KIND>(st, moves ? slot : RMX_WAIT, a, 1, T, rr, &bad, (Pcg*)nullptr);
+        const float rw = o.reward;
+        uint32_t bits;
+        memcpy(&bits, &rw, 4);
+        if (!(rw >= -128.0f && rw <= 127.0f && rw == (float)(int)rw) || (rw == 0.0f && (bits >> 31)))
+          return "lean window: a step reward is not an integer in [-128, 127]";
+        const uint32_t nrow = (uint32_t)st.q * (uint32_t)HW + (uint32_t)st.y * (uint32_t)W + (uint32_t)st.x;
+        s[(size_t)row * kLnSlots + slot] =
+            ln_entry(nrow, st.q == fq, (st.f & RMX_F_FAIL) != 0, st.q == fq, (int)rw);
+      }
+    }
+    size_t same = out.words.size() / sec;
+    for (size_t b = 0; b < out.words.size() / sec; ++b)
+      if (std::equal(s.begin(), s.end(), out.words.begin() + b * sec)) {
+        same = b;
+        break;
+      }
+    if (same == out.words.size() / sec) out.words.insert(out.words.end(), s.begin(), s.end());
+    out.base[a] = (uint32_t)(same * sec * 4);
+    const uint32_t r0 = (uint32_t)r.init_q[a] * (uint32_t)HW + (uint32_t)r.start_y[a] * (uint32_t)W + (uint32_t)r.start_x[a];
+    out.init[a] = ln_word(r0, RMX_F_ACTIVE, r.init_q[a] == fq);
+  }
+  out.rows_off = (uint32_t)(out.words.size() * 4);
+  for (int row = 0; row < rows; ++row) {
+    const int q = row / HW, cell = row % HW;
+    out.words.push_back(pk_cell((uint32_t)(cell % W), (uint32_t)(cell / W), (uint32_t)q));
+  }
+  return std::string();
+}
+
+template <int KIND>
+void lean_check_kind(const LeanRules& r, const TableView& T, const LeanTable& tb, int64_t* n_checked, int64_t* n_bad,
+                     std::string* first) {
+  const int HW = r.HW, W = r.W;
+  const int32_t acts[6] = {0, 1, 2, 3, 4, 7};
+  const int32_t t1s[3] = {1, r.max_t, r.max_t + 1};
+  const int32_t stepss[4] = {0, r.max_t - 1, r.max_t, r.max_t + 1};
+  const float rets[2] = {0.0f, -2.5f};
+  int64_t nc = 0, nb = 0;
+  for (int a = 0; a < r.A; ++a) {
+    const int32_t fq = r.final_q[a];
+    const uint32_t* sec = tb.words.data() + tb.base[a] / 4;
+    for (int row = 0; row < tb.rows; ++row)
+      for (uint32_t fl = 0; fl < 4; ++fl)
+        for (int32_t act : acts)
+          for (int32_t t1 : t1s)
+            for (int32_t steps : stepss)
+              for (float ret0 : rets) {
+                if (steps < 0 || steps > 0xFFFF || t1 < 1) continue;
+                const int q = row / HW, cell = row % HW;
+                const uint32_t f0 = (fl & 1u ? RMX_F_ACTIVE : 0u) | (fl & 2u ? RMX_F_FAIL : 0u) |
+                                    ((uint32_t)steps << RMX_F_STEPS_SHIFT);
+                const float disc = 0.75f;
+                AgentReg st = {cell % W, cell / W, q, f0, ret0};
+                uint32_t bad_ref = 0;
+                const AgentOut o = agent_step<KIND>(st, act, a, t1, T, r, &bad_ref, (Pcg*)nullptr);
+                const float ret_ref = fmaf(disc, o.reward, ret0);
+                const uint32_t succ_ref = (o.term && st.q == fq && ret_ref > 0.0f) ? 1u : 0u;
+                const uint32_t nrow = (uint32_t)st.q * (uint32_t)HW + (uint32_t)st.y * (uint32_t)W + (uint32_t)st.x;
+                const uint32_t word_ref = ln_word(nrow, st.f, st.q == fq);
+                const uint32_t w0 = ln_word((uint32_t)row, f0, q == fq);
+                uint32_t bad = 0;
+                const uint32_t slot = ln_slot<KIND>(w0, act, bad);
+                const LeanOut l = ln_step<KIND>(w0, sec[ln_index(w0, slot)], t1, r.max_t, disc, ret0);
+                ++nc;
+                const bool ok = l.word == word_ref && memcmp(&l.ret, &ret_ref, 4) == 0 &&
+                                memcmp(&l.reward, &o.reward, 4) == 0 && l.term == (o.term ? 1u : 0u) &&
+                                l.trunc == (o.trunc ? 1u : 0u) && l.succ == succ_ref && bad == bad_ref &&
+                                ln_flags(l.word, false) == (st.f & (RMX_F_ACTIVE | RMX_F_FAIL | 0xFFFF0000u));
+                if (!ok && nb++ == 0 && first) {
+                  char buf[256];
+                  snprintf(buf, sizeof(buf),
+                           "agent %d row %d flags %u act %d t1 %d steps %d: word %08x (rules %08x) ret %g (%g) reward %g "
+                           "(%g) term %u (%d) trunc %u (%d) succ %u (%u) bad %u (%u)",
+                           a, row, fl, act, t1, steps, l.word, word_ref, (double)l.ret, (double)ret_ref,
+                           (double)l.reward, (double)o.reward, l.term, (int)o.term, l.trunc, (int)o.trunc, l.succ,
+                           succ_ref, bad, bad_ref);
+                  *first = buf;
+                }
+              }
+  }
+  *n_checked = nc;
+  *n_bad = nb;
+}
+
+}
+
+std::string build_lean_table(int kind, const LeanRules& r, const TableView& T, LeanTable& out) {
+  return kind == RMX_FROZEN_LAKE ? lean_build<RMX_FROZEN_LAKE>(r, T, out) : lean_build<RMX_OFFICE_WORLD>(r, T, out);
+}
+
+void lean_check(int kind, const LeanRules& r, const TableView& T, const LeanTable& tb, int64_t* n_checked,
+                int64_t* n_bad, std::string* first) {
+  if (first) first->clear();
+  if (kind == RMX_FROZEN_LAKE)
+    lean_check_kind<RMX_FROZEN_LAKE>(r, T, tb, n_checked, n_bad, first);
+  else
+    lean_check_kind<RMX_OFFICE_WORLD>(r, T, tb, n_checked, n_bad, first);
+}
+
+}
diff --git a/multiagent-rl-rm_amd/rmx/_capi.py b/multiagent-rl-rm_amd/rmx/_capi.py
--- a/multiagent-rl-rm_amd/rmx/_capi.py
+++ b/multiagent-rl-rm_amd/rmx/_capi.py
@@ -22,7 +22,7 @@
     "rmx_get_state", "rmx_set_state", "rmx_step_report", "rmx_step_report_fused", "rmx_reset_sync", "rmx_step_sync",
     "rmx_step_sync_begin", "rmx_sync_wait", "rmx_sync_end", "rmx_step_seq", "rmx_queue_counters", "rmx_queue_info",
     "rmx_code_object_check", "rmx_device_count", "rmx_queue_timing", "rmx_queue_times", "rmx_step_info",
-    "rmx_seq_packed", "rmx_learn_states", "rmx_learn_bind", "rmx_learn_step", "rmx_learn_step_policy",
+    "rmx_seq_packed", "rmx_lean_check", "rmx_learn_states", "rmx_learn_bind", "rmx_learn_step", "rmx_learn_step_policy",
     "rmx_learn_rng_bind", "rmx_learn_rng_seed", "rmx_learn_lambda_slots", "rmx_learn_lambda_bind",
     "rmx_learn_traces_clear", "rmx_learn_run", "rmx_learn_eps_bind", "rmx_learn_eps_decay",
 )
@@ -53,7 +53,7 @@
                   "rmx_comd.cpp", "rmx_build_info.cpp", "rmx_internal.h", "rmx_layout.h", "rmx_host.h", "rmx_device.h",
                   "rmx_generic.h", "rmx_comd.h", "rmx_hoststep.cpp", "rmx_hoststep.h", "rmx_learn.hip", "rmx_learn_run.hip", "rmx_learn.h",
                   "rmx_rules.h", "../../include/rmx.h",
-                  "Makefile", "rmx_learn_eps.hip", "rmx_learn_run_eps.hip")
+                  "Makefile", "rmx_learn_eps.hip", "rmx_learn_run_eps.hip", "rmx_lean.h")
 
 
 def source_hash(csrc: str = CSRC) -> str:
@@ -194,6 +194,7 @@
         "rmx_step_report": (C.c_int, [vp, vp, C.c_int, vp, vp]),
         "rmx_step_report_fused": (C.c_int, [vp]),
         "rmx_seq_packed": (C.c_int, [vp]),
+        "rmx_lean_check": (C.c_int, [vp, C.POINTER(C.c_int64), C.POINTER(C.c_int64), C.c_char_p, C.c_size_t]),
         "rmx_step_seq": (C.c_int, [vp, vp, C.c_int64, C.c_int32, C.c_int, vp, vp]),
         "rmx_queue_timing": (C.c_int, [vp, C.c_int]),
         "rmx_queue_times": (C.c_int, [vp, vp, C.c_int64, C.POINTER(C.c_int64)]),
```
